# Tongji-MIC-Lab/TDVC

Measured on AMD Instinct MI355X. Metric: 1080p P-frames/sec (encode + reconstruct, lambda=2048 config), higher is better.
Workload: dtype f16; 1 GPU; 1x 1920x1080 (padded 1088x1920) 7-frame synthetic GOP (seed 1234), batch 1, P-frames coded in GOP order; gop=7, batch=1, parallelism=gop-sharded x1, weights=closed-form filler (no checkpoint ships)

## Files before the change

include/tdvc_hip.h:

```cpp
#ifndef TDVC_HIP_H
#define TDVC_HIP_H

#include <stdint.h>

#ifdef __cplusplus
extern "C" {
#endif

#define TDVC_OK 0
#define TDVC_EINVAL (-1)
#define TDVC_ENOSUP (-2)

typedef struct {
  void* p;
  int32_t N, H, W, C;
  int64_t sn;
  int32_t sp;
  int32_t dtype;
} tdvc_fmap;

enum { TDVC_F16 = 0, TDVC_F32 = 1 };
enum { TDVC_ACT_NONE = 0, TDVC_ACT_RELU = 1, TDVC_ACT_LRELU = 2, TDVC_ACT_CLAMP01 = 3, TDVC_ACT_SIGMOID = 4 };
enum { TDVC_GDN_NONE = 0, TDVC_GDN_FWD = 1, TDVC_GDN_INV = 2 };
enum { TDVC_OUT_NHWC = 0,
       TDVC_OUT_SHUFFLE2 = 1,
       TDVC_OUT_NCHW_F32 = 2 };

#define TDVC_MAX_TAPS 49

typedef struct {
  tdvc_fmap x;
  tdvc_fmap y;
  const void* w;
  const float* bias;
  int32_t cout;
  int32_t ntaps;
  int8_t tap_dy[TDVC_MAX_TAPS], tap_dx[TDVC_MAX_TAPS];
  int32_t kh, kw, stride, pad;
  int32_t ck;
  int32_t square_input;
  int32_t gdn;
  tdvc_fmap aux;
  int32_t act; float slope;
  int32_t round_before_act;
  tdvc_fmap res;
  tdvc_fmap res2;
  int32_t out_mode;
  int32_t s2d;
  int32_t bcast_T;
  float bcast_slope;
  float* chan_sum;
} tdvc_conv_desc;

int tdvc_abi_version(void);
const char* tdvc_last_error(void);
int tdvc_prepare_device(void);
const char* tdvc_last_conv_kernel(void);

int tdvc_set_predicate(const int* flag);
int tdvc_last_launch_predicated(void);
#define TDVC_MAX_PREDICATE_IMAGES 4
int tdvc_set_predicate_images(const int* flags, int n);
int tdvc_frame_changed(const tdvc_fmap* cur, tdvc_fmap* cache, int* flag, void* stream);
int tdvc_frames_changed(const tdvc_fmap* cur, tdvc_fmap* cache, int* flags, unsigned force_mask, void* stream);


int tdvc_conv_plan(int cin, int kh, int kw, int stride);
int64_t tdvc_conv_packed_bytes(int cout, int cin, int ntaps, int ck);
int tdvc_pack_conv_weights(const float* w_oihw, int cout, int cin_real, int cin, int kh, int kw,
                           int ntaps, const int8_t* tap_dy, const int8_t* tap_dx, int ck, uint16_t* dst);
int tdvc_conv2d(const tdvc_conv_desc* d, void* stream);
int tdvc_conv_chan_sum_rows(const tdvc_conv_desc* d);
const char* tdvc_conv_select(const tdvc_conv_desc* d);
int tdvc_conv2d_f32(const tdvc_conv_desc* d, void* stream);

typedef struct {
  tdvc_fmap x, y;
  const void* w;
  const float* bias;
  int32_t act1; float slope1;
  int32_t act2; float slope2;
  int32_t add_input;
  tdvc_fmap res2;
} tdvc_conv_pair_desc;
int64_t tdvc_conv_pair_packed_bytes(void);
int tdvc_pack_conv_pair_weights(const float* w1_oihw, const float* w2_oihw, uint16_t* dst);
int tdvc_conv_pair_supported(const tdvc_conv_pair_desc* d);
int tdvc_conv_pair(const tdvc_conv_pair_desc* d, void* stream);

typedef struct {
  tdvc_fmap x, om, y;
  const void* w;
  const float* bias;
  int32_t groups;
  int32_t act; float slope; int32_t round_before_act;
  void* x_planar;
} tdvc_dcn_desc;
int tdvc_dcn_fused(const tdvc_dcn_desc* d, void* stream);

int tdvc_dcn_v2_forward_f32(const float* input, const float* weight, const float* bias,
                            const float* offset, const float* mask, float* output,
                            int B, int C, int H, int W, int Cout,
                            int kh, int kw, int sh, int sw, int ph, int pw, int dh, int dw,
                            int deformable_group, void* stream);
int tdvc_dcn_v2_backward_f32(const float* input, const float* weight, const float* bias,
                             const float* offset, const float* mask, const float* grad_output,
                             float* grad_input, float* grad_offset, float* grad_mask,
                             float* grad_weight, float* grad_bias, float* columns,
                             int B, int C, int H, int W, int Cout,
                             int kh, int kw, int sh, int sw, int ph, int pw, int dh, int dw,
                             int deformable_group, void* stream);

int tdvc_nchw_to_fmap(const float* src, int C, const tdvc_fmap* y, void* stream);
int tdvc_fmap_to_nchw(const tdvc_fmap* x, int C, float* dst, void* stream);
int tdvc_scale_act_res(const tdvc_fmap* a, const float* gate, int act, float slope,
                       const tdvc_fmap* r, float r_sign, const tdvc_fmap* y, const tdvc_fmap* y2, void* stream);
int tdvc_add_flow(const tdvc_fmap* off, const tdvc_fmap* flow, void* stream);
int tdvc_bcast_add_act(const tdvc_fmap* x, const tdvc_fmap* b, int T, float slope, void* stream);

int tdvc_channel_sum(const tdvc_fmap* x, float* partial, int nblocks, void* stream);
int tdvc_se_gate(const float* partial, int nblocks, float inv_count, int N, int C, int Cmid,
                 const float* w1, const float* b1, const float* w2, const float* b2,
                 float* gate, void* stream);

int tdvc_upsample2x(const tdvc_fmap* x, const tdvc_fmap* y, void* stream);
int tdvc_avgpool2(const tdvc_fmap* x, const tdvc_fmap* y, void* stream);
int tdvc_spynet_level_input(const tdvc_fmap* ref, const tdvc_fmap* supp, const tdvc_fmap* flow_lo,
                            const tdvc_fmap* flow_up, const tdvc_fmap* cat8, void* stream);
int tdvc_resize_bilinear(const tdvc_fmap* x, const tdvc_fmap* y, const float* chscale, void* stream);

int64_t tdvc_avgpool_k_work_floats(int N, int hp, int wp, int C, int scale);
int tdvc_avgpool_k(const tdvc_fmap* x, int scale, float* pooled, int hp, int wp, float* work, int64_t work_floats, void* stream);
int tdvc_patch_match(const float* pin, const float* pref, int N, int hp, int wp, int C,
                     int32_t* idx, void* stream);
int tdvc_match_gather(const tdvc_fmap* fin, const tdvc_fmap* fref, const int32_t* idx, int scale,
                      int hp, int wp, const tdvc_fmap* cat, void* stream);

int tdvc_eb_forward(const tdvc_fmap* z, const float* params, const tdvc_fmap* noise,
                    const tdvc_fmap* z_hat, double* bits_out, float* partial, int partial_cap, void* stream);
int tdvc_gc_forward(const tdvc_fmap* y, const tdvc_fmap* gp, const tdvc_fmap* noise,
                    double* bits_out, float* partial, int partial_cap, void* stream);
int tdvc_quantize(const tdvc_fmap* y, const tdvc_fmap* noise, const tdvc_fmap* y_hat, void* stream);

int64_t tdvc_rans_encode(const int32_t* symbols, const int32_t* indexes, int64_t n,
                         const int32_t* cdfs, int32_t cdf_stride, const int32_t* cdf_sizes,
                         const int32_t* offsets, uint8_t* out, int64_t cap);
int tdvc_rans_decode(const uint8_t* data, int64_t nbytes, const int32_t* indexes, int64_t n,
                     const int32_t* cdfs, int32_t cdf_stride, const int32_t* cdf_sizes,
                     const int32_t* offsets, int32_t* symbols_out);

void* tdvc_rans_decoder_create(const uint8_t* data, int64_t nbytes);
int tdvc_rans_decoder_decode(void* handle, const int32_t* indexes, int64_t n, const int32_t* cdfs,
                             int32_t cdf_stride, const int32_t* cdf_sizes, const int32_t* offsets,
                             int32_t* symbols_out);
void tdvc_rans_decoder_destroy(void* handle);

int64_t tdvc_rans_encode_lanes(const int32_t* symbols, const int32_t* indexes, int64_t npos, int M, int L,
                               const int32_t* cdfs, int32_t cdf_stride, const int32_t* cdf_sizes,
                               const int32_t* offsets, uint8_t* out, int64_t cap);
int tdvc_rans_decode_lanes(const uint8_t* data, int64_t nbytes, const int32_t* indexes, int64_t npos, int M,
                           const int32_t* cdfs, int32_t cdf_stride, const int32_t* cdf_sizes,
                           const int32_t* offsets, int32_t* symbols_out);

int tdvc_pmf_to_quantized_cdf(const float* pmf, int n, int precision, int32_t* cdf_out);

int tdvc_ar_gather_batch(const tdvc_fmap* y_hat, const tdvc_fmap* params, const int32_t* pos, int npos,
                         const tdvc_fmap* x1, const tdvc_fmap* pc, void* stream);
int tdvc_ar_quantize_batch(const tdvc_fmap* y, const tdvc_fmap* gp, const int32_t* pos, int npos, const float* scale_table, int ntable,
                           const int32_t* symbols_in, const tdvc_fmap* y_hat, int32_t* symbols, int32_t* indexes, int64_t cbase, void* stream);
int tdvc_ar_indexes_batch(const tdvc_fmap* gp, const int32_t* pos, int npos, int B, const float* scale_table, int ntable,
                          int M, int H, int W, int32_t* indexes, int64_t cbase, void* stream);
int tdvc_ar_wavefront_batch(const uint8_t* const* data, const int64_t* nbytes, int B, const int32_t* cdfs, int32_t cdf_stride,
                            const int32_t* cdf_sizes, const int32_t* offsets, const tdvc_fmap* y, const tdvc_fmap* y_hat,
                            const tdvc_fmap* params, const tdvc_fmap* x1, const tdvc_fmap* pc, const tdvc_conv_desc* convs, int nconvs,
                            const tdvc_fmap* gp, const int32_t* pos_dev, const int32_t* step_sizes, int nsteps, int M, int W,
                            const float* scale_table, int ntable, int32_t* idx_dev, int32_t* sym_dev, void* stream);
int tdvc_ar_decode_serial_batch(const uint8_t* const* data, const int64_t* nbytes, int B, const int32_t* cdfs, int32_t cdf_stride,
                                const int32_t* cdf_sizes, const int32_t* offsets, const tdvc_fmap* y_hat, const tdvc_fmap* params,
                                const tdvc_fmap* x1, const tdvc_fmap* pc, const tdvc_conv_desc* convs, int nconvs, const tdvc_fmap* gp,
// ... 123 lines not shown
```

tdvc_amd/_lib.py:

```python
from __future__ import annotations

import ctypes as C
import os

_HERE = os.path.dirname(os.path.abspath(__file__))
LIB_PATH = os.path.join(_HERE, "libtdvc_hip.so")

MAX_TAPS = 49
F16, F32 = 0, 1
ACT_NONE, ACT_RELU, ACT_LRELU, ACT_CLAMP01, ACT_SIGMOID = 0, 1, 2, 3, 4
GDN_NONE, GDN_FWD, GDN_INV = 0, 1, 2
OUT_NHWC, OUT_SHUFFLE2, OUT_NCHW_F32 = 0, 1, 2


class FMapDesc(C.Structure):
    _fields_ = [("p", C.c_void_p), ("N", C.c_int32), ("H", C.c_int32), ("W", C.c_int32), ("C", C.c_int32),
                ("sn", C.c_int64), ("sp", C.c_int32), ("dtype", C.c_int32)]


class ConvDesc(C.Structure):
    _fields_ = [("x", FMapDesc), ("y", FMapDesc), ("w", C.c_void_p), ("bias", C.c_void_p),
                ("cout", C.c_int32), ("ntaps", C.c_int32),
                ("tap_dy", C.c_int8 * MAX_TAPS), ("tap_dx", C.c_int8 * MAX_TAPS),
                ("kh", C.c_int32), ("kw", C.c_int32), ("stride", C.c_int32), ("pad", C.c_int32),
                ("ck", C.c_int32), ("square_input", C.c_int32), ("gdn", C.c_int32),
                ("aux", FMapDesc), ("act", C.c_int32), ("slope", C.c_float),
                ("round_before_act", C.c_int32), ("res", FMapDesc), ("res2", FMapDesc), ("out_mode", C.c_int32), ("s2d", C.c_int32),
                ("bcast_T", C.c_int32), ("bcast_slope", C.c_float), ("chan_sum", C.c_void_p)]


class DcnDesc(C.Structure):
    _fields_ = [("x", FMapDesc), ("om", FMapDesc), ("y", FMapDesc), ("w", C.c_void_p), ("bias", C.c_void_p),
                ("groups", C.c_int32), ("act", C.c_int32), ("slope", C.c_float), ("round_before_act", C.c_int32), ("x_planar", C.c_void_p)]


class ConvPairDesc(C.Structure):
    _fields_ = [("x", FMapDesc), ("y", FMapDesc), ("w", C.c_void_p), ("bias", C.c_void_p), ("act1", C.c_int32), ("slope1", C.c_float),
                ("act2", C.c_int32), ("slope2", C.c_float), ("add_input", C.c_int32), ("res2", FMapDesc)]


class WgradReduceJob(C.Structure):
    _fields_ = [("work", C.c_void_p), ("bwork", C.c_void_p), ("row_off", C.c_void_p), ("chan_off", C.c_void_p), ("tap_off", C.c_void_p),
                ("bias_index", C.c_void_p), ("dw", C.c_void_p), ("db", C.c_void_p), ("scale", C.c_float),
                ("nworkers", C.c_int32), ("cow", C.c_int32), ("ciw", C.c_int32), ("ntaps", C.c_int32), ("cout", C.c_int32), ("cin", C.c_int32),
                ("wblocks", C.c_int32), ("nblocks", C.c_int32)]


_P = C.c_void_p
_FM = C.POINTER(FMapDesc)
_i, _f, _i64 = C.c_int, C.c_float, C.c_int64

SIGNATURES = {
    "tdvc_abi_version": (_i, []),
    "tdvc_conv_chan_sum_rows": (_i, [C.POINTER(ConvDesc)]),
    "tdvc_conv_select": (C.c_char_p, [C.POINTER(ConvDesc)]),
    "tdvc_last_error": (C.c_char_p, []),
    "tdvc_last_conv_kernel": (C.c_char_p, []),
    "tdvc_prepare_device": (_i, []),
    "tdvc_set_predicate": (_i, [_P]),
    "tdvc_set_predicate_images": (_i, [_P, _i]),
    "tdvc_last_launch_predicated": (_i, []),
    "tdvc_frame_changed": (_i, [_FM, _FM, _P, _P]),
    "tdvc_frames_changed": (_i, [_FM, _FM, _P, C.c_uint, _P]),
    "tdvc_conv_plan": (_i, [_i, _i, _i, _i]),
    "tdvc_conv_packed_bytes": (_i64, [_i, _i, _i, _i]),
    "tdvc_pack_conv_weights": (_i, [_P, _i, _i, _i, _i, _i, _i, _P, _P, _i, _P]),
    "tdvc_conv2d": (_i, [C.POINTER(ConvDesc), _P]),
    "tdvc_conv2d_f32": (_i, [C.POINTER(ConvDesc), _P]),
    "tdvc_pack_conv_weights_indexed": (_i, [_P] * 7 + [_i] * 4 + [_P, _P]),
    "tdvc_pack_conv_weights_indexed_f32": (_i, [_P] * 7 + [_i] * 4 + [_P, _P]),
    "tdvc_pack_job_blocks": (_i64, [_i, _i, _i, _i]),
    "tdvc_pack_conv_weights_batch": (_i, [_P, _P, _i, _i, _P]),
    "tdvc_act_backward": (_i, [_FM, _FM, _FM, _i, _f, _FM, _P]),
    "tdvc_pixel_unshuffle": (_i, [_FM, _FM, _P]),
    "tdvc_bias_grad_work_floats": (_i64, [_i, _i]),
    "tdvc_bias_grad": (_i, [_FM, _i, _P, _f, _P, _P, _i64, _P]),
    "tdvc_copy_cast": (_i, [_FM, _FM, _P]),
    "tdvc_clamp01_backward": (_i, [_FM, _FM, _P]),
    "tdvc_gate_backward_work_floats": (_i64, [_i, _i]),
    "tdvc_gate_backward": (_i, [_FM, _FM, _P, _FM, _P, _P, _i64, _P]),
    "tdvc_se_gate_backward": (_i, [_P, _i, _f, _i, _i, _i] + [_P] * 6 + [_f] + [_P] * 6),
    "tdvc_bcast_channel_add": (_i, [_FM, _P, _f, _P]),
    "tdvc_add_flow_backward": (_i, [_FM, _FM, _P]),
    "tdvc_bcast_add_act_backward": (_i, [_FM, _FM, _FM, _f, _P]),
    "tdvc_upsample2x_backward": (_i, [_FM, _FM, _P]),
    "tdvc_resize_bilinear_backward": (_i, [_FM, _FM, _P, _P]),
    "tdvc_spynet_level_input_backward": (_i, [_FM, _FM, _FM, _FM, _FM, _P]),
    "tdvc_sigmoid_f32": (_i, [_P, _P, _i64, _P]),
    "tdvc_sigmoid_backward_f32": (_i, [_P, _P, _i64, _P]),
    "tdvc_axpy_f32": (_i, [_P, _P, _f, _i64, _P]),
    "tdvc_match_gather_backward": (_i, [_FM, _FM, _P, _i, _i, _i, _FM, _FM, _FM, _P]),
    "tdvc_eb_backward": (_i, [_FM, _P, _FM, _f, _FM, _P, _P]),
    "tdvc_eb_pack": (_i, [_P, _P, _P, _i, _P]),
    "tdvc_eb_param_chain": (_i, [_P, _P, _P, _f, _i, _P]),
    "tdvc_eb_aux": (_i, [_P, _P, _f, _P, _P, _i, _P]),
    "tdvc_gc_backward": (_i, [_FM, _FM, _FM, _f, _FM, _FM, _P]),
    "tdvc_dcn_columns": (_i, [_FM, _FM, _i, _FM, _P]),
    "tdvc_ar_lanes_state_bytes": (_i64, [_i]),
    "tdvc_ar_gather_batch": (_i, [_FM, _FM, _P, _i, _FM, _FM, _P]),
    "tdvc_ar_quantize_batch": (_i, [_FM, _FM, _P, _i, _P, _i, _P, _FM, _P, _P, _i64, _P]),
    "tdvc_ar_indexes_batch": (_i, [_FM, _P, _i, _i, _P, _i, _i, _i, _i, _P, _i64, _P]),
    "tdvc_ar_wavefront_batch": (_i, [_P, _P, _i, _P, _i, _P, _P, _FM, _FM, _FM, _FM, _FM, _P, _i, _FM, _P, _P, _i, _i, _i, _P, _i, _P, _P, _P]),
    "tdvc_ar_decode_serial_batch": (_i, [_P, _P, _i, _P, _i, _P, _P, _FM, _FM, _FM, _FM, _P, _i, _FM, _P, _i, _i, _i, _P, _i, _P, _P, _P]),
    "tdvc_ar_lanes_batch_layout": (_i64, [_P, _i, _i, _P]),
    "tdvc_ar_lanes_init_batch": (_i, [_P, _i64, _P, _i, _i, _P, _P]),
    "tdvc_ar_decode_lanes_step_batch": (_i, [_FM, _P, _i, _P, _i, _P, _i64, _P, _i, _P, C.c_int32, _P, _P, _P, C.c_int32, _P, _FM, _P, _P, _i64, _P]),
    "tdvc_ar_wavefront_lanes_batch": (_i, [_P, _P, _i, _P, _i64, _P, _P, C.c_int32, _P, _P, _P, C.c_int32, _FM, _FM, _FM, _FM, _P, _i, _FM, _P, _P, _i, _i, _i,
                                           _P, _i, _P, _P, _P, _P]),
# ... 85 lines not shown
```

tdvc_amd/csrc/conv_common.h:

```cpp
#pragma once
#include "common.h"

namespace convk {

struct ConvParams {
  const half_t* x; long x_sn; int x_sp; int H, W, Cin;
  const half_t* w; const float* bias;
  FMap y; int Ho, Wo; int cout;
  FMap aux; FMap res; FMap res2;
  int ntaps, kh, kw, pad;
  int in_stride;
  int nchunks, steps;
  int square, gdn, act; float slope; int round16, out_mode;
  int tiles_x;
  int simple;
  int s2d, Corig;
  int reverse;
  int bcast_T; float bcast_slope;
  float* csum;
  int8_t tap_dy[TDVC_MAX_TAPS], tap_dx[TDVC_MAX_TAPS];
  const int* pred;
};

enum ConvSwitch { SW_NONE = -1, SW_V2, SW_V3, SW_V5, SW_V7, SW_V9, SW_V10, SW_V11, SW_ROW, SW_C8, SW_N16, SW_GDN128, SW_COUNT };
int conv_on(int id);
long conv_v9_work_limit();

constexpr long LARGE_MAP_PIXELS = 8192;

inline bool taps_dense(const tdvc_conv_desc* d, int kh, int kw, int pad) {
  if (d->ntaps != kh * kw || d->kh != kh || d->kw != kw || d->pad != pad) return false;
  for (int t = 0; t < d->ntaps; ++t)
    if (d->tap_dy[t] != t / kw || d->tap_dx[t] != t % kw) return false;
  return true;
}

inline bool all_waves_store(const tdvc_conv_desc* d, int wave_ch) {
  const int ych = d->out_mode == TDVC_OUT_SHUFFLE2 ? d->cout >> 2 : (d->cout + wave_ch - 1) / wave_ch * wave_ch;
  return d->y.C > ych - wave_ch;
}

inline int persistent_grid_x(int slots, int cout_blocks, int N, int ntiles) {
  const int gx = slots / (cout_blocks * N);
  return gx < 1 ? 1 : (gx > ntiles ? ntiles : gx);
}

template <auto Kern, typename... Args>
int launch_big_lds(const char* what, int lds_limit, dim3 grid, dim3 block, int lds, hipStream_t st, Args... args) {
  static TdvcPerDeviceFlag raised;
  bool& done = raised.flag();
  if (!done) {
    const hipError_t err = hipFuncSetAttribute(reinterpret_cast<const void*>(Kern), hipFuncAttributeMaxDynamicSharedMemorySize, lds_limit);
    if (err != hipSuccess) { tdvc_set_error("%s: hipFuncSetAttribute failed: %s", what, hipGetErrorString(err)); return (int)err; }
    done = true;
  }
  hipLaunchKernelGGL(Kern, grid, block, lds, st, args...);
  return tdvc_launch_status(what);
}


template <bool F32MAPS = false>
__device__ __forceinline__ void epilogue4(const ConvParams& p, int n, int oy, int ox, int co, float v[4]) {
  if (p.bias) {
    const f32x4 b4 = *reinterpret_cast<const f32x4*>(p.bias + co);
#pragma unroll
    for (int i = 0; i < 4; ++i) v[i] += b4[i];
  }
  int py = oy, px = ox, pc = co, PW = p.Wo;
  if (p.out_mode == TDVC_OUT_SHUFFLE2) {
    const int cq = p.cout >> 2;
    const int sub = co / cq;
    pc = co - sub * cq;
    py = 2 * oy + (sub >> 1);
    px = 2 * ox + (sub & 1);
    PW = 2 * p.Wo;
  }
  if (p.gdn) {
// ... 149 lines not shown
#pragma unroll
  for (int k0 = 0; k0 < 4; k0 += KB) {
    half8 r0[KB], r1[KB], r2[KB];
    int opix[KB], apix[KB];
    bool ok[KB];
#pragma unroll
    for (int k = 0; k < KB; ++k) {
      const int ox = ox_first + (k0 + k) * 8 + prow;
      ok[k] = full ? ch_ok : (row_ok && ox < p.Wo);
      opix[k] = ok[k] ? (mul * oy + sub_y) * PW + (mul * ox + sub_x) : 0;
      apix[k] = ok[k] ? oy * p.Wo + ox : 0;
    }
    if (gdn) {
      const half_t* ab = reinterpret_cast<const half_t*>(p.aux.p) + (long)n * p.aux.sn + (ch_ok ? co : 0);
#pragma unroll
      for (int k = 0; k < KB; ++k) r0[k] = *reinterpret_cast<const half8*>(ab + (long)apix[k] * p.aux.sp);
    }
    if (has1) {
      const half_t* rb = reinterpret_cast<const half_t*>(p.res.p) + (long)n * p.res.sn + pcc;
#pragma unroll
      for (int k = 0; k < KB; ++k) r1[k] = *reinterpret_cast<const half8*>(rb + (long)opix[k] * p.res.sp);
    }
    if (has2) {
      const half_t* rb = reinterpret_cast<const half_t*>(p.res2.p) + (long)n * p.res2.sn + pcc;
#pragma unroll
      for (int k = 0; k < KB; ++k) r2[k] = *reinterpret_cast<const half8*>(rb + (long)opix[k] * p.res2.sp);
    }
#pragma unroll
    for (int k = 0; k < KB; ++k) {
      half8 h = *reinterpret_cast<const half8*>(ew + ((k0 + k) * 8 + prow) * EPS + chunk * 16);
      if (gdn) {
        float v[8];
#pragma unroll
        for (int j = 0; j < 8; ++j) v[j] = (float)r0[k][j] * (p.gdn == TDVC_GDN_FWD ? rsqrtf((float)h[j]) : sqrtf((float)h[j]));
        if (has1) {
#pragma unroll
          for (int j = 0; j < 8; ++j) v[j] += (float)r1[k][j];
        }
        if (has2) {
#pragma unroll
          for (int j = 0; j < 8; ++j) v[j] += (float)r2[k][j];
        }
#pragma unroll
        for (int j = 0; j < 8; ++j) h[j] = (half_t)v[j];
      } else {
        if (has1) h = h + r1[k];
        if (has2) h = h + r2[k];
      }
      if (ok[k]) *reinterpret_cast<half8*>(reinterpret_cast<half_t*>(p.y.p) + (long)n * p.y.sn + (long)opix[k] * p.y.sp + pc) = h;
    }
  }
}

template <int NTX, bool BIAS_IN_ACC, bool BCAST = false, bool CSUM = false>
__device__ __forceinline__ void epilogue_lean_seq(const ConvParams& p, f32x16 (&acc)[2][NTX], const float* bias64, unsigned char* ew, int n,
                                                  int cbase, int oy_first, int ox_first, int lane, bool zero_acc, bool full, float* cs = nullptr) {
  constexpr int EPS = 144;
  const int hh = lane >> 5, r = lane & 31;
  const int chunk = lane & 7, prow = lane >> 3;
  const int co = cbase + chunk * 8;
  const bool ch_ok = co < p.y.C && co < ((p.cout + 63) & ~63);
  const int cc = ch_ok ? co : 0;
  const bool has1 = p.res.p != nullptr, has2 = p.res2.p != nullptr;
  const half_t sl = (half_t)p.slope;
  const half2v sl2 = {sl, sl}, zero2 = {(half_t)0.f, (half_t)0.f};
  const bool act = p.slope != 1.f, relu = p.slope == 0.f;
  half_t* yb = reinterpret_cast<half_t*>(p.y.p) + (long)n * p.y.sn + cc;
  const half_t* rb1 = reinterpret_cast<const half_t*>(p.res.p) + (long)n * p.res.sn + cc;
  const half_t* rb2 = reinterpret_cast<const half_t*>(p.res2.p) + (long)n * p.res2.sn + cc;
  f32x4 b4[2][4];
  if constexpr (!BIAS_IN_ACC) {
#pragma unroll
    for (int mt = 0; mt < 2; ++mt)
#pragma unroll
      for (int g = 0; g < 4; ++g) b4[mt][g] = *reinterpret_cast<const f32x4*>(bias64 + mt * 32 + 8 * g + 4 * hh);
  }
#pragma unroll
  for (int nt = 0; nt < NTX; ++nt) {
    const int oy = oy_first + nt;
    int opix[4];
    bool ok[4];
#pragma unroll
    for (int k = 0; k < 4; ++k) {
      const int ox = ox_first + k * 8 + prow;
      ok[k] = full ? ch_ok : (ch_ok && oy < p.Ho && ox < p.Wo);
      opix[k] = ok[k] ? oy * p.Wo + ox : 0;
    }
    half8 r1[4], r2[4];
    if (has1 && !BCAST) {
#pragma unroll
      for (int k = 0; k < 4; ++k) r1[k] = *reinterpret_cast<const half8*>(rb1 + (long)opix[k] * p.res.sp);
    }
    if (has2) {
#pragma unroll
      for (int k = 0; k < 4; ++k) r2[k] = *reinterpret_cast<const half8*>(rb2 + (long)opix[k] * p.res2.sp);
    }
#pragma unroll
    for (int mt = 0; mt < 2; ++mt)
#pragma unroll
      for (int g = 0; g < 4; ++g) {
        float v[4];
#pragma unroll
        for (int i = 0; i < 4; ++i) {
          v[i] = acc[mt][nt][4 * g + i];
          if constexpr (!BIAS_IN_ACC) {
            v[i] += b4[mt][g][i];
            if (zero_acc) acc[mt][nt][4 * g + i] = 0.f;
          }
        }
        half2v lo = {(half_t)v[0], (half_t)v[1]}, hi = {(half_t)v[2], (half_t)v[3]};
        if (relu) {
          lo = __builtin_elementwise_max(lo, zero2);
          hi = __builtin_elementwise_max(hi, zero2);
        } else if (act) {
          lo = __builtin_elementwise_max(lo, lo * sl2);
          hi = __builtin_elementwise_max(hi, hi * sl2);
        }
        const half4 o = {lo[0], lo[1], hi[0], hi[1]};
        *reinterpret_cast<half4*>(ew + r * EPS + (mt * 32 + 8 * g + 4 * hh) * 2) = o;
      }
    if constexpr (BCAST) {
#pragma unroll
      for (int k = 0; k < 4; ++k) {
        const half8 v = *reinterpret_cast<const half8*>(ew + (k * 8 + prow) * EPS + chunk * 16);
        half_t* yp = yb + (long)opix[k] * p.y.sp;
        const half_t* sp = has1 ? rb1 + (long)opix[k] * p.res.sp : yp;
        half8 xs[4];
#pragma unroll
        for (int t = 0; t < 4; ++t) xs[t] = *reinterpret_cast<const half8*>(sp + t * 64);
#pragma unroll
        for (int t = 0; t < 4; ++t) {
          half8 o;
#pragma unroll
          for (int j = 0; j < 8; ++j) {
            const float s = (float)xs[t][j] + (float)v[j];
            o[j] = (half_t)(s > 0.f ? s : s * p.bcast_slope);
          }
          if (ok[k]) *reinterpret_cast<half8*>(yp + t * 64) = o;
        }
      }
      continue;
    }
#pragma unroll
    for (int k = 0; k < 4; ++k) {
      half8 v = *reinterpret_cast<const half8*>(ew + (k * 8 + prow) * EPS + chunk * 16);
      if (has1) v = v + r1[k];
      if (has2) v = v + r2[k];
      if (ok[k]) *reinterpret_cast<half8*>(yb + (long)opix[k] * p.y.sp) = v;
      if constexpr (CSUM) {
#pragma unroll
        for (int j = 0; j < 8; ++j) cs[j] += ok[k] ? (float)v[j] : 0.f;
      }
    }
  }
}

template <int NTX, bool BIAS_IN_ACC = false, int MODE = 3>
__device__ __forceinline__ void epilogue_simple_rows(const ConvParams& p, f32x16 (&acc)[2][NTX], const float* bias64,
                                                     unsigned char* ew, int n, int cbase, int oy_first, int ox_first,
                                                     int lane, bool zero_acc, bool full = false) {
  if constexpr (MODE == 2) {
    epilogue_lean_seq<NTX, BIAS_IN_ACC>(p, acc, bias64, ew, n, cbase, oy_first, ox_first, lane, zero_acc, full);
    return;
  }
  if constexpr (MODE == 3) {
    if (p.simple == 2) {
      epilogue_lean_seq<NTX, BIAS_IN_ACC>(p, acc, bias64, ew, n, cbase, oy_first, ox_first, lane, zero_acc, full);
      return;
    }
  }
  PackedRow rows[NTX];
  epilogue_pack<NTX, BIAS_IN_ACC>(p, acc, bias64, lane, rows, zero_acc);
#pragma unroll
  for (int nt = 0; nt < NTX; ++nt) epilogue_store_row(p, rows[nt], ew, n, cbase, oy_first + nt, ox_first, lane, full);
}

inline bool conv_is_lean(const ConvParams& p) {
  return conv_is_simple(p) && p.out_mode == TDVC_OUT_NHWC && !p.gdn;
}

template <int NRES, int NR, bool STAMPED = false>
__device__ __forceinline__ void epilogue_lean_rows(const ConvParams& p, const f32x16 (&acc)[2][NR], unsigned char* ew, int n,
                                                   int cbase, int oy, int ox_first, int lane, bool full, long long* st = nullptr) {
#define EST(i) do { if constexpr (STAMPED) { if (st) st[i] = clock64(); } } while (0)
  static_assert(NR % 2 == 0, "two rows per round");
  constexpr int EPS = 144, EROW = 32 * EPS;
  const int hh = lane >> 5, r = lane & 31;
  const int chunk = lane & 7, prow = lane >> 3;
  const int co = cbase + chunk * 8;
  const bool ch_ok = co < p.y.C && co < ((p.cout + 63) & ~63);
  const int cc = ch_ok ? co : 0;
  int opix[NR][4];
  bool ok[NR][4];
#pragma unroll
  for (int j = 0; j < NR; ++j)
#pragma unroll
    for (int k = 0; k < 4; ++k) {
      const int ox = ox_first + k * 8 + prow;
      ok[j][k] = full ? ch_ok : (ch_ok && oy + j < p.Ho && ox < p.Wo);
      opix[j][k] = ok[j][k] ? (oy + j) * p.Wo + ox : 0;
// ... 61 lines not shown
```

tdvc_amd/csrc/conv_dispatch.hip:

```cpp
#include <stdlib.h>

#include "conv_common.h"

using convk::ConvParams;
bool conv_v2_eligible(const tdvc_conv_desc* d, int Ho, int Wo); int launch_conv_v2(const ConvParams& p, int cout_blocks, int N, hipStream_t st);
bool conv_v3_eligible(const tdvc_conv_desc* d, int Ho, int Wo); int launch_conv_v3(const ConvParams& p, int cout_blocks, int N, hipStream_t st);
bool conv_v5_eligible(const tdvc_conv_desc* d, int Ho, int Wo); int launch_conv_v5(const ConvParams& p, int cout_blocks, int N, hipStream_t st); int conv_v5_chan_sum_rows(int Ho, int Wo, int cout_blocks, int N);
bool conv_v7_eligible(const tdvc_conv_desc* d, const ConvParams& p, int Ho, int Wo); int launch_conv_v7(const ConvParams& p, int cout_blocks, int N, hipStream_t st);
bool conv_v9_eligible(const tdvc_conv_desc* d, int Ho, int Wo, bool v3_ok); int launch_conv_v9(const ConvParams& p, int ck8, int cout_tiles32, int N, hipStream_t st);
bool conv_v10_eligible(const tdvc_conv_desc* d, const ConvParams& p, int Ho, int Wo); int launch_conv_v10(const ConvParams& p, int cout_blocks, int N, hipStream_t st);
bool conv_v11_eligible(const tdvc_conv_desc* d, const ConvParams& p, int Ho, int Wo); int launch_conv_v11(const ConvParams& p, int cout_blocks, int N, hipStream_t st);
int conv_row_geometry(const tdvc_conv_desc* d, const ConvParams& p, int Ho, int Wo); int launch_conv_row(int geo, const ConvParams& p, int N, hipStream_t st);
bool conv_c8_eligible(const tdvc_conv_desc* d, const ConvParams& p, int Ho, int Wo); int launch_conv_c8(const ConvParams& p, int N, hipStream_t st);
bool conv_n16_eligible(const tdvc_conv_desc* d, int Ho, int Wo); int launch_conv_n16(const ConvParams& p, int N, hipStream_t st);
bool gdn128_eligible(const tdvc_conv_desc* d, const ConvParams& p, int Ho, int Wo); int launch_gdn128(const ConvParams& p, int N, hipStream_t st);
int conv_direct_lds_bytes(const tdvc_conv_desc* d);
int conv_cout_tiles(int cout);
int launch_conv_direct(const ConvParams& p, int ck8, int stride, int N, hipStream_t st);
int conv_f32_validate(const tdvc_conv_desc* d, int& Ho, int& Wo);

namespace {
const char* const kSwitchEnv[convk::SW_COUNT] = {nullptr, "TDVC_CONV_NO_V3", "TDVC_CONV_NO_V5", "TDVC_CONV_NO_V7", "TDVC_CONV_NO_V9", "TDVC_CONV_NO_V10",
                                                 "TDVC_CONV_NO_V11", "TDVC_CONV_NO_ROW", "TDVC_CONV_NO_C8", "TDVC_CONV_NO_N16", "TDVC_CONV_NO_GDN128"};
int g_enabled[convk::SW_COUNT] = {1, 1, 1, 1, 1, 1, 1, 15, 1, 1, 1};
long g_v9_work_limit = 1L << 20;
}

int convk::conv_on(int id) {
  static const struct EnvOff {
    bool off[convk::SW_COUNT];
    EnvOff() {
      const bool v1 = getenv("TDVC_CONV_V1") != nullptr;
      for (int i = 0; i < convk::SW_COUNT; ++i) off[i] = v1 || (kSwitchEnv[i] && getenv(kSwitchEnv[i]) != nullptr);
    }
  } env;
  return id == convk::SW_NONE ? 1 : (env.off[id] ? 0 : g_enabled[id]);
}
long convk::conv_v9_work_limit() { return g_v9_work_limit; }

extern "C" void tdvc_debug_enable_conv_v9(int enable) { g_enabled[convk::SW_V9] = enable != 0; }
extern "C" void tdvc_debug_enable_conv_v10(int enable) { g_enabled[convk::SW_V10] = enable != 0; }
extern "C" void tdvc_debug_enable_conv_v11(int enable) { g_enabled[convk::SW_V11] = enable != 0; }
extern "C" void tdvc_debug_enable_conv_row(int mask) { g_enabled[convk::SW_ROW] = mask; }
extern "C" void tdvc_debug_enable_conv_c8(int enable) { g_enabled[convk::SW_C8] = enable != 0; }
extern "C" void tdvc_debug_enable_conv_n16(int enable) { g_enabled[convk::SW_N16] = enable != 0; }
extern "C" void tdvc_debug_enable_gdn128(int enable) { g_enabled[convk::SW_GDN128] = enable != 0; }
extern "C" void tdvc_debug_set_conv_v9_work_limit(long v) { g_v9_work_limit = v; }

namespace {

struct Pick {
  const tdvc_conv_desc* d;
  int Ho, Wo;
  int geo;
  int ck8() const { return d->ck / 8; }
  int N() const { return d->x.N; }
  int cout_blocks() const { return conv_cout_tiles(d->cout) / 2; }
};

struct Entry {
  const char* name;
  int sw;
  bool (*eligible)(Pick& k, const ConvParams& p);
  int (*launch)(const Pick& k, const ConvParams& p, hipStream_t st);
  bool (*only)(const tdvc_conv_desc* d);
  const char* only_msg;
};

bool v3_on_and_eligible(const Pick& k) { return convk::conv_on(convk::SW_V3) && conv_v3_eligible(k.d, k.Ho, k.Wo); }

bool bcast_eligible(Pick& k, const ConvParams& p) {
  const tdvc_conv_desc* d = k.d;
  return d->bcast_T == 4 && d->kh == 1 && d->kw == 1 && d->stride == 1 && d->pad == 0 && d->cout == 64 && d->y.C == 64 && d->y.sp >= 4 * 64 &&
         d->y.dtype == TDVC_F16 && d->out_mode == TDVC_OUT_NHWC && d->act == TDVC_ACT_NONE && !d->gdn && !d->res2.p &&
         (!d->res.p || (d->res.dtype == TDVC_F16 && d->res.C == 64 && d->res.sp >= 4 * 64 && d->res.N == d->y.N && d->res.H == d->y.H && d->res.W == d->y.W)) &&
         !d->square_input && !d->round_before_act && d->bias && d->bcast_slope >= 0.f && d->bcast_slope <= 1.f && conv_v5_eligible(d, k.Ho, k.Wo) &&
         convk::conv_is_lean(p);
}
int bcast_launch(const Pick& k, const ConvParams& p, hipStream_t st) {
  ConvParams q = p;
  q.simple = 2;
  q.slope = 1.f;
  return launch_conv_v5(q, 1, k.N(), st);
}
bool row_eligible(Pick& k, const ConvParams& p) { return (k.geo = conv_row_geometry(k.d, p, k.Ho, k.Wo)) >= 0; }

constexpr char kNameV5[] = "conv_mfma_v5", kNameDirect[] = "conv_mfma<%d,%d,%d>";

const Entry kTable[] = {
    {"conv_mfma_v5(bcast)", convk::SW_V5, bcast_eligible, bcast_launch, [](const tdvc_conv_desc* d) { return d->bcast_T != 0; },
     "tdvc_conv2d: bcast_T needs a plain 1x1 / stride 1 conv to 64 channels of >= 8192 pixels, y (and res, the optional source of the slices) a 64-channel window of a buffer with >= 4 slices, bcast_T == 4"},
    {"conv_row(s2d)", convk::SW_ROW, [](Pick& k, const ConvParams& p) { return k.d->s2d && row_eligible(k, p); },
     [](const Pick& k, const ConvParams& p, hipStream_t st) { return launch_conv_row(k.geo, p, k.N(), st); }, nullptr, nullptr},
    {"conv_mfma_v3(s2d)", convk::SW_V3, [](Pick& k, const ConvParams&) { return k.d->s2d && conv_v3_eligible(k.d, k.Ho, k.Wo); },
     [](const Pick& k, const ConvParams& p, hipStream_t st) { return launch_conv_v3(p, k.cout_blocks(), k.N(), st); },
     [](const tdvc_conv_desc* d) { return d->s2d != 0; }, "tdvc_conv2d: s2d conv not eligible for the stage-pipelined kernel"},
    {"conv_mfma_v9", convk::SW_V9, [](Pick& k, const ConvParams&) { return conv_v9_eligible(k.d, k.Ho, k.Wo, v3_on_and_eligible(k)); },
     [](const Pick& k, const ConvParams& p, hipStream_t st) { return launch_conv_v9(p, k.ck8(), conv_cout_tiles(k.d->cout), k.N(), st); }, nullptr, nullptr},
    {"gdn128", convk::SW_GDN128, [](Pick& k, const ConvParams& p) { return gdn128_eligible(k.d, p, k.Ho, k.Wo); },
// ... 74 lines not shown
    if (d->y.dtype == TDVC_F16) TDVC_CHECK((d->y.C % 8) == 0, "tdvc_conv2d: fp16 output C %% 8");
  }
  if (d->gdn) {
    TDVC_CHECK(fmap_ok16(d->aux) && d->aux.H == Ho && d->aux.W == Wo && d->aux.N == d->x.N && d->aux.C >= d->cout &&
                   !shuf && (d->cout % 64) == 0,
               "tdvc_conv2d: GDN aux fmap mismatch");
  }
  if (d->res.p) {
    TDVC_CHECK(d->res.dtype == TDVC_F32 ? fmap_ok32(d->res) : fmap_ok16(d->res), "tdvc_conv2d: bad residual fmap");
    TDVC_CHECK(d->res.N == d->x.N && d->res.H == (shuf ? 2 * Ho : Ho) && d->res.W == (shuf ? 2 * Wo : Wo),
               "tdvc_conv2d: residual geometry mismatch");
  }
  if (d->res2.p) {
    TDVC_CHECK(fmap_ok16(d->res2) && d->res2.N == d->x.N && d->res2.H == (shuf ? 2 * Ho : Ho) && d->res2.W == (shuf ? 2 * Wo : Wo),
               "tdvc_conv2d: bad second residual fmap");
  }
  if (d->bias) TDVC_CHECK(aligned16(d->bias), "tdvc_conv2d: bias unaligned");

  memset(&p, 0, sizeof(p));
  p.x = reinterpret_cast<const half_t*>(d->x.p); p.x_sn = d->x.sn; p.x_sp = d->x.sp;
  p.H = d->x.H; p.W = d->x.W; p.Cin = d->x.C;
  p.w = reinterpret_cast<const half_t*>(d->w); p.bias = d->bias;
  p.y = to_dev(d->y); p.Ho = Ho; p.Wo = Wo; p.cout = d->cout;
  p.aux = d->gdn ? to_dev(d->aux) : null_fmap();
  p.res = d->res.p ? to_dev(d->res) : null_fmap();
  p.res2 = d->res2.p ? to_dev(d->res2) : null_fmap();
  p.ntaps = d->ntaps; p.kh = d->kh; p.kw = d->kw; p.pad = d->pad;
  p.in_stride = d->stride;
  p.s2d = d->s2d; p.Corig = d->x.C;
  p.bcast_T = d->bcast_T; p.bcast_slope = d->bcast_slope;
  p.nchunks = d->s2d ? (4 * d->x.C) / d->ck : (d->x.C + d->ck - 1) / d->ck;
  p.steps = (d->ntaps * (d->ck / 8) + 1) / 2;
  p.square = d->square_input; p.gdn = d->gdn; p.act = d->act; p.slope = d->slope;
  p.round16 = d->round_before_act; p.out_mode = d->out_mode;
  memcpy(p.tap_dy, d->tap_dy, sizeof(p.tap_dy));
  memcpy(p.tap_dx, d->tap_dx, sizeof(p.tap_dx));
  p.tiles_x = (Wo + 31) / 32;
  if (conv_cout_tiles(d->cout) > 1 && convk::conv_is_simple(p)) {
    p.simple = convk::conv_is_lean(p) ? 2 : 1;
    p.slope = convk::conv_simple_slope(p);
  }
  return TDVC_OK;
}

thread_local char g_last_kernel[48] = "";

thread_local unsigned g_walk_parity = 0;
int g_walk_mode = -1;
int next_walk_reverse() {
  if (g_walk_mode < 0) { const char* e = getenv("TDVC_CONV_WALK"); g_walk_mode = e ? atoi(e) : 1; }
  return g_walk_mode == 1 ? (int)(g_walk_parity++ & 1u) : 0;
}

int conv2d_impl(const tdvc_conv_desc* d, void* stream, bool query_rows) {
  TDVC_CHECK(d, "tdvc_conv2d: null descriptor");
  if (d->x.dtype == TDVC_F32) {
    if (query_rows) return 0;
    TDVC_CHECK(!d->chan_sum, "tdvc_conv2d: chan_sum is not available on the fp32 path (tdvc_conv_chan_sum_rows() == 0)");
    snprintf(g_last_kernel, sizeof(g_last_kernel), "conv_f32");
    return tdvc_conv2d_f32(d, stream);
  }
  ConvParams p;
  Pick k = {d, 0, 0, -1};
  if (const int rc = prepare(d, p, k.Ho, k.Wo)) return rc;
  p.reverse = query_rows ? 0 : next_walk_reverse();
  const Entry* e = select(k, p);
  const bool csum_ok = e && e->name == kNameV5 && k.cout_blocks() == 1 && p.simple == 2;
  if (query_rows) return csum_ok ? conv_v5_chan_sum_rows(k.Ho, k.Wo, 1, k.N()) : 0;
  TDVC_CHECK(!d->chan_sum || (csum_ok && (reinterpret_cast<uintptr_t>(d->chan_sum) & 15) == 0),
             "tdvc_conv2d: chan_sum on a conv whose kernel has no fused channel sum (tdvc_conv_chan_sum_rows() == 0) or unaligned");
  p.csum = d->chan_sum;
  if (!e) return TDVC_EINVAL;
  kernel_name(e, k, g_last_kernel);
  return e->launch(k, p, reinterpret_cast<hipStream_t>(stream));
}

}

extern "C" void tdvc_debug_set_conv_walk(int mode) { g_walk_mode = mode; }
extern "C" int tdvc_conv2d(const tdvc_conv_desc* d, void* stream) { return conv2d_impl(d, stream, false); }
extern "C" int tdvc_conv_chan_sum_rows(const tdvc_conv_desc* d) { return conv2d_impl(d, nullptr, true); }
extern "C" const char* tdvc_last_conv_kernel(void) { return g_last_kernel; }

extern "C" const char* tdvc_conv_select(const tdvc_conv_desc* d) {
  static thread_local char name[48];
  if (!d) { tdvc_set_error("tdvc_conv_select: null descriptor"); return nullptr; }
  if (d->x.dtype == TDVC_F32) {
    int Ho, Wo;
    return conv_f32_validate(d, Ho, Wo) == TDVC_OK ? "conv_f32" : nullptr;
  }
  ConvParams p;
  Pick k = {d, 0, 0, -1};
  if (prepare(d, p, k.Ho, k.Wo) != TDVC_OK) return nullptr;
  const Entry* e = select(k, p);
  if (!e) return nullptr;
  kernel_name(e, k, name);
  return name;
}
```

tdvc_amd/csrc/conv_mfma_v5.hip:

```cpp
#include <type_traits>

#include "conv_common.h"

using convk::ConvParams;

namespace {

typedef unsigned u32x4 __attribute__((ext_vector_type(4)));

constexpr int WR = 2, TW5 = 32, CK5 = 32, PS5 = 80, NTHR5 = 512, NWAVE = 8;
constexpr int WSL5 = 4096;

struct V5Extra {
  int nbtiles;
  int wtile_bytes;
};

template <int SIMPLE, int TL>
__global__ __launch_bounds__(NTHR5, 1) void conv_mfma_v5_kernel(const ConvParams p, const V5Extra e) {
  extern __shared__ __attribute__((aligned(16))) unsigned char smem[];
  int* tapoff = reinterpret_cast<int*>(smem);
  float* bias_s = reinterpret_cast<float*>(smem + 256);
  unsigned char* wlds = smem + 512;
  const int tid = threadIdx.x, lane = tid & 63, wave = tid >> 6;
// ... 67 lines not shown

  f32x16 acc[2][WR];
#pragma unroll
  for (int mt = 0; mt < 2; ++mt)
#pragma unroll
    for (int nt = 0; nt < WR; ++nt)
#pragma unroll
      for (int i = 0; i < 16; ++i) acc[mt][nt][i] = 0.f;

  float cs[8] = {0.f, 0.f, 0.f, 0.f, 0.f, 0.f, 0.f, 0.f};
  issue(I0{}, 0);
  if (nstages > 1) issue(I1{}, 1);

  auto stage = [&](auto setc, int S) {
    constexpr int SET = decltype(setc)::value;
    const int tile_i = S / nchunks, ch = S - tile_i * nchunks;
#pragma unroll
    for (int j = 0; j < TL; ++j) {
      const u32x4 z = {0u, 0u, 0u, 0u};
      u32x4 val = ((okmask[SET] >> j) & 1u) ? treg[SET][j] : z;
      if (p.square) {
        half8 hv = __builtin_bit_cast(half8, val);
        hv = hv * hv;
        val = __builtin_bit_cast(u32x4, hv);
      }
      if (it_dst[j] >= 0) *reinterpret_cast<u32x4*>(tbuf + it_dst[j]) = val;
    }

    const unsigned char* wch = wlds + ch * ntaps * WSL5 + lane * 16;
    for (int t = 0; t < ntaps; ++t) {
      const unsigned char* wslot = wch + t * WSL5;
      const int toff = tapoff[t];
#pragma unroll
      for (int s2 = 0; s2 < 2; ++s2) {
        half8 a[2], b[WR];
#pragma unroll
        for (int mt = 0; mt < 2; ++mt) a[mt] = *reinterpret_cast<const half8*>(wslot + (mt * 2 + s2) * 1024);
#pragma unroll
        for (int nt = 0; nt < WR; ++nt) b[nt] = *reinterpret_cast<const half8*>(tbuf + base[nt] + toff + s2 * 32);
#pragma unroll
        for (int mt = 0; mt < 2; ++mt)
#pragma unroll
          for (int nt = 0; nt < WR; ++nt)
            acc[mt][nt] = __builtin_amdgcn_mfma_f32_32x32x16_f16(a[mt], b[nt], acc[mt][nt], 0, 0, 0);
      }
    }

    if (ch == nchunks - 1) {
      const int tile = p.reverse ? e.nbtiles - 1 - (first + tile_i * stride) : first + tile_i * stride;
      const int ty = tile / p.tiles_x, tx = tile - ty * p.tiles_x;
      const int oy0 = ty * (WR * NWAVE) + wave * WR;
      if constexpr (SIMPLE == 4) {
        convk::epilogue_lean_seq<WR, false, true>(p, acc, bias_s, tbuf, n, cb * 64, oy0, tx * TW5, lane, true, false);
      } else if constexpr (SIMPLE) {
        if (SIMPLE == 2 && p.csum) convk::epilogue_lean_seq<WR, false, false, true>(p, acc, bias_s, tbuf, n, cb * 64, oy0, tx * TW5, lane, true, false, cs);
        else convk::epilogue_simple_rows<WR, false, SIMPLE>(p, acc, bias_s, tbuf, n, cb * 64, oy0, tx * TW5, lane, true);
      } else {
        const int ox = tx * TW5 + r;
#pragma unroll
        for (int nt = 0; nt < WR; ++nt) {
          const int oy = oy0 + nt;
          const bool ok = oy < p.Ho && ox < p.Wo;
#pragma unroll
          for (int mt = 0; mt < 2; ++mt) {
#pragma unroll
            for (int g = 0; g < 4; ++g) {
              float v[4];
#pragma unroll
              for (int i = 0; i < 4; ++i) { v[i] = acc[mt][nt][4 * g + i]; acc[mt][nt][4 * g + i] = 0.f; }
              if (ok) convk::epilogue4(p, n, oy, ox, (cb * 2 + mt) * 32 + 8 * g + 4 * hh, v);
            }
          }
        }
      }
    }
    if (S + 2 < nstages) issue(setc, S + 2);
  };
  for (int S = 0; S < nstages; S += 2) {
    stage(I0{}, S);
    if (S + 1 < nstages) stage(I1{}, S + 1);
  }
  if (SIMPLE == 2 && p.csum) {
#pragma unroll
    for (int j = 0; j < 8; ++j) {
      cs[j] += __shfl_xor(cs[j], 8);
      cs[j] += __shfl_xor(cs[j], 16);
      cs[j] += __shfl_xor(cs[j], 32);
    }
    if (lane < 8) {
      float* o = p.csum + (((long)n * gridDim.x + blockIdx.x) * NWAVE + wave) * 64 + lane * 8;
      *reinterpret_cast<f32x4*>(o) = f32x4{cs[0], cs[1], cs[2], cs[3]};
      *reinterpret_cast<f32x4*>(o + 4) = f32x4{cs[4], cs[5], cs[6], cs[7]};
    }
  }
}

inline int v5_wtile_bytes(int kh, int kw) {
  const int b = (WR + kh - 1) * (TW5 + kw - 1) * PS5;
  return b < 32 * 144 ? 32 * 144 : b;
}
inline int v5_lds_bytes(int kh, int kw, int ntaps, int nchunks) { return 512 + nchunks * ntaps * WSL5 + NWAVE * v5_wtile_bytes(kh, kw); }
inline int v5_tl(int kh, int kw) { return ((WR + kh - 1) * (TW5 + kw - 1) * 4 + 63) / 64; }

template <int TL>
int launch_tl(const ConvParams& q, const V5Extra& e, int mode, dim3 grid, int lds, hipStream_t st) {
  const auto go = mode == 4 ? convk::launch_big_lds<&conv_mfma_v5_kernel<4, TL>, ConvParams, V5Extra>
                  : mode == 2 ? convk::launch_big_lds<&conv_mfma_v5_kernel<2, TL>, ConvParams, V5Extra>
                  : mode == 1 ? convk::launch_big_lds<&conv_mfma_v5_kernel<1, TL>, ConvParams, V5Extra>
                              : convk::launch_big_lds<&conv_mfma_v5_kernel<0, TL>, ConvParams, V5Extra>;
  return go("tdvc_conv2d(v5)", 160 * 1024, grid, dim3(NTHR5), lds, st, q, e);
}

}

bool conv_v5_eligible(const tdvc_conv_desc* d, int Ho, int Wo) {
  const int nchunks = (d->x.C + CK5 - 1) / CK5;
  const int tl = v5_tl(d->kh, d->kw);
  const bool stride_ok = d->stride == 1 || (d->stride == 2 && d->kh == 1 && d->kw == 1 && d->pad == 0);
  return d->ck == 32 && stride_ok && d->ntaps >= 1 && d->ntaps <= 9 && d->kh <= 3 && d->kw <= 3 && d->cout >= 64 &&
         d->x.C >= 32 && !d->s2d && ((long)Ho * Wo >= convk::LARGE_MAP_PIXELS || d->stride == 2) && tl == 4 &&
         v5_lds_bytes(d->kh, d->kw, d->ntaps, nchunks) <= 160 * 1024;
}

static int v5_grid_x(int nbtiles, int cout_blocks, int N) { return convk::persistent_grid_x(256, cout_blocks, N, nbtiles); }
int conv_v5_chan_sum_rows(int Ho, int Wo, int cout_blocks, int N) {
  const int nbtiles = ((Wo + TW5 - 1) / TW5) * ((Ho + WR * NWAVE - 1) / (WR * NWAVE));
  return v5_grid_x(nbtiles, cout_blocks, N) * NWAVE;
}

int launch_conv_v5(const ConvParams& p, int cout_blocks, int N, hipStream_t st) {
  ConvParams q = p;
  q.tiles_x = (p.Wo + TW5 - 1) / TW5;
  const int tiles_y = (p.Ho + WR * NWAVE - 1) / (WR * NWAVE);
  V5Extra e;
  e.nbtiles = q.tiles_x * tiles_y;
  e.wtile_bytes = v5_wtile_bytes(p.kh, p.kw);
  const int lds = v5_lds_bytes(p.kh, p.kw, p.ntaps, p.nchunks);
  const bool simple = convk::conv_is_simple(p);
  if (simple) q.slope = convk::conv_simple_slope(p);
  dim3 grid(v5_grid_x(e.nbtiles, cout_blocks, N), cout_blocks, N);
  const int tl = v5_tl(p.kh, p.kw);
  if (tl == 4) return launch_tl<4>(q, e, p.bcast_T ? 4 : (simple ? (convk::conv_is_lean(p) ? 2 : 1) : 0), grid, lds, st);
  tdvc_set_error("conv v5: unsupported window %dx%d", p.kh, p.kw);
  return TDVC_EINVAL;
}
```

tdvc_amd/csrc/conv_n16.hip:

```cpp
#include "conv_common.h"

using convk::ConvParams;

namespace {

constexpr int N16_TH = 8, N16_TW = 64, N16_NTHR = 512;

struct N16Extra {
  int ksteps;
  int ps;
  int a_bytes;
  int ntiles, tiles_x;
  int cin_shift;
};

template <int NCB>
__global__ __launch_bounds__(N16_NTHR, 1) void conv_n16_kernel(const ConvParams p, const N16Extra e) {
  extern __shared__ __attribute__((aligned(16))) unsigned char smem[];
  unsigned char* wl = smem;
  unsigned char* tile = wl + e.a_bytes;
  const int tid = threadIdx.x, lane = tid & 63;
  const int wave = __builtin_amdgcn_readfirstlane(tid >> 6);
  const int px = lane & 15, kg = lane >> 4;
  const int TIW = N16_TW + p.kw - 1, TIH = N16_TH + p.kh - 1;
// ... 63 lines not shown
      const int off = frag_off(S);
#pragma unroll
      for (int cb = 0; cb < NCB; ++cb) a[cb] = *reinterpret_cast<const half8*>(wl + ((S * NCB + cb) * 64 + lane) * 16);
#pragma unroll
      for (int c = 0; c < 4; ++c) b[c] = *reinterpret_cast<const half8*>(tile + off + c * cstep);
    };
    auto mm = [&](half8 (&a)[NCB], half8 (&b)[4]) {
#pragma unroll
      for (int c = 0; c < 4; ++c)
#pragma unroll
        for (int cb = 0; cb < NCB; ++cb) acc[cb][c] = __builtin_amdgcn_mfma_f32_16x16x32_f16(a[cb], b[c], acc[cb][c], 0, 0, 0);
    };
    const int KS = e.ksteps;
    load(0, a0, b0);
    for (int S = 0; S < KS; S += 2) {
      load(min(S + 1, KS - 1), a1, b1);
      mm(a0, b0);
      load(min(S + 2, KS - 1), a0, b0);
      if (S + 1 < KS) mm(a1, b1);
    }

    const int oy = ty * N16_TH + wave;
#pragma unroll
    for (int c = 0; c < 4; ++c) {
      const int ox = tx * N16_TW + 16 * c + px;
      if (oy < p.Ho && ox < p.Wo) {
#pragma unroll
        for (int cb = 0; cb < NCB; ++cb) {
          float v[4] = {acc[cb][c][0], acc[cb][c][1], acc[cb][c][2], acc[cb][c][3]};
          convk::epilogue4(p, n, oy, ox, 16 * cb + 4 * kg, v);
        }
      }
    }
  }
}

inline int n16_ps(int cin) { return 2 * cin + 16; }
inline int n16_ksteps(int ntaps, int cin) { return (ntaps * cin + 31) / 32; }
inline int n16_lds(int cin, int kh, int kw, int ntaps, int ncb) {
  return n16_ksteps(ntaps, cin) * ncb * 1024 + (N16_TH + kh - 1) * (N16_TW + kw - 1) * n16_ps(cin);
}

}

bool conv_n16_eligible(const tdvc_conv_desc* d, int Ho, int Wo) {
  const int cin = d->x.C;
  const bool cin_ok = cin == 8 || cin == 16 || cin == 32 || cin == 64;
  const bool dense = convk::taps_dense(d, d->kh, d->kw, d->pad);
  return cin_ok && dense && d->ck == cin && d->stride == 1 && d->cout <= 32 && !d->s2d && !d->square_input && !d->gdn &&
         (long)Ho * Wo >= convk::LARGE_MAP_PIXELS &&
         n16_lds(cin, d->kh, d->kw, d->ntaps, d->cout <= 16 ? 1 : 2) <= 150 * 1024;
}

int launch_conv_n16(const ConvParams& p, int N, hipStream_t st) {
  const int ncb = p.cout <= 16 ? 1 : 2;
  N16Extra e;
  e.ksteps = n16_ksteps(p.ntaps, p.Cin);
  e.ps = n16_ps(p.Cin);
  e.a_bytes = e.ksteps * ncb * 1024;
  e.tiles_x = (p.Wo + N16_TW - 1) / N16_TW;
  e.ntiles = N * e.tiles_x * ((p.Ho + N16_TH - 1) / N16_TH);
  e.cin_shift = p.Cin == 8 ? 3 : p.Cin == 16 ? 4 : p.Cin == 32 ? 5 : 6;
  const int lds = n16_lds(p.Cin, p.kh, p.kw, p.ntaps, ncb);
  const int per_cu = lds <= 78 * 1024 ? 2 : 1;
  int grid = e.ntiles < 256 * per_cu ? e.ntiles : 256 * per_cu;
  const auto go = ncb == 1 ? convk::launch_big_lds<&conv_n16_kernel<1>, ConvParams, N16Extra> : convk::launch_big_lds<&conv_n16_kernel<2>, ConvParams, N16Extra>;
  return go("tdvc_conv2d(n16)", 160 * 1024, dim3(grid), dim3(N16_NTHR), lds, st, p, e);
}
```

tdvc_amd/csrc/lib.cpp:

```cpp
#include <hip/hip_runtime.h>
#include <stdarg.h>
#include <stdio.h>

#include <mutex>

#include "../../include/tdvc_hip.h"

static thread_local char g_err[512] = "";

void tdvc_set_error(const char* fmt, ...) {
  va_list ap;
  va_start(ap, fmt);
  vsnprintf(g_err, sizeof(g_err), fmt, ap);
  va_end(ap);
}

extern "C" int tdvc_abi_version(void) { return 10; }
extern "C" const char* tdvc_last_error(void) { return g_err; }

static thread_local const int* g_pred = nullptr;
static thread_local int g_pred_taken = 0, g_pred_last = 0;
static thread_local const int* g_pred_img = nullptr;
static thread_local int g_pred_img_n = 0;

extern "C" int tdvc_set_predicate(const int* flag) {
  if (reinterpret_cast<uintptr_t>(flag) & 3) { tdvc_set_error("tdvc_set_predicate: flag must be 4-byte aligned"); return TDVC_EINVAL; }
  if (flag && g_pred_img) { tdvc_set_error("tdvc_set_predicate: a per-image predicate is set (clear it first)"); return TDVC_EINVAL; }
  g_pred = flag;
  return TDVC_OK;
}
extern "C" int tdvc_set_predicate_images(const int* flags, int n) {
  if (!flags || n == 0) { g_pred_img = nullptr; g_pred_img_n = 0; return TDVC_OK; }
  if (reinterpret_cast<uintptr_t>(flags) & 3) { tdvc_set_error("tdvc_set_predicate_images: flags must be 4-byte aligned"); return TDVC_EINVAL; }
  if (n < 1 || n > TDVC_MAX_PREDICATE_IMAGES) { tdvc_set_error("tdvc_set_predicate_images: 1 <= n <= %d images, got %d", TDVC_MAX_PREDICATE_IMAGES, n); return TDVC_EINVAL; }
  if (g_pred) { tdvc_set_error("tdvc_set_predicate_images: a launch predicate is set (clear it first)"); return TDVC_EINVAL; }
  g_pred_img = flags; g_pred_img_n = n;
  return TDVC_OK;
}
const int* tdvc_launch_predicate_images(int N) {
  if (!g_pred_img || N != g_pred_img_n) return nullptr;
  g_pred_taken = 1;
  return g_pred_img;
}
extern "C" int tdvc_last_launch_predicated(void) { return g_pred_last; }
const int* tdvc_launch_predicate() {
  g_pred_taken = g_pred != nullptr;
  return g_pred;
}
static thread_local long g_launches = 0, g_loop_launches = 0;
void tdvc_note_launch() {
  g_pred_last = g_pred_taken;
  g_pred_taken = 0;
  ++g_launches;
}
long tdvc_launch_count() { return g_launches; }
void tdvc_set_loop_launches(long n) { g_loop_launches = n; }
extern "C" int64_t tdvc_ar_last_loop_launches(void) { return g_loop_launches; }

namespace {
constexpr int kMaxDev = 64;
constexpr size_t kZeroBytes = 4096, kDumpBytes = 16384;
std::mutex g_scratch_mu;
unsigned char* g_scratch[kMaxDev] = {};
}

int tdvc_scratch_pages(const void** zeros, void** dump) {
  int dev = 0;
  hipError_t err = hipGetDevice(&dev);
  if (err != hipSuccess || dev < 0 || dev >= kMaxDev) {
    tdvc_set_error("scratch pages: hipGetDevice failed or device index %d out of range: %s", dev, hipGetErrorString(err));
// ... 22 lines not shown
```

tdvc_amd/csrc/pointwise.hip:

```cpp
#include "pointwise_common.h"

namespace {

__global__ void nchw_to_fmap_kernel(const float* src, int C, FMap y) {
  const long npix = (long)y.H * y.W;
  const long i = (long)blockIdx.x * blockDim.x + threadIdx.x;
  if (i >= npix * y.N) return;
  const int n = (int)(i / npix);
  const long pix = i % npix;
  for (int c0 = 0; c0 < y.C; c0 += 8) {
    float v[8];
#pragma unroll
    for (int j = 0; j < 8; ++j) v[j] = (c0 + j < C) ? src[((long)n * C + c0 + j) * npix + pix] : 0.f;
    store8(y, n, pix, c0, v);
  }
}

__global__ void fmap_to_nchw_kernel(FMap x, int C, float* dst) {
  const long npix = (long)x.H * x.W;
  const long i = (long)blockIdx.x * blockDim.x + threadIdx.x;
  if (i >= npix * x.N) return;
  const int n = (int)(i / npix);
  const long pix = i % npix;
  for (int c0 = 0; c0 < C; c0 += 8) {
    float v[8];
    load8(x, n, pix, c0, v);
#pragma unroll
    for (int j = 0; j < 8; ++j)
      if (c0 + j < C) dst[((long)n * C + c0 + j) * npix + pix] = v[j];
  }
}

__global__ void scale_act_res_kernel(FMap a, const float* gate, int act, float slope, FMap r, float rs, FMap y, FMap y2) {
  const int chunks = (a.C + 7) / 8;
  const long npix = (long)a.H * a.W;
  const long i = (long)blockIdx.x * blockDim.x + threadIdx.x;
  if (i >= npix * chunks * a.N) return;
  const int c = (int)(i % chunks) * 8;
  const long t = i / chunks;
  const long pix = t % npix;
  const int n = (int)(t / npix);
  float v[8];
  load8(a, n, pix, c, v);
  if (gate) {
#pragma unroll
    for (int j = 0; j < 8; ++j)
      if (c + j < a.C) v[j] *= gate[(long)n * a.C + c + j];
  }
  if (act) {
#pragma unroll
    for (int j = 0; j < 8; ++j) v[j] = act_apply(v[j], act, slope);
  }
  if (r.p) {
    float q[8];
    load8(r, n, pix, c, q);
#pragma unroll
    for (int j = 0; j < 8; ++j) v[j] += rs * q[j];
  }
  store8(y, n, pix, c, v);
  if (y2.p) store8(y2, n, pix, c, v);
}

template <int U>
__global__ __launch_bounds__(256) void scale_act_res16_kernel(FMap a, const float* gate, int act, float slope, FMap r, float rs, FMap y, FMap y2,
                                                              unsigned total, unsigned chunks, unsigned npix) {
  const unsigned T = gridDim.x * 256u;
  for (unsigned base = blockIdx.x * 256u + threadIdx.x; base < total; base += U * T) {
    half8 av[U], rv[U];
    unsigned ck[U], nn[U];
    long pa[U];
    bool ok[U];
#pragma unroll
    for (int u = 0; u < U; ++u) {
      const unsigned i = base + u * T;
      ok[u] = i < total;
      const unsigned ii = ok[u] ? i : 0u;
      const unsigned pp = ii / chunks;
      ck[u] = ii - pp * chunks;
      nn[u] = pp / npix;
      pa[u] = (long)(pp - nn[u] * npix);
      av[u] = *reinterpret_cast<const half8*>(reinterpret_cast<const half_t*>(a.p) + (long)nn[u] * a.sn + pa[u] * a.sp + ck[u] * 8);
      if (r.p) rv[u] = *reinterpret_cast<const half8*>(reinterpret_cast<const half_t*>(r.p) + (long)nn[u] * r.sn + pa[u] * r.sp + ck[u] * 8);
    }
#pragma unroll
    for (int u = 0; u < U; ++u) {
      float v[8];
#pragma unroll
      for (int j = 0; j < 8; ++j) v[j] = (float)av[u][j];
      if (gate) {
        const f32x4* g4 = reinterpret_cast<const f32x4*>(gate + (long)nn[u] * a.C + ck[u] * 8);
        const f32x4 g0 = g4[0], g1 = g4[1];
#pragma unroll
        for (int j = 0; j < 4; ++j) { v[j] *= g0[j]; v[4 + j] *= g1[j]; }
      }
      if (act) {
#pragma unroll
        for (int j = 0; j < 8; ++j) v[j] = act_apply(v[j], act, slope);
      }
      if (r.p) {
#pragma unroll
        for (int j = 0; j < 8; ++j) v[j] += rs * (float)rv[u][j];
      }
      half8 h;
#pragma unroll
      for (int j = 0; j < 8; ++j) h[j] = (half_t)v[j];
      if (ok[u]) {
        *reinterpret_cast<half8*>(reinterpret_cast<half_t*>(y.p) + (long)nn[u] * y.sn + pa[u] * y.sp + ck[u] * 8) = h;
        if (y2.p) *reinterpret_cast<half8*>(reinterpret_cast<half_t*>(y2.p) + (long)nn[u] * y2.sn + pa[u] * y2.sp + ck[u] * 8) = h;
      }
    }
  }
}

__global__ void add_flow_kernel(FMap off, FMap flow) {
  const int chunks = off.C / 8;
  const long npix = (long)off.H * off.W;
  const long i = (long)blockIdx.x * blockDim.x + threadIdx.x;
  if (i >= npix * chunks * off.N) return;
  const int c = (int)(i % chunks) * 8;
  const long t = i / chunks;
  const long pix = t % npix;
  const int n = (int)(t / npix);
  const float* fp = reinterpret_cast<const float*>(flow.p) + (long)n * flow.sn + pix * flow.sp;
  const float fx = fp[0], fy = fp[1];
  float v[8];
  load8(off, n, pix, c, v);
#pragma unroll
  for (int j = 0; j < 8; ++j) v[j] += (j & 1) ? fy : fx;
  store8(off, n, pix, c, v);
}

__global__ void bcast_add_act_kernel(FMap x, FMap b, float slope) {
  const int chunks = x.C / 8;
  const long npix = (long)x.H * x.W;
  const long i = (long)blockIdx.x * blockDim.x + threadIdx.x;
  if (i >= npix * chunks * x.N) return;
  const int c = (int)(i % chunks) * 8;
  const long t = i / chunks;
  const long pix = t % npix;
  const int n = (int)(t / npix);
  float v[8], q[8];
  load8(x, n, pix, c, v);
  load8(b, n, pix, c % b.C, q);
#pragma unroll
  for (int j = 0; j < 8; ++j) v[j] = act_apply(v[j] + q[j], TDVC_ACT_LRELU, slope);
  store8(x, n, pix, c, v);
}

template <int T>
__global__ __launch_bounds__(256) void bcast_add_act_t_kernel(FMap x, FMap b, float slope, unsigned total, unsigned chunks, unsigned npix) {
  const unsigned i = blockIdx.x * 256u + threadIdx.x;
  if (i >= total) return;
  const unsigned pp = i / chunks, ck = i - pp * chunks;
  const unsigned n = pp / npix;
  const long pix = (long)(pp - n * npix);
  const half8 bv = *reinterpret_cast<const half8*>(reinterpret_cast<const half_t*>(b.p) + (long)n * b.sn + pix * b.sp + ck * 8);
  half_t* xp = reinterpret_cast<half_t*>(x.p) + (long)n * x.sn + pix * x.sp + ck * 8;
  half8 xv[T];
#pragma unroll
  for (int t = 0; t < T; ++t) xv[t] = *reinterpret_cast<const half8*>(xp + t * b.C);
#pragma unroll
  for (int t = 0; t < T; ++t) {
    half8 h;
#pragma unroll
// ... 73 lines not shown
    for (int wy = 0; wy < ways; ++wy) s += part[wy * C + tid];
    mean[tid] = s * inv_count;
  }
  __syncthreads();
  if (tid < Cmid) {
    float s = b1[tid];
    for (int c = 0; c < C; ++c) s += w1[tid * C + c] * mean[c];
    mid[tid] = s > 0.f ? s : 0.f;
  }
  __syncthreads();
  if (tid < C) {
    float s = b2[tid];
    for (int j = 0; j < Cmid; ++j) s += w2[tid * Cmid + j] * mid[j];
    gate[(long)n * C + tid] = 1.f / (1.f + expf(-s));
  }
}

__global__ void upsample2x_kernel(FMap x, FMap y) {
  const int chunks = x.C / 8;
  const long npix = (long)y.H * y.W;
  const long i = (long)blockIdx.x * blockDim.x + threadIdx.x;
  if (i >= npix * chunks * y.N) return;
  const int c = (int)(i % chunks) * 8;
  const long t = i / chunks;
  const long pix = t % npix;
  const int n = (int)(t / npix);
  const int oy = (int)(pix / y.W), ox = (int)(pix % y.W);
  const float sy = fmaxf((oy + 0.5f) * 0.5f - 0.5f, 0.f), sx = fmaxf((ox + 0.5f) * 0.5f - 0.5f, 0.f);
  const int y0 = (int)sy, x0 = (int)sx;
  const int y1 = y0 + (y0 < x.H - 1), x1 = x0 + (x0 < x.W - 1);
  const float ly1 = sy - y0, lx1 = sx - x0, ly0 = 1.f - ly1, lx0 = 1.f - lx1;
  float a[8], b[8], cc[8], d[8], v[8];
  load8(x, n, (long)y0 * x.W + x0, c, a);
  load8(x, n, (long)y0 * x.W + x1, c, b);
  load8(x, n, (long)y1 * x.W + x0, c, cc);
  load8(x, n, (long)y1 * x.W + x1, c, d);
#pragma unroll
  for (int j = 0; j < 8; ++j) v[j] = ly0 * (lx0 * a[j] + lx1 * b[j]) + ly1 * (lx0 * cc[j] + lx1 * d[j]);
  store8(y, n, pix, c, v);
}

__global__ void avgpool2_kernel(FMap x, FMap y) {
  const long npix = (long)y.H * y.W;
  const long i = (long)blockIdx.x * blockDim.x + threadIdx.x;
  if (i >= npix * y.N) return;
  const int n = (int)(i / npix);
  const long pix = i % npix;
  const int oy = (int)(pix / y.W), ox = (int)(pix % y.W);
  const float* xp = reinterpret_cast<const float*>(x.p) + (long)n * x.sn;
  float* yp = reinterpret_cast<float*>(y.p) + (long)n * y.sn + pix * y.sp;
  const long p00 = ((long)(2 * oy) * x.W + 2 * ox) * x.sp, p10 = p00 + (long)x.W * x.sp;
  for (int c = 0; c < y.C; ++c)
    yp[c] = (xp[p00 + c] + xp[p00 + x.sp + c] + xp[p10 + c] + xp[p10 + x.sp + c]) * 0.25f;
}

template <bool VEC>
__global__ void spynet_level_input_kernel(FMap ref, FMap supp, FMap flow_lo, FMap flow_up, FMap cat8) {
  typedef float f32x2 __attribute__((ext_vector_type(2)));
  const int H = ref.H, W = ref.W;
  const long npix = (long)H * W;
  const long i = (long)blockIdx.x * blockDim.x + threadIdx.x;
  if (i >= npix * ref.N) return;
  const int n = (int)(i / npix);
  const long pix = i % npix;
  const int y = (int)(pix / W), x = (int)(pix % W);
  float fx = 0.f, fy = 0.f;
  if (flow_lo.p) {
    const int h2 = flow_lo.H, w2 = flow_lo.W;
    const float ry = (H > 1) ? (float)(h2 - 1) / (float)(H - 1) : 0.f;
    const float rx = (W > 1) ? (float)(w2 - 1) / (float)(W - 1) : 0.f;
    const float sy = ry * y, sx = rx * x;
    const int y0 = (int)sy, x0 = (int)sx;
    const int y1 = y0 + (y0 < h2 - 1), x1 = x0 + (x0 < w2 - 1);
    const float ly1 = sy - y0, lx1 = sx - x0, ly0 = 1.f - ly1, lx0 = 1.f - lx1;
    const float* fl = reinterpret_cast<const float*>(flow_lo.p) + (long)n * flow_lo.sn;
    const float* pa = fl + ((long)y0 * w2 + x0) * flow_lo.sp;
    const float* pb = fl + ((long)y0 * w2 + x1) * flow_lo.sp;
    const float* pc = fl + ((long)y1 * w2 + x0) * flow_lo.sp;
    const float* pd = fl + ((long)y1 * w2 + x1) * flow_lo.sp;
    f32x2 a, b, c, d;
    if constexpr (VEC) {
      a = *reinterpret_cast<const f32x2*>(pa); b = *reinterpret_cast<const f32x2*>(pb);
      c = *reinterpret_cast<const f32x2*>(pc); d = *reinterpret_cast<const f32x2*>(pd);
    } else {
      a = f32x2{pa[0], pa[1]}; b = f32x2{pb[0], pb[1]}; c = f32x2{pc[0], pc[1]}; d = f32x2{pd[0], pd[1]};
    }
    fx = (ly0 * (lx0 * a[0] + lx1 * b[0]) + ly1 * (lx0 * c[0] + lx1 * d[0])) * 2.0f;
    fy = (ly0 * (lx0 * a[1] + lx1 * b[1]) + ly1 * (lx0 * c[1] + lx1 * d[1])) * 2.0f;
  }
  const float gx = (float)x + fx, gy = (float)y + fy;
  const float wm = (float)(W - 1 > 1 ? W - 1 : 1), hm = (float)(H - 1 > 1 ? H - 1 : 1);
  const float nx = 2.0f * gx / wm - 1.0f, ny = 2.0f * gy / hm - 1.0f;
  float ix = ((nx + 1.f) / 2.f) * (float)(W - 1), iy = ((ny + 1.f) / 2.f) * (float)(H - 1);
  ix = fminf((float)(W - 1), fmaxf(ix, 0.f));
  iy = fminf((float)(H - 1), fmaxf(iy, 0.f));
  const float xw = floorf(ix), yn = floorf(iy);
  const int ix0 = (int)xw, iy0 = (int)yn, ix1 = ix0 + 1, iy1 = iy0 + 1;
  const float w_nw = ((float)ix1 - ix) * ((float)iy1 - iy), w_ne = (ix - (float)ix0) * ((float)iy1 - iy);
  const float w_sw = ((float)ix1 - ix) * (iy - (float)iy0), w_se = (ix - (float)ix0) * (iy - (float)iy0);
  const float* sp = reinterpret_cast<const float*>(supp.p) + (long)n * supp.sn;
  float wv[3] = {0.f, 0.f, 0.f};
  const bool x0ok = ix0 >= 0 && ix0 < W, x1ok = ix1 >= 0 && ix1 < W, y0ok = iy0 >= 0 && iy0 < H, y1ok = iy1 >= 0 && iy1 < H;
  const float* rp = reinterpret_cast<const float*>(ref.p) + (long)n * ref.sn + pix * ref.sp;
  float r3[3];
  if constexpr (VEC) {
    const int cx0 = min(max(ix0, 0), W - 1), cx1 = min(max(ix1, 0), W - 1), cy0 = min(max(iy0, 0), H - 1), cy1 = min(max(iy1, 0), H - 1);
// ... 333 lines not shown
  const int n = (int)(t / npix);
  float v[8];
  load8(y, n, pix, c, v);
  if (noise.p) {
    float q[8];
    load8(noise, n, pix, c, q);
#pragma unroll
    for (int j = 0; j < 8; ++j) v[j] += q[j];
  } else {
#pragma unroll
    for (int j = 0; j < 8; ++j) v[j] = rintf(v[j]);
  }
  store8(y_hat, n, pix, c, v);
}

}

extern "C" int tdvc_nchw_to_fmap(const float* src, int C, const tdvc_fmap* y, void* stream) {
  TDVC_CHECK(src && y && fmap_any(*y) && C >= 1 && C <= y->C, "tdvc_nchw_to_fmap: bad arguments");
  const long total = (long)y->N * y->H * y->W;
  hipLaunchKernelGGL(nchw_to_fmap_kernel, grid1d(total), dim3(EW_BLOCK), 0, ST(stream), src, C, to_dev(*y));
  return tdvc_launch_status("tdvc_nchw_to_fmap");
}

extern "C" int tdvc_fmap_to_nchw(const tdvc_fmap* x, int C, float* dst, void* stream) {
  TDVC_CHECK(dst && x && fmap_any(*x) && C >= 1 && C <= x->C, "tdvc_fmap_to_nchw: bad arguments");
  const long total = (long)x->N * x->H * x->W;
  hipLaunchKernelGGL(fmap_to_nchw_kernel, grid1d(total), dim3(EW_BLOCK), 0, ST(stream), to_dev(*x), C, dst);
  return tdvc_launch_status("tdvc_fmap_to_nchw");
}

extern "C" int tdvc_scale_act_res(const tdvc_fmap* a, const float* gate, int act, float slope,
                                  const tdvc_fmap* r, float r_sign, const tdvc_fmap* y, const tdvc_fmap* y2, void* stream) {
  TDVC_CHECK(a && y && fmap_any(*a) && fmap_any(*y) && same_geom(*a, *y) && y->C == a->C, "tdvc_scale_act_res: bad a/y");
  if (r) TDVC_CHECK(fmap_any(*r) && same_geom(*a, *r) && r->C == a->C, "tdvc_scale_act_res: bad residual");
  if (y2) TDVC_CHECK(fmap_any(*y2) && same_geom(*a, *y2) && y2->C == a->C, "tdvc_scale_act_res: bad y2");
  const long total = (long)a->N * a->H * a->W * ((a->C + 7) / 8);
  const bool all16 = a->dtype == TDVC_F16 && y->dtype == TDVC_F16 && (!r || r->dtype == TDVC_F16) && (!y2 || y2->dtype == TDVC_F16) &&
                     (!gate || aligned16(gate)) && total < (1L << 31) - (1L << 23);
  if (all16) {
    constexpr int U = 4;
    long blocks = (total + 256 * U - 1) / (256 * U);
    if (blocks > 4096) blocks = 4096;
    hipLaunchKernelGGL(scale_act_res16_kernel<U>, dim3((unsigned)blocks), dim3(256), 0, ST(stream), to_dev(*a), gate, act, slope,
                       r ? to_dev(*r) : null_fmap(), r_sign, to_dev(*y), y2 ? to_dev(*y2) : null_fmap(), (unsigned)total, (unsigned)(a->C / 8),
                       (unsigned)((long)a->H * a->W));
    return tdvc_launch_status("tdvc_scale_act_res");
  }
  hipLaunchKernelGGL(scale_act_res_kernel, grid1d(total), dim3(EW_BLOCK), 0, ST(stream), to_dev(*a), gate, act, slope,
                     r ? to_dev(*r) : null_fmap(), r_sign, to_dev(*y), y2 ? to_dev(*y2) : null_fmap());
  return tdvc_launch_status("tdvc_scale_act_res");
}

extern "C" int tdvc_add_flow(const tdvc_fmap* off, const tdvc_fmap* flow, void* stream) {
  TDVC_CHECK(off && flow && fmap_ok16(*off) && fmap_ok32(*flow) && flow->C >= 2 && same_geom(*off, *flow), "tdvc_add_flow: bad arguments");
  const long total = (long)off->N * off->H * off->W * (off->C / 8);
  hipLaunchKernelGGL(add_flow_kernel, grid1d(total), dim3(EW_BLOCK), 0, ST(stream), to_dev(*off), to_dev(*flow));
  return tdvc_launch_status("tdvc_add_flow");
}

extern "C" int tdvc_bcast_add_act(const tdvc_fmap* x, const tdvc_fmap* b, int T, float slope, void* stream) {
  TDVC_CHECK(x && b && fmap_ok16(*x) && fmap_ok16(*b) && same_geom(*x, *b) && x->C == T * b->C, "tdvc_bcast_add_act: bad arguments");
  const long total = (long)x->N * x->H * x->W * (x->C / 8);
  if (T == 4 && total / 4 < (1L << 31)) {
    const long items = total / 4;
    hipLaunchKernelGGL(bcast_add_act_t_kernel<4>, grid1d(items), dim3(256), 0, ST(stream), to_dev(*x), to_dev(*b), slope, (unsigned)items,
                       (unsigned)(b->C / 8), (unsigned)((long)x->H * x->W));
    return tdvc_launch_status("tdvc_bcast_add_act");
  }
  hipLaunchKernelGGL(bcast_add_act_kernel, grid1d(total), dim3(EW_BLOCK), 0, ST(stream), to_dev(*x), to_dev(*b), slope);
  return tdvc_launch_status("tdvc_bcast_add_act");
}

extern "C" int tdvc_channel_sum(const tdvc_fmap* x, float* partial, int nblocks, void* stream) {
  TDVC_CHECK(x && partial && fmap_any(*x) && (x->C % 8) == 0 && x->C <= 256 && nblocks >= 1 && nblocks <= 4096, "tdvc_channel_sum: bad arguments");
  hipLaunchKernelGGL(channel_sum_kernel, dim3(nblocks, x->N), dim3(256), 0, ST(stream), to_dev(*x), partial, nblocks);
  return tdvc_launch_status("tdvc_channel_sum");
}

extern "C" int tdvc_se_gate(const float* partial, int nblocks, float inv_count, int N, int C, int Cmid,
                            const float* w1, const float* b1, const float* w2, const float* b2, float* gate, void* stream) {
  TDVC_CHECK(partial && w1 && b1 && w2 && b2 && gate && C <= 256 && Cmid <= 32 && N >= 1, "tdvc_se_gate: bad arguments");
  hipLaunchKernelGGL(se_gate_kernel, dim3(N), dim3(1024), 0, ST(stream), partial, nblocks, inv_count, C, Cmid, w1, b1, w2, b2, gate);
  return tdvc_launch_status("tdvc_se_gate");
}

extern "C" int tdvc_upsample2x(const tdvc_fmap* x, const tdvc_fmap* y, void* stream) {
  TDVC_CHECK(x && y && fmap_ok16(*x) && fmap_ok16(*y) && y->H == 2 * x->H && y->W == 2 * x->W && y->C == x->C && y->N == x->N,
             "tdvc_upsample2x: bad arguments");
  const long total = (long)y->N * y->H * y->W * (y->C / 8);
  hipLaunchKernelGGL(upsample2x_kernel, grid1d(total), dim3(EW_BLOCK), 0, ST(stream), to_dev(*x), to_dev(*y));
  return tdvc_launch_status("tdvc_upsample2x");
}

extern "C" int tdvc_avgpool2(const tdvc_fmap* x, const tdvc_fmap* y, void* stream) {
  TDVC_CHECK(x && y && fmap_ok32(*x) && fmap_ok32(*y) && y->H == x->H / 2 && y->W == x->W / 2 && y->C <= x->C && y->N == x->N,
             "tdvc_avgpool2: bad arguments");
  const long total = (long)y->N * y->H * y->W;
  hipLaunchKernelGGL(avgpool2_kernel, grid1d(total), dim3(EW_BLOCK), 0, ST(stream), to_dev(*x), to_dev(*y));
  return tdvc_launch_status("tdvc_avgpool2");
}

extern "C" int tdvc_spynet_level_input(const tdvc_fmap* ref, const tdvc_fmap* supp, const tdvc_fmap* flow_lo,
                                       const tdvc_fmap* flow_up, const tdvc_fmap* cat8, void* stream) {
  TDVC_CHECK(ref && supp && flow_up && cat8, "tdvc_spynet_level_input: null");
  TDVC_CHECK(fmap_ok32(*ref) && fmap_ok32(*supp) && ref->C >= 3 && supp->C >= 3 && same_geom(*ref, *supp), "tdvc_spynet_level_input: bad ref/supp");
  TDVC_CHECK(fmap_ok32(*flow_up) && flow_up->C >= 2 && same_geom(*ref, *flow_up), "tdvc_spynet_level_input: bad flow_up");
  TDVC_CHECK(fmap_ok16(*cat8) && cat8->C == 8 && same_geom(*ref, *cat8), "tdvc_spynet_level_input: bad cat8");
  if (flow_lo) TDVC_CHECK(fmap_ok32(*flow_lo) && flow_lo->C >= 2 && flow_lo->N == ref->N && flow_lo->H * 2 == ref->H && flow_lo->W * 2 == ref->W,
                          "tdvc_spynet_level_input: bad flow_lo");
  const long total = (long)ref->N * ref->H * ref->W;
  auto pix16 = [](const tdvc_fmap& f) { return f.C >= 4 && (f.sp % 4) == 0 && (f.sn % 4) == 0 && aligned16(f.p); };
  auto pix8 = [](const tdvc_fmap& f) { return (f.sp % 2) == 0 && (f.sn % 2) == 0 && (((uintptr_t)f.p) & 7) == 0; };
  const bool vec = pix16(*ref) && pix16(*supp) && pix8(*flow_up) && (!flow_lo || pix8(*flow_lo));
  if (vec)
    hipLaunchKernelGGL(spynet_level_input_kernel<true>, grid1d(total), dim3(EW_BLOCK), 0, ST(stream), to_dev(*ref), to_dev(*supp),
                       flow_lo ? to_dev(*flow_lo) : null_fmap(), to_dev(*flow_up), to_dev(*cat8));
  else
    hipLaunchKernelGGL(spynet_level_input_kernel<false>, grid1d(total), dim3(EW_BLOCK), 0, ST(stream), to_dev(*ref), to_dev(*supp),
                       flow_lo ? to_dev(*flow_lo) : null_fmap(), to_dev(*flow_up), to_dev(*cat8));
  return tdvc_launch_status("tdvc_spynet_level_input");
}

extern "C" int tdvc_resize_bilinear(const tdvc_fmap* x, const tdvc_fmap* y, const float* chscale, void* stream) {
  TDVC_CHECK(x && y && fmap_ok32(*x) && fmap_ok32(*y) && y->C <= x->C && y->N == x->N, "tdvc_resize_bilinear: bad arguments");
  const long total = (long)y->N * y->H * y->W;
  hipLaunchKernelGGL(resize_bilinear_kernel, grid1d(total), dim3(EW_BLOCK), 0, ST(stream), to_dev(*x), to_dev(*y), chscale);
  return tdvc_launch_status("tdvc_resize_bilinear");
}

extern "C" int64_t tdvc_avgpool_k_work_floats(int N, int hp, int wp, int C_, int scale) {
  return (int64_t)N * hp * wp * ((scale + POOL_ROWS - 1) / POOL_ROWS) * C_;
}

extern "C" int tdvc_avgpool_k(const tdvc_fmap* x, int scale, float* pooled, int hp, int wp, float* work, int64_t work_floats, void* stream) {
  TDVC_CHECK(x && pooled && work && fmap_ok16(*x) && x->C <= 256 && scale >= 1 && hp == x->H / scale && wp == x->W / scale && hp >= 1 && wp >= 1,
             "tdvc_avgpool_k: bad arguments");
  const int nsplit = (scale + POOL_ROWS - 1) / POOL_ROWS;
  TDVC_CHECK(work_floats >= tdvc_avgpool_k_work_floats(x->N, hp, wp, x->C, scale), "tdvc_avgpool_k: workspace too small (tdvc_avgpool_k_work_floats)");
  const int* pred = tdvc_launch_predicate();
  hipLaunchKernelGGL(avgpool_k_strip_kernel, dim3(hp * wp * nsplit, x->N), dim3(256), 0, ST(stream), to_dev(*x), scale, work, wp, nsplit, pred);
  const long total = (long)x->N * hp * wp * x->C;
  hipLaunchKernelGGL(avgpool_k_final_kernel, grid1d(total), dim3(256), 0, ST(stream), work, pooled, total, x->C, nsplit, (float)scale * (float)scale, pred);
  return tdvc_launch_status("tdvc_avgpool_k");
}

extern "C" int tdvc_frame_changed(const tdvc_fmap* cur, tdvc_fmap* cache, int* flag, void* stream) {
  TDVC_CHECK(cur && cache && flag && fmap_ok16(*cur) && fmap_ok16(*cache) && same_geom(*cur, *cache) && cur->C == cache->C &&
             (reinterpret_cast<uintptr_t>(flag) & 3) == 0, "tdvc_frame_changed: fp16 maps of one geometry and a 4-byte aligned flag");
  const hipError_t err = hipMemsetAsync(flag, 0, sizeof(int), ST(stream));
  if (err != hipSuccess) { tdvc_set_error("tdvc_frame_changed: hipMemsetAsync failed: %s", hipGetErrorString(err)); return (int)err; }
  const long words = (long)cur->N * cur->H * cur->W * (cur->C / 8);
  hipLaunchKernelGGL(frame_compare_kernel, grid1d(words), dim3(EW_BLOCK), 0, ST(stream), to_dev(*cur), to_dev(*cache), words, flag);
// ... 69 lines not shown
```

tdvc_amd/model/modules.py:

```python
from __future__ import annotations

import torch
import torch.nn as nn

from .. import ops
from ..ops import ACT_LRELU, ACT_NONE, ACT_RELU, FM
from .ring import SlotRing


class PackCache:

    def _pk(self, key, fn):
        c = self.__dict__.setdefault("_packed", {})
        if key not in c:
            c[key] = fn()
        return c[key]


def _dev(m: nn.Module):
    return next(m.parameters()).device


def pk_conv(owner: PackCache, name: str, conv: nn.Module, **kw) -> ops.PackedConv:
    def build():
        w = conv.weight
        if w.dim() == 5:
            co, ci, kt, kh, kw_ = w.shape
            if kt == 1:
                return ops.pack_conv(w.view(co, ci, kh, kw_), conv.bias, stride=1, pad=conv.padding[-1], device=w.device,
                                     param_w=conv.weight, param_b=conv.bias, **kw)
            return ops.pack_conv(w, conv.bias, stride=1, pad=0, device=w.device,
                                 layout=ops.convpack.WeightLayout.conv3d_temporal(co, ci, kt), param_w=conv.weight, param_b=conv.bias, **kw)
        return ops.pack_conv(w, conv.bias, stride=conv.stride[0], pad=conv.padding[0], device=w.device, **kw)
    return owner._pk(name, build)


class ConvAct(nn.Module):

    def __init__(self, cin, cout, k, stride=1, padding=0):
        super().__init__()
        self.conv = nn.Conv2d(cin, cout, k, stride, padding, bias=True)


class SELayer(nn.Module, PackCache):

    def __init__(self, channels, ratio=16):
        super().__init__()
        self.channels = channels
        self.conv1 = ConvAct(channels, int(channels / ratio), 1)
        self.conv2 = ConvAct(int(channels / ratio), channels, 1)

    def params(self) -> ops.SEParams:
        def build():
            c, m = self.channels, self.conv1.conv.out_channels
            f = lambda t: t.detach().float().contiguous()
            return ops.SEParams(f(self.conv1.conv.weight.view(m, c)), f(self.conv1.conv.bias),
                                f(self.conv2.conv.weight.view(c, m)), f(self.conv2.conv.bias), c, m,
                                params=(self.conv1.conv.weight, self.conv1.conv.bias, self.conv2.conv.weight, self.conv2.conv.bias))
        return self._pk("se", build)

    def gate(self, x: FM, partial=None) -> torch.Tensor:
        return ops.se_gate(x, self.params(), partial=partial)

    def run(self, x: FM, out: FM | None = None, act=ACT_NONE, slope=0.0, res: FM | None = None, out2: FM | None = None, sums: list | None = None):
        out = FM.empty(x.N, x.H, x.W, x.C, dtype=x.t.dtype, device=x.t.device) if out is None else out
        return ops.scale_act_res(x, out, gate=self.gate(x, sums[0] if sums else None), act=act, slope=slope, res=res, out2=out2)


class Res_Block(nn.Module, PackCache):

    def __init__(self, channels=64):
        super().__init__()
        self.conv1 = nn.Conv2d(channels, channels, 3, 1, 1)
        self.conv2 = nn.Conv2d(channels, channels, 3, 1, 1)

    def run(self, x: FM, out: FM | None = None, res2: FM | None = None) -> FM:
        if self.conv1.in_channels == 64 and ops.conv_pair_supported(x, out, res2) and (out is None or out.desc().p != x.desc().p):
            pp = self._pk("pair", lambda: ops.pack_conv_pair(self.conv1.weight, self.conv1.bias, self.conv2.weight, self.conv2.bias))
            return ops.conv_pair(x, pp, out=out, act1=ACT_RELU, act2=ACT_NONE, add_input=True, res2=res2)
        t = ops.conv(x, pk_conv(self, "c1", self.conv1), act=ACT_RELU)
        return ops.conv(t, pk_conv(self, "c2", self.conv2), out=out, res=x, res2=res2)


def res_stack(n, ch=64):
    return nn.Sequential(*[Res_Block(ch) for _ in range(n)])


def run_stack(stack, x: FM, out: FM | None = None, res2: FM | None = None) -> FM:
    n = len(stack)
    for i, blk in enumerate(stack):
        last = i == n - 1
        x = blk.run(x, out=out if last else None, res2=res2 if last else None)
    return x


class SPyNetBasicModule(nn.Module):
    def __init__(self):
        super().__init__()
        ch = [8, 32, 64, 32, 16, 2]
        self.basic_module = nn.Sequential(*[ConvAct(ch[i], ch[i + 1], 7, 1, 3) for i in range(5)])


class SPyNet(nn.Module, PackCache):

    def __init__(self):
        super().__init__()
        self.basic_module = nn.ModuleList([SPyNetBasicModule() for _ in range(6)])
        self.register_buffer("mean", torch.tensor([0.485, 0.456, 0.406]).view(1, 3, 1, 1))
        self.register_buffer("std", torch.tensor([0.229, 0.224, 0.225]).view(1, 3, 1, 1))

    def compute_flow(self, ref: FM, supp: FM) -> FM:
        refs, supps = [ref], [supp]
        for _ in range(5):
            refs.append(ops.avgpool2(refs[-1]))
            supps.append(ops.avgpool2(supps[-1]))
        refs, supps = refs[::-1], supps[::-1]
        dev = ref.t.device
        flow = None
        for lvl in range(6):
            r, s = refs[lvl], supps[lvl]
            up = FM.empty(r.N, r.H, r.W, 2, dtype=torch.float32, device=dev)
            x = FM.empty(r.N, r.H, r.W, 8, device=dev)
            ops.spynet_level_input(r, s, flow, up, x)
            bm = self.basic_module[lvl].basic_module
            for i in range(4):
                x = ops.conv(x, pk_conv(self, f"l{lvl}c{i}", bm[i].conv), act=ACT_RELU)
            flow = ops.conv(x, pk_conv(self, f"l{lvl}c4", bm[4].conv), res=up, out_dtype=torch.float32)
        return flow

    def run(self, ref: FM, supp: FM) -> FM:
        H, W = ref.H, ref.W
        Hu = H if H % 32 == 0 else 32 * (H // 32 + 1)
        Wu = W if W % 32 == 0 else 32 * (W // 32 + 1)
        if (Hu, Wu) != (H, W):
            ref, supp = ops.resize_bilinear(ref, Hu, Wu), ops.resize_bilinear(supp, Hu, Wu)
        flow = self.compute_flow(ref, supp)
        if (Hu, Wu) != (H, W):
            sc = torch.tensor([float(W) / float(Wu), float(H) / float(Hu)], dtype=torch.float32, device=flow.t.device)
            flow = ops.resize_bilinear(flow, H, W, sc)
        return flow


class FeaExtra(nn.Module, PackCache):

    def __init__(self, num_block):
        super().__init__()
        self.conv_first = nn.Conv2d(3, 64, 3, 1, 1)
        self.residual_layer = res_stack(num_block)

    def run(self, img8: FM, out: FM) -> FM:
        x = ops.conv(img8, pk_conv(self, "first", self.conv_first), act=ACT_LRELU, slope=0.1)
        return run_stack(self.residual_layer, x, out=out)


class OffsetGen(nn.Module, PackCache):

    def __init__(self, nf=64):
        super().__init__()
        self.offset_conv11 = nn.ModuleDict()
        self.offset_conv11_1 = nn.ModuleDict()
        self.offset_conv12 = nn.ModuleDict()
        self.feat_fusion = nn.ModuleDict()
        for i in (3, 2, 1):
            lv = f"l{i}"
            self.offset_conv11[lv] = nn.Conv2d(nf * 2, nf, 3, 1, 1)
            self.offset_conv11_1[lv] = nn.Conv2d(nf, nf, 3, 1, 1)
            self.offset_conv12[lv] = nn.Conv2d(nf, nf, 3, 1, 1)
            if i < 3:
                self.feat_fusion[lv] = nn.Conv2d(nf * 2, nf, 1, 1, 0)
        self.upsample_conv = nn.Conv2d(nf, nf, 3, 1, 1)
        self.conv_l2_1 = nn.Conv2d(nf, nf, 3, 2, 1)
        self.conv_l2_2 = nn.Conv2d(nf, nf, 3, 1, 1)
        self.conv_l3_1 = nn.Conv2d(nf, nf, 3, 2, 1)
        self.conv_l3_2 = nn.Conv2d(nf, nf, 3, 1, 1)
        self.spynet = SPyNet()
        self.attn = SELayer(64)
        self.feat_fusion_ = nn.Conv2d(nf, nf, 3, 1, 1)

    def run(self, feats: FM, cur32: FM, ref32: FM) -> FM:
        B, H, W = feats.N, feats.H, feats.W
        dev = feats.t.device
        lr = dict(act=ACT_LRELU, slope=0.1)
        cat1 = feats.ch(0, 128)
        cat2 = FM.empty(B, H // 2, W // 2, 128, device=dev)
        cat3 = FM.empty(B, H // 4, W // 4, 128, device=dev)
        for k in (0, 1):
            t = ops.conv(cat1.ch(64 * k, 64), pk_conv(self, "l2_1", self.conv_l2_1), **lr)
            ops.conv(t, pk_conv(self, "l2_2", self.conv_l2_2), out=cat2.ch(64 * k, 64), **lr)
            t = ops.conv(cat2.ch(64 * k, 64), pk_conv(self, "l3_1", self.conv_l3_1), **lr)
            ops.conv(t, pk_conv(self, "l3_2", self.conv_l3_2), out=cat3.ch(64 * k, 64), **lr)
        cats = {1: cat1, 2: cat2, 3: cat3}
        up_o1 = None
        off = None
        for i in (3, 2, 1):
            lv = f"l{i}"
            c = cats[i]
            o1 = ops.conv(c, pk_conv(self, "c11" + lv, self.offset_conv11[lv]), **lr)
            if i == 3:
                if ops.conv_pair_supported(o1):
                    c1_, c2_ = self.offset_conv11_1[lv], self.offset_conv12[lv]
                    pp = self._pk("pair_l3", lambda: ops.pack_conv_pair(c1_.weight, c1_.bias, c2_.weight, c2_.bias))
                    off = ops.conv_pair(o1, pp, act1=ACT_LRELU, slope1=0.1, act2=ACT_LRELU, slope2=0.1, add_input=False)
                else:
                    o1 = ops.conv(o1, pk_conv(self, "c11_1" + lv, self.offset_conv11_1[lv]), **lr)
                    off = ops.conv(o1, pk_conv(self, "c12" + lv, self.offset_conv12[lv]), **lr)
            else:
                ops.conv(o1, pk_conv(self, "c11_1" + lv, self.offset_conv11_1[lv]), out=up_o1.ch(64, 64), **lr)
                off = ops.conv(up_o1, pk_conv(self, "ff" + lv, self.feat_fusion[lv]), **lr)
            if i > 1:
                up = ops.upsample2x(off)
                up_o1 = FM.empty(B, up.H, up.W, 128, device=dev)
                ops.conv(up, pk_conv(self, "upc", self.upsample_conv), out=up_o1.ch(0, 64))
        flow = self.spynet.run(cur32, ref32)
        if ops.TAPE is not None:
            off = ops.clone(off)
        ops.add_flow(off, flow)
        sums = []
        e = ops.conv(off, pk_conv(self, "ff_", self.feat_fusion_), chan_sum=sums)
        return self.attn.run(e, sums=sums)


class DCN(nn.Module, PackCache):

    def __init__(self, cin, cout, k, stride, padding, dilation=1, deformable_groups=1):
        super().__init__()
        assert k == 3 and stride == 1 and padding == 1 and dilation == 1
        self.deformable_groups = deformable_groups
        self.weight = nn.Parameter(torch.zeros(cout, cin, k, k))
        self.bias = nn.Parameter(torch.zeros(cout))
        self.conv_offset_mask = nn.Conv2d(cin, deformable_groups * 3 * k * k, k, stride, padding)

    def run(self, x: FM, y: FM, out: FM, act=ACT_NONE, slope=0.0) -> FM:
        om = ops.conv(y, pk_conv(self, "om", self.conv_offset_mask))
        pc = self._pk("w", lambda: ops.pack_conv(self.weight, self.bias, stride=1, pad=1, ck=8 * self.deformable_groups,
                                                 device=self.weight.device))
        return ops.dcn_fused(x, om, pc, out, groups=self.deformable_groups, act=act, slope=slope, round16=True)


class MCNet(nn.Module, PackCache):

    def __init__(self, num_block):
        super().__init__()
        self.dconv = DCN(64, 64, 3, stride=1, padding=1, deformable_groups=8)
        self.recon_layer = res_stack(num_block)
        self.feat_down = nn.Conv2d(64, 3, 3, 1, 1)
        self.conv = nn.Conv2d(128, 64, 3, 1, 1)

    def run(self, offset: FM, feats: FM, out: FM) -> FM:
        ref = feats.ch(64, 64)
        dcn_out = feats.ch(128, 64)
        self.dconv.run(ref, offset, dcn_out, act=ACT_LRELU, slope=0.1)
        perm = list(range(64, 128)) + list(range(0, 64))
        pc = self._pk("conv", lambda: ops.pack_conv(self.conv.weight, self.conv.bias, stride=1, pad=1, cin_perm=perm,
                                                    device=self.conv.weight.device))
        o2 = ops.conv(feats.ch(64, 128), pc, act=ACT_LRELU, slope=0.1)
        return run_stack(self.recon_layer, o2, out=out, res2=dcn_out)


class Bottleneck3D(nn.Module):
    def __init__(self):
        super().__init__()
        self.conv1 = nn.Conv3d(64, 64, (1, 3, 3), padding=(0, 1, 1))
        self.spatial_conv3d = nn.Conv3d(64, 64, (1, 3, 3), padding=(0, 1, 1))
        self.temporal_conv3d = nn.Conv3d(64, 64, (3, 1, 1), stride=(3, 1, 1), bias=False)
        self.conv3 = nn.Conv3d(64, 64, (1, 3, 3), padding=(0, 1, 1))


LOOPFILTER_PAIR = True
LOOPFILTER_BCAST = True
LOOPFILTER_REUSE = True
LOOPFILTER_RING = 9


class LoopFilterReuse:

    __slots__ = ("key", "ring", "A", "S", "F", "flags", "usable", "log")

    def __init__(self, key, slots):
        self.key, self.ring, self.usable, self.log = key, SlotRing(slots), None, []
        self.A = self.S = self.F = self.flags = None


class LoopFilter(nn.Module, PackCache):

    def __init__(self):
        super().__init__()
        self.conv01 = nn.Conv2d(3, 64, 3, 1, 1)
        self.conv02 = nn.Conv2d(64, 64, 3, 1, 1)
        self.conv1 = nn.Conv3d(64, 64, (1, 3, 3), padding=(0, 1, 1))
        self.layer1 = Bottleneck3D()
        self.attn = SELayer(64)
        self.feat_fusion = nn.Conv2d(256, 64, 1, 1)

    def _slices(self, name, conv, src: FM, dst: FM, res_buf: FM | None = None, **kw):
        pc = pk_conv(self, name, conv)
        for b in range(src.N):
            ops.conv(src.as_slices(b, 4, 64), pc, out=dst.as_slices(b, 4, 64),
                     res=res_buf.as_slices(b, 4, 64) if res_buf is not None else None, **kw)

    def run(self, xt: FM, refs8: FM, out: FM) -> FM:
        if (LOOPFILTER_REUSE and LOOPFILTER_PAIR and LOOPFILTER_BCAST and not self.training and ops.TAPE is None and ops.PROFILE is None
                and not xt.f32 and not refs8.f32 and xt.H * xt.W >= 8192 and ops.conv_pair_supported(xt.as_slices(0, 4, 64))):
            r = self._run_reuse(xt, refs8, out)
            if r is not None:
                return r
        return self._run_plain(xt, refs8, out)

    def reuse_state(self) -> LoopFilterReuse | None:
        return self.__dict__.get("_packed", {}).get("lf_reuse")

    def _run_reuse(self, xt: FM, refs8: FM, out: FM) -> FM | None:
        B, H, W = xt.N, xt.H, xt.W
        dev = xt.t.device
        key = (dev.index, ops._stream().value, B, H, W)
        cache = self.__dict__.setdefault("_packed", {})
        st = cache.get("lf_reuse")
        if st is None or st.key != key or st.ring.slots != LOOPFILTER_RING:
            st = cache["lf_reuse"] = LoopFilterReuse(key, LOOPFILTER_RING)
        if st.usable is False:
            return None
        try:
            return self._reuse_call(st, xt, refs8, out)
        except BaseException:
            cache.pop("lf_reuse", None)
            raise

    def _reuse_call(self, st: LoopFilterReuse, xt: FM, refs8: FM, out: FM) -> FM | None:
        B, H, W = xt.N, xt.H, xt.W
        dev = xt.t.device
        lr = dict(act=ACT_LRELU, slope=0.1)
        R = st.ring.slots
        if st.A is None:
            st.A, st.S = FM.empty(B, H, W, 64 * R, device=dev), FM.empty(B, H, W, 64 * R, device=dev)
            st.F = FM.empty(B * R, H, W, refs8.C, device=dev)
            st.flags = torch.ones((B, 4), dtype=torch.int32, device=dev)
            a3, a4, s4 = FM(st.A.t, st.A.off, 3, 64, 64), FM(st.A.t, st.A.off, 4, 64, 64), FM(st.S.t, st.S.off, 4, 64, 64)
            if not (ops.conv_pair_supported(a3) and ops.conv_pair_supported(a4, s4)):
                st.usable = False
                st.A = st.S = st.F = st.flags = None
                return None
        p, force = st.ring.begin()
        win = lambda buf, b, j0, n: FM(buf.t, buf.off + b * buf.sn + 64 * (p + j0), n, 64, 64)
        l1 = self.layer1
        p01, pc1 = pk_conv(self, "c01", self.conv01), pk_conv(self, "c1", self.conv1)
        pp_a = self._pk("pair_c02_c1", lambda: ops.pack_conv_pair(self.conv02.weight, self.conv02.bias,
                                                                   self.conv1.weight.view(64, 64, 3, 3), self.conv1.bias))
        pp_b = self._pk("pair_b1_bs", lambda: ops.pack_conv_pair(l1.conv1.weight.view(64, 64, 3, 3), l1.conv1.bias,
                                                                  l1.spatial_conv3d.weight.view(64, 64, 3, 3), l1.spatial_conv3d.bias))
        log = []
        for b in range(B):
            frames = refs8.batch(4 * b + 1, 3)
            ops.frames_changed(frames, st.F.batch(b * R + p, 3), st.flags[b, :3], force)
            with ops.predicate_images(st.flags[b, :3]) as lg:
                t = ops.conv(frames, p01, **lr)
                ops.conv_pair(t, pp_a, out=win(st.A, b, 0, 3), act1=ACT_NONE, act2=ACT_LRELU, slope2=0.1, add_input=False)
            log += lg
            ops.conv(xt.as_slices(b, 4, 64).batch(3, 1), pc1, out=win(st.A, b, 3, 1), **lr)
            with ops.predicate_images(st.flags[b, :4]) as lg:
                ops.conv_pair(win(st.A, b, 0, 4), pp_b, out=win(st.S, b, 0, 4), act1=ACT_LRELU, slope1=0.1, act2=ACT_NONE, add_input=False)
            log += lg
        st.log = list(log)
        if not all(log):
            st.usable = False
            st.A = st.S = st.F = st.flags = None
            return None
        st.usable = True
        st.ring.commit()
        s = FM.empty(B, H, W, 256, device=dev)
        ops.conv(st.S.ch(64 * p, 192), pk_conv(self, "bt", l1.temporal_conv3d), out=s.ch(0, 64), bcast_T=4, bcast_slope=0.1,
                 res=st.S.ch(64 * p, 64))
        o = FM.empty(B, H, W, 256, device=dev)
        pc3 = pk_conv(self, "b3", l1.conv3)
        for b in range(B):
            ops.conv(s.as_slices(b, 4, 64), pc3, out=o.as_slices(b, 4, 64), res=win(st.A, b, 0, 4))
        sums = []
        f = ops.conv(o, pk_conv(self, "ff", self.feat_fusion), chan_sum=sums, **lr)
        return self.attn.run(f, out=out, res=xt.ch(192, 64), sums=sums)

    def _run_plain(self, xt: FM, refs8: FM, out: FM) -> FM:
        B, H, W = xt.N, xt.H, xt.W
        dev = xt.t.device
        lr = dict(act=ACT_LRELU, slope=0.1)
        p01, p02 = pk_conv(self, "c01", self.conv01), pk_conv(self, "c02", self.conv02)
        a = FM.empty(B, H, W, 256, device=dev)
        fuse = LOOPFILTER_PAIR and ops.conv_pair_supported(a.as_slices(0, 4, 64).batch(0, 3))
        if fuse:
            pp = self._pk("pair_c02_c1", lambda: ops.pack_conv_pair(self.conv02.weight, self.conv02.bias,
                                                                     self.conv1.weight.view(64, 64, 3, 3), self.conv1.bias))
            pc1 = pk_conv(self, "c1", self.conv1)
        for b in range(B):
            t = ops.conv(refs8.batch(4 * b + 1, 3), p01, **lr)
            if fuse:
                ops.conv_pair(t, pp, out=a.as_slices(b, 4, 64).batch(0, 3), act1=ACT_NONE, act2=ACT_LRELU, slope2=0.1, add_input=False)
                ops.conv(xt.as_slices(b, 4, 64).batch(3, 1), pc1, out=a.as_slices(b, 4, 64).batch(3, 1), **lr)
            else:
                ops.conv(t, p02, out=xt.as_slices(b, 4, 64).batch(0, 3))
        if not fuse:
            self._slices("c1", self.conv1, xt, a, **lr)
        l1 = self.layer1
        bf = FM.empty(B, H, W, 256, device=dev)
        s = FM.empty(B, H, W, 256, device=dev)
        if LOOPFILTER_PAIR and ops.conv_pair_supported(a.as_slices(0, 4, 64), s.as_slices(0, 4, 64)):
            pp = self._pk("pair_b1_bs", lambda: ops.pack_conv_pair(l1.conv1.weight.view(64, 64, 3, 3), l1.conv1.bias,
                                                                    l1.spatial_conv3d.weight.view(64, 64, 3, 3), l1.spatial_conv3d.bias))
            for b in range(B):
                ops.conv_pair(a.as_slices(b, 4, 64), pp, out=s.as_slices(b, 4, 64), act1=ACT_LRELU, slope1=0.1, act2=ACT_NONE,
                              add_input=False)
        else:
            self._slices("b1", l1.conv1, a, bf, **lr)
            self._slices("bs", l1.spatial_conv3d, bf, s)
        if ops.TAPE is None and LOOPFILTER_BCAST and H * W >= 8192:
            ops.conv(s.ch(0, 192), pk_conv(self, "bt", l1.temporal_conv3d), out=s.ch(0, 64), bcast_T=4, bcast_slope=0.1)
        else:
            tm = ops.conv(s.ch(0, 192), pk_conv(self, "bt", l1.temporal_conv3d))
            if ops.TAPE is not None:
                s = ops.clone(s)
            ops.bcast_add_act(s, tm, 4, 0.1)
        o = bf if ops.TAPE is None else FM.empty(B, H, W, 256, device=dev)
        self._slices("b3", l1.conv3, s, o, res_buf=a)
        sums = []
        f = ops.conv(o, pk_conv(self, "ff", self.feat_fusion), chan_sum=sums, **lr)
        return self.attn.run(f, out=out, res=xt.ch(192, 64), sums=sums)


class FeatureExtract(nn.Module, PackCache):

    def __init__(self, cin, mid, nblocks):
        super().__init__()
        self.conv_first = nn.Conv2d(cin, mid, 3, 1, 1)
        self.body = res_stack(nblocks, mid)
        self.conv_last = nn.Conv2d(mid, mid, 3, 1, 1)

    def run(self, x: FM, out: FM | None = None) -> FM:
        x1 = ops.conv(x, pk_conv(self, "first", self.conv_first), act=ACT_LRELU, slope=0.01)
        t = run_stack(self.body, x1)
        return ops.conv(t, pk_conv(self, "last", self.conv_last), out=out, res=x1)


FEATUREFIX_REUSE = True


class IFrameReuse:

    __slots__ = ("key", "y", "iframe", "pref", "flag", "usable", "log")

    def __init__(self, key):
        self.key, self.usable, self.log = key, None, []
        self.y = self.iframe = self.pref = self.flag = None


class FeatureFix(nn.Module, PackCache):

    def __init__(self):
        super().__init__()
        self.FeatureExtract_input = FeatureExtract(64, 64, 2)
        self.FeatureExtract_ref = FeatureExtract(3, 64, 2)
        self.recon_layer = res_stack(2)
        self.conv_10 = nn.Conv2d(64, 64, 3, 2, 1)
        self.conv_11 = nn.Conv2d(64, 64, 3, 1, 1)
        self.conv_12 = nn.Conv2d(64, 64, 3, 2, 1)
        self.conv_13 = nn.Conv2d(64, 64, 3, 1, 1)
        self.featfusion = nn.Conv2d(128, 64, 3, 1, 1)
        self.featfusion2 = nn.Conv2d(128, 64, 3, 1, 1)
        self.featdown = nn.Conv2d(64, 3, 3, 1, 1)
        self.attn = SELayer(64)

    def run(self, x: FM, iframe8: FM, training: bool, trace=None) -> torch.Tensor:
        B, H, W = x.N, x.H, x.W
        dev = x.t.device
        lr = dict(act=ACT_LRELU, slope=0.1)
        fin = self.FeatureExtract_input.run(x)
        scale = 8 if training else int(H / 8)
        if FEATUREFIX_REUSE and not training and ops.TAPE is None and ops.PROFILE is None and trace is None and not iframe8.f32:
            y, pref = self._iframe_features(iframe8, scale)
            fref = y.ch(64, 64)
        else:
            y = FM.empty(B, H, W, 128, device=dev)
            fref = self.FeatureExtract_ref.run(iframe8, out=y.ch(64, 64))
            pref = ops.avgpool_k(fref, scale)
        pin = ops.avgpool_k(fin, scale)
        idx = ops.patch_match(pin, pref)
        cat = FM.empty(B, H, W, 128, device=dev)
        ops.match_gather(fin, fref, idx, scale, cat)
        ops.conv(cat, pk_conv(self, "ff", self.featfusion), out=y.ch(0, 64), **lr)
        sums = []
        o2 = ops.conv(y, pk_conv(self, "ff2", self.featfusion2), chan_sum=sums)
        o2 = self.attn.run(o2, sums=sums, **lr)
        o = run_stack(self.recon_layer, o2, res2=x)
        rgb = torch.empty((B, 3, H, W), dtype=torch.float32, device=dev)
        ops.conv(o, pk_conv(self, "down", self.featdown), act=ops.ACT_CLAMP01, nchw_out=rgb)
        if trace is not None:
            trace.update(ff_idx=idx, ff_fin=fin, ff_fref=fref)
        return rgb

    def reuse_state(self) -> IFrameReuse | None:
        return self.__dict__.get("_packed", {}).get("iframe_reuse")

    def _iframe_features(self, iframe8: FM, scale: int):
        B, H, W = iframe8.N, iframe8.H, iframe8.W
        dev = iframe8.t.device
        key = (dev.index, ops._stream().value, B, H, W, scale)
        cache = self.__dict__.setdefault("_packed", {})
        st = cache.get("iframe_reuse")
        if st is None or st.key != key:
            st = cache["iframe_reuse"] = IFrameReuse(key)

        def chain(y, pref):
            fref = self.FeatureExtract_ref.run(iframe8, out=y.ch(64, 64))
            ops.avgpool_k(fref, scale, out=pref)

        def fresh():
            return (FM.empty(B, H, W, 128, device=dev),
                    torch.empty((B, H // scale, W // scale, 64), dtype=torch.float32, device=dev))

        if st.usable is False:
            y, pref = fresh()
            chain(y, pref)
            return y, pref
        if st.usable is None:
            st.y, st.pref = fresh()
            st.iframe = FM.empty(B, H, W, iframe8.C, device=dev)
            st.flag = torch.ones(1, dtype=torch.int32, device=dev)
            ops.copy_cast(iframe8, st.iframe)
        else:
            ops.frame_changed(iframe8, st.iframe, st.flag)
        with ops.predicate(st.flag) as log:
            chain(st.y, st.pref)
        st.log = list(log)
        y, pref = st.y, st.pref
        if not all(log):
            if st.usable is not None:
                chain(y, pref)
            st.usable = False
            st.y = st.iframe = st.pref = st.flag = None
        else:
            st.usable = True
        return y, pref
```

tdvc_amd/model/pnet.py:

```python
from __future__ import annotations

import torch
import torch.nn as nn

from .. import ops
from ..ops import FM
from .coder import MVCoder, ResCoder
from .modules import FeaExtra, FeatureFix, LoopFilter, MCNet, OffsetGen


def _ref_views(refs8: FM, B: int):
    return (FM(refs8.t, refs8.off + 3 * refs8.sn, B, refs8.C, 4 * refs8.sn), FM(refs8.t, refs8.off, B, refs8.C, 4 * refs8.sn))


class VideoCompressor(nn.Module):
    fp32_islands_supported = True

    def __init__(self):
        super().__init__()
        self.coder_fp32 = False
        self.train_coder_fp32 = False
        self.stream_order = "raster"
        self.stream_lanes = 64
        self.mvCoder = MVCoder(N=128)
        self.resCoder = ResCoder(N=128)
        self.extra_fea = FeaExtra(2)
        self.motion_est = OffsetGen()
        self.mcnet = MCNet(3)
        self.loopfilter = FeatureFix()
        self.mcfilter = LoopFilter()

    def clear_packed(self):
        for m in self.modules():
            m.__dict__.pop("_packed", None)
            m.__dict__.pop("_tables", None)
            m.__dict__.pop("_ar_cache", None)

    def load_state_dict(self, *a, **kw):
        r = super().load_state_dict(*a, **kw)
        self.clear_packed()
        return r

    def _apply(self, fn, *a, **kw):
        self.clear_packed()
        return super()._apply(fn, *a, **kw)

    def forward(self, input_image, refer_frames, enabled_amp=True, is_compress=False, trace=None, noise=None):
        noise = noise or {}
        if not (input_image.is_cuda and refer_frames.is_cuda):
            raise RuntimeError("tdvc_amd.VideoCompressor runs on a HIP device only (no CPU fallback)")
        f32 = (not enabled_amp) or self.coder_fp32
        if self.training and self.train_coder_fp32:
            f32 = True
        elif f32 and self.training:
            if not self.__dict__.get("_warned_fp32_train"):
                import warnings
                warnings.warn("tdvc_amd: the fp32-island coders are an inference / coding mode; training runs the default "
                              "fp16-in / fp32-accumulate coders (enabled_amp=False ignored in .train())")
                self.__dict__["_warned_fp32_train"] = True
            f32 = False
        training = self.training
        B, _, H, W = input_image.shape
        if H % 64 or W % 64:
            raise RuntimeError(f"input must be padded to a multiple of 64 (got {H}x{W}); see tools/predict.py:51-53")
        dev = input_image.device
        with torch.cuda.device(dev), torch.no_grad():
            x = input_image.float()
            refs = refer_frames.float().reshape(B * 4, 3, H, W)
            cur32 = ops.from_nchw(x, Cpad=4, dtype=torch.float32)
            cur8 = ops.from_nchw(x, Cpad=8)
            refs8 = ops.from_nchw(refs, Cpad=8)
            last = refer_frames[:, 3].float()
            ref32 = ops.from_nchw(last, Cpad=4, dtype=torch.float32)
            ref8, iframe8 = _ref_views(refs8, B)
            if ops.TAPE is not None:
                for t in (cur32, cur8, refs8, ref32, ref8, iframe8):
                    ops.TAPE.mark_input(t)

            feats = FM.empty(B, H, W, 192, device=dev)
            npx_ = float(B * H * W)
            f_cur = self.extra_fea.run(cur8, feats.ch(0, 64))
            self.extra_fea.run(ref8, feats.ch(64, 64))
            estmv = self.motion_est.run(feats, cur32, ref32)

            tr_mv = {} if trace is not None else None
            mv_hat, mv_bits = self.mvCoder.run(estmv, training=training, trace=tr_mv, noise=noise.get("mv"), f32=f32)
            coded = {}
            if is_compress:
                self.mvCoder.update(force=True)
                coded["mv"] = self.mvCoder.compress(estmv, f32=f32)

            xt = FM.empty(B, H, W, 256, device=dev)
            pred1 = self.mcnet.run(mv_hat, feats, xt.ch(192, 64))
            pred = FM.empty(B, H, W, 64, device=dev)
            self.mcfilter.run(xt, refs8, pred)
            resid = ops.scale_act_res(f_cur, FM.empty(B, H, W, 64, device=dev), res=pred, res_sign=-1.0)

            tr_res = {} if trace is not None else None
            recon_f, res_bits = self.resCoder.run(resid, training=training, res=pred, trace=tr_res, noise=noise.get("res"), f32=f32)
            if is_compress:
                self.resCoder.update(force=True)
                coded["res"] = self.resCoder.compress(resid, f32=f32)
                self.last_strings = {k: v["strings"] for k, v in coded.items()}
                self.last_ac_bpp = {k: sum(len(s[0]) for s in v["strings"]) * 8.0 / npx_ for k, v in coded.items()}

            recon = self.loopfilter.run(recon_f, iframe8, training=training, trace=trace)

            npx = float(B * H * W)
            bpp_mv = (mv_bits.sum() / npx).float().view(-1)
            bpp_res = (res_bits.sum() / npx).float().view(-1)
            if trace is not None:
                trace.update(f_cur=f_cur, f_ref=feats.ch(64, 64), estmv=estmv, mv_x_hat=mv_hat, pred1=pred1, pred=pred,
                             resid=resid, recon_f=recon_f, mv=tr_mv, res=tr_res)
        if training:
            return recon, bpp_res, bpp_mv, self.mvCoder.aux_loss(), self.resCoder.aux_loss()
        return recon, bpp_res, bpp_mv

    def _prepare(self, refer_frames, input_image=None):
        B, _, _, H, W = refer_frames.shape
        if H % 64 or W % 64:
            raise RuntimeError(f"frames must be padded to a multiple of 64 (got {H}x{W})")
        dev = refer_frames.device
        refs8 = ops.from_nchw(refer_frames.float().reshape(B * 4, 3, H, W), Cpad=8)
        last = refer_frames[:, 3].float()
        ref8, iframe8 = _ref_views(refs8, B)
        feats = FM.empty(B, H, W, 192, device=dev)
        self.extra_fea.run(ref8, feats.ch(64, 64))
        return B, H, W, dev, refs8, last, iframe8, feats

    def _reconstruct(self, mv_y_hat: FM, res_y_hat_fn, feats: FM, refs8: FM, iframe8: FM):
        B, H, W, dev = feats.N, feats.H, feats.W, feats.t.device
        mv_hat = self.mvCoder.run_g_s(mv_y_hat)
        xt = FM.empty(B, H, W, 256, device=dev)
        self.mcnet.run(mv_hat, feats, xt.ch(192, 64))
        pred = FM.empty(B, H, W, 64, device=dev)
        self.mcfilter.run(xt, refs8, pred)
        recon_f = self.resCoder.run_g_s(res_y_hat_fn(pred), res=pred)
        return self.loopfilter.run(recon_f, iframe8, training=False)

    @torch.no_grad()
    def encode(self, input_image, refer_frames):
        assert not self.training
        if refer_frames.shape[0] > 1:
            return self._encode_batch(input_image, refer_frames)
        B, H, W, dev, refs8, last, iframe8, feats = self._prepare(refer_frames)
        x = input_image.float()
        f_cur = self.extra_fea.run(ops.from_nchw(x, Cpad=8), feats.ch(0, 64))
        estmv = self.motion_est.run(feats, ops.from_nchw(x, Cpad=4, dtype=torch.float32), ops.from_nchw(last, Cpad=4, dtype=torch.float32))
        self.mvCoder.update()
# ... 79 lines not shown
```

tdvc_amd/ops.py:

```python
from __future__ import annotations

import ctypes as C
from dataclasses import dataclass

import numpy as np
import torch

from . import _lib as L
from . import convpack
from ._lib import (ACT_CLAMP01, ACT_LRELU, ACT_NONE, ACT_RELU, GDN_FWD, GDN_INV, GDN_NONE, OUT_NCHW_F32,
                   OUT_NHWC, OUT_SHUFFLE2)


_raw_stream = torch._C._cuda_getCurrentRawStream
_cur_dev = torch._C._cuda_getDevice
FORCE_STREAM = None
FORCE_KEEP = None


def _stream():
    if FORCE_STREAM is not None:
        return C.c_void_p(FORCE_STREAM)
    return C.c_void_p(_raw_stream(_cur_dev()))

# ... 398 lines not shown
        out_dtype = torch.float32 if x.f32 else torch.float16
    if pc.s2d and (x.f32 or x.N * (x.H // 2) * (x.W // 2) <= SMALL_MAP_PIXELS):
        pc = _plain_form(pc)
    if pc.s2d:
        if x.H % 2 or x.W % 2:
            raise L.TdvcHipError("conv: the space-to-depth stride-2 path needs even H, W")
        Ho, Wo = x.H // 2, x.W // 2
    else:
        Ho = (x.H + 2 * pc.pad - pc.kh) // pc.stride + 1
        Wo = (x.W + 2 * pc.pad - pc.kw) // pc.stride + 1
    wt = pc.packed_f32() if x.f32 else pc.w
    key = "_tmpl32" if x.f32 else "_tmpl16"
    tm = pc.__dict__.get(key)
    if tm is None or tm[1] != wt.data_ptr():
        t_ = L.ConvDesc()
        t_.w = wt.data_ptr()
        t_.bias = pc.bias.data_ptr()
        t_.cout, t_.ntaps = pc.cout, len(pc.taps)
        for i, (dy, dx) in enumerate(pc.taps):
            t_.tap_dy[i], t_.tap_dx[i] = dy, dx
        t_.kh, t_.kw, t_.stride, t_.pad, t_.ck = pc.kh, pc.kw, pc.stride, pc.pad, pc.ck
        t_.s2d = int(pc.s2d)
        tm = pc.__dict__[key] = (t_, wt.data_ptr())
    d = L.ConvDesc.from_buffer_copy(tm[0])
    d.x = x.desc()
    d.square_input, d.gdn = int(square), gdn
    d.aux = aux.desc() if aux is not None else _NULL_FM
    d.act, d.slope, d.round_before_act = act, slope, int(round16)
    d.res = res.desc() if res is not None else _NULL_FM
    d.res2 = res2.desc() if res2 is not None else _NULL_FM
    d.bcast_T, d.bcast_slope = int(bcast_T), float(bcast_slope)
    if nchw_out is not None:
        assert nchw_out.shape == (x.N, pc.cout, Ho, Wo) and nchw_out.dtype == torch.float32 and nchw_out.is_contiguous()
        d.out_mode = OUT_NCHW_F32
        d.y = L.FMapDesc(nchw_out.data_ptr(), x.N, Ho, Wo, pc.cout, pc.cout * Ho * Wo, 1, L.F32)
        ret = nchw_out
    else:
        if pc.shuffle:
            d.out_mode = OUT_SHUFFLE2
            if out is None:
                out = FM.empty(x.N, 2 * Ho, 2 * Wo, pad8(pc.cout // 4), dtype=out_dtype, device=x.t.device)
        else:
            d.out_mode = OUT_NHWC
            if out is None:
                out = FM.empty(x.N, Ho, Wo, pc.cout if (out_dtype == torch.float32 and not x.f32) else pad8(pc.cout),
                               dtype=out_dtype, device=x.t.device)
        d.y = out.desc()
        ret = out
    return d, ret, Ho, Wo, pc, rec_pc


def conv(x: FM, pc: PackedConv, out: FM | None = None, act=ACT_NONE, slope=0.0, res: FM | None = None,
         res2: FM | None = None, gdn=GDN_NONE, aux: FM | None = None, square=False, out_dtype=None,
         round16=False, nchw_out: torch.Tensor | None = None, bcast_T=0, bcast_slope=0.0, chan_sum: list | None = None) -> FM | torch.Tensor:
    d, ret, Ho, Wo, pc, rec_pc = conv_desc(x, pc, out, act, slope, res, res2, gdn, aux, square, out_dtype, round16, nchw_out, bcast_T, bcast_slope)
    if chan_sum is not None and TAPE is None and FUSE_CHAN_SUM:
        rows = L.lib().tdvc_conv_chan_sum_rows(C.byref(d))
        if rows > 0:
            part = torch.empty((x.N, rows, pc.cout), dtype=torch.float32, device=x.t.device)
            d.chan_sum = part.data_ptr()
            chan_sum.append((part, rows))
    if bcast_T and TAPE is not None and not _IN_BACKWARD:
        raise L.TdvcHipError("conv: bcast_T is an inference-only fusion (under the tape use conv + bcast_add_act)")
    if PROFILE is not None:
        e0, e1 = torch.cuda.Event(enable_timing=True), torch.cuda.Event(enable_timing=True)
        e0.record()
        L.check(L.lib().tdvc_conv2d(C.byref(d), _stream()), "conv2d")
        e1.record()
        PROFILE.append(dict(kernel=L.lib().tdvc_last_conv_kernel().decode(),
                            shape=f"{pc.kh}x{pc.kw} s{pc.stride} {x.C}->{pc.cout} @{x.H}x{x.W}" + (" f32out" if out_dtype == torch.float32 else "") + (" nchw" if nchw_out is not None else ""),
                            e0=e0, e1=e1,
                            flops=2.0 * x.N * Ho * Wo * pc.cout * x.C * len(pc.taps),
                            flops_real=(x.N * Ho * Wo * pc.flops_per_px) if pc.s2d else 2.0 * x.N * Ho * Wo * pc.cout * pc.cin_real * len(pc.taps),
                            bytes=2.0 * x.N * (x.H * x.W * x.C + Ho * Wo * pc.cout * (4 if pc.shuffle else 1) / (4 if pc.shuffle else 1))))
        _rec("conv", x, rec_pc, None if nchw_out is not None else ret, act, slope, res, res2, gdn, aux, square, nchw_out)
        return ret
    L.check(L.lib().tdvc_conv2d(C.byref(d), _stream()), "conv2d")
    _log_predicated()
    _rec("conv", x, rec_pc, None if nchw_out is not None else ret, act, slope, res, res2, gdn, aux, square, nchw_out)
    return ret


class PackedConvPair:

    def __init__(self, w: torch.Tensor, bias: torch.Tensor):
        self.w, self.bias = w, bias


def pack_conv_pair(w1: torch.Tensor, b1: torch.Tensor | None, w2: torch.Tensor, b2: torch.Tensor | None) -> PackedConvPair:
    for w in (w1, w2):
        if tuple(w.shape) != (64, 64, 3, 3):
            raise L.TdvcHipError(f"pack_conv_pair: weights must be (64, 64, 3, 3), got {tuple(w.shape)}")
    frag = lambda w: w.detach().float().reshape(4, 16, 2, 4, 8, 9).permute(0, 5, 2, 3, 1, 4)
    w = torch.stack([frag(w1), frag(w2)]).contiguous().to(torch.float16)
    zb = lambda b_: torch.zeros(64, device=w1.device) if b_ is None else b_.detach().float()
    return PackedConvPair(w, torch.cat([zb(b1), zb(b2)]).contiguous())


def _pair_desc(x: FM, pp: PackedConvPair, out: FM, act1, slope1, act2, slope2, add_input, res2):
    d = L.ConvPairDesc()
    d.x, d.y = x.desc(), out.desc()
    d.w, d.bias = pp.w.data_ptr(), pp.bias.data_ptr()
    d.act1, d.slope1, d.act2, d.slope2 = act1, slope1, act2, slope2
    d.add_input = 1 if add_input else 0
    d.res2 = res2.desc() if res2 is not None else L.FMapDesc()
    return d


def conv_pair_supported(x: FM, out: FM | None = None, res2: FM | None = None) -> bool:
    if TAPE is not None or x.f32 or x.C != 64:
        return False
    d = L.ConvPairDesc()
    d.x = x.desc()
    d.y = out.desc() if out is not None else x.desc()
    d.res2 = res2.desc() if res2 is not None else L.FMapDesc()
    d.w = d.bias = 1
    return bool(L.lib().tdvc_conv_pair_supported(C.byref(d)))


def conv_pair(x: FM, pp: PackedConvPair, out: FM | None = None, act1=ACT_RELU, slope1=0.0, act2=ACT_NONE, slope2=0.0,
              add_input=True, res2: FM | None = None) -> FM:
    if TAPE is not None:
        raise L.TdvcHipError("conv_pair: inference only (the intermediate map is not kept for the backward pass)")
    if out is None:
        out = FM.empty(x.N, x.H, x.W, 64, device=x.t.device)
    d = _pair_desc(x, pp, out, act1, slope1, act2, slope2, add_input, res2)
    if PROFILE is not None:
        e0, e1 = torch.cuda.Event(enable_timing=True), torch.cuda.Event(enable_timing=True)
        e0.record()
        L.check(L.lib().tdvc_conv_pair(C.byref(d), _stream()), "conv_pair")
        e1.record()
        fl = 2 * 2.0 * x.N * x.H * x.W * 64 * 64 * 9
        PROFILE.append(dict(kernel="conv_pair", shape=f"2x(3x3 s1 64->64) @{x.H}x{x.W}", e0=e0, e1=e1, flops=fl, flops_real=fl,
# ... 255 lines not shown
def dcn_col2im(x: FM, om: FM, dcol: FM, groups: int, dom: FM) -> FM:
    dx32 = FM.zeros(x.N, x.H, x.W, x.C, dtype=torch.float32, device=x.t.device)
    lib = L.lib()
    nwork = lib.tdvc_dcn_col2im_work_floats(x.N, x.H, x.W, groups)
    work = torch.empty((nwork,), dtype=torch.float32, device=x.t.device)
    d1, d2, d3, d4 = x.desc(), om.desc(), dcol.desc(), dom.desc()
    if DETERMINISTIC:
        dev = x.t.device
        cap = max(1 << 16, x.N * x.H * x.W * groups * 36 // 8)
        keys = torch.empty((cap,), dtype=torch.int64, device=dev)
        vals = torch.empty((cap, 8), dtype=torch.float32, device=dev)
        cnt = torch.zeros((1,), dtype=torch.int32, device=dev)
        L.check(lib.tdvc_dcn_col2im_det(C.byref(d1), C.byref(d2), C.byref(d3), groups, dx32.t.data_ptr(), C.byref(d4), work.data_ptr(), nwork,
                                        keys.data_ptr(), vals.data_ptr(), cnt.data_ptr(), cap, _stream()), "dcn_col2im_det")
        n = int(cnt.item())
        if n > cap:
            raise L.TdvcHipError(f"dcn_col2im (deterministic): {n} far samples exceed the record capacity {cap}")
        if n:
            ks, order = torch.sort(keys[:n], stable=True)
            L.check(lib.tdvc_dcn_far_apply(ks.data_ptr(), order.data_ptr(), vals.data_ptr(), n, dx32.t.data_ptr(), _stream()), "dcn_far_apply")
        return dx32
    L.check(lib.tdvc_dcn_col2im(C.byref(d1), C.byref(d2), C.byref(d3), groups, dx32.t.data_ptr(), C.byref(d4), work.data_ptr(), nwork, _stream()),
            "dcn_col2im")
    return dx32


def dcn_column_conv(pc: PackedConv, groups: int) -> PackedConv:
    cp = pc.__dict__.get("_colpc")
    if cp is None:
        cin = 8 * groups
        chan = np.array([(g * 8 + j) * 9 + t for g in range(groups) for t in range(9) for j in range(8)], dtype=np.int64)
        lay = convpack.WeightLayout(pc.cout, 9 * cin, 1, 1, np.arange(pc.cout, dtype=np.int64) * cin * 9, chan, np.zeros(1, dtype=np.int64))
        cp = pack_conv(pc.wsrc, None, stride=1, pad=0, layout=lay, param_w=pc.param_w)
        pc.__dict__["_colpc"] = cp
    return cp


def sigmoid_f32(x: torch.Tensor) -> torch.Tensor:
    out = torch.empty_like(x)
    L.check(L.lib().tdvc_sigmoid_f32(x.data_ptr(), out.data_ptr(), x.numel(), _stream()), "sigmoid_f32")
    return out


def sigmoid_backward_f32(g: torch.Tensor, s: torch.Tensor) -> torch.Tensor:
    L.check(L.lib().tdvc_sigmoid_backward_f32(g.data_ptr(), s.data_ptr(), g.numel(), _stream()), "sigmoid_backward_f32")
    return g


def axpy_f32(dst: torch.Tensor, src: torch.Tensor, scale: float) -> None:
    assert dst.numel() == src.numel() and dst.dtype == src.dtype == torch.float32 and dst.is_contiguous() and src.is_contiguous()
    L.check(L.lib().tdvc_axpy_f32(dst.data_ptr(), src.data_ptr(), scale, dst.numel(), _stream()), "axpy_f32")


def scale_act_res(a: FM, out: FM, gate: torch.Tensor | None = None, act=ACT_NONE, slope=0.0, res: FM | None = None,
                  res_sign=1.0, out2: FM | None = None) -> FM:
    da, dy = a.desc(), out.desc()
    dr = res.desc() if res is not None else None
    d2 = out2.desc() if out2 is not None else None
    L.check(L.lib().tdvc_scale_act_res(C.byref(da), gate.data_ptr() if gate is not None else None, act, slope,
                                       C.byref(dr) if dr is not None else None, res_sign, C.byref(dy),
                                       C.byref(d2) if d2 is not None else None, _stream()), "scale_act_res")
    _rec("scale_act_res", a, out, gate, act, slope, res, res_sign, out2)
    return out


def clone(x: FM) -> FM:
    out = copy_cast(x, FM.empty(x.N, x.H, x.W, x.C, dtype=x.t.dtype, device=x.t.device))
    _rec("clone", x, out)
    return out


def add_flow(off: FM, flow: FM):
    do, df = off.desc(), flow.desc()
    L.check(L.lib().tdvc_add_flow(C.byref(do), C.byref(df), _stream()), "add_flow")
    _rec("add_flow", off, flow)


def bcast_add_act(x: FM, b: FM, T: int, slope: float):
    dx, db = x.desc(), b.desc()
    L.check(L.lib().tdvc_bcast_add_act(C.byref(dx), C.byref(db), T, slope, _stream()), "bcast_add_act")
    _rec("bcast_add_act", x, b, slope)


@dataclass
class SEParams:
    w1: torch.Tensor
    b1: torch.Tensor
    w2: torch.Tensor
    b2: torch.Tensor
    C: int
    Cmid: int
    params: tuple = ()


FUSE_CHAN_SUM = True


def se_gate(x: FM, p: SEParams, partial=None) -> torch.Tensor:
    npix = x.H * x.W
    gate = torch.empty((x.N, x.C), dtype=torch.float32, device=x.t.device)
    lib = L.lib()
    if partial is not None:
        partial, nblocks = partial
        assert tuple(partial.shape) == (x.N, nblocks, x.C) and partial.dtype == torch.float32
    else:
        nblocks = max(1, min(1024, npix // 256))
        partial = torch.empty((x.N, nblocks, x.C), dtype=torch.float32, device=x.t.device)
        dx = x.desc()
        L.check(lib.tdvc_channel_sum(C.byref(dx), partial.data_ptr(), nblocks, _stream()), "channel_sum")
    L.check(lib.tdvc_se_gate(partial.data_ptr(), nblocks, 1.0 / npix, x.N, p.C, p.Cmid, p.w1.data_ptr(),
                             p.b1.data_ptr(), p.w2.data_ptr(), p.b2.data_ptr(), gate.data_ptr(), _stream()), "se_gate")
    _rec("se_gate", x, p, partial, nblocks, gate)
    return gate


def upsample2x(x: FM, out: FM | None = None) -> FM:
    if out is None:
        out = FM.empty(x.N, 2 * x.H, 2 * x.W, x.C, device=x.t.device)
    dx, dy = x.desc(), out.desc()
    L.check(L.lib().tdvc_upsample2x(C.byref(dx), C.byref(dy), _stream()), "upsample2x")
    _rec("upsample2x", x, out)
    return out


def avgpool2(x: FM) -> FM:
    out = FM.empty(x.N, x.H // 2, x.W // 2, x.C, dtype=torch.float32, device=x.t.device)
    dx, dy = x.desc(), out.desc()
    L.check(L.lib().tdvc_avgpool2(C.byref(dx), C.byref(dy), _stream()), "avgpool2")
    return out


def spynet_level_input(ref: FM, supp: FM, flow_lo: FM | None, flow_up: FM, cat8: FM):
    dr, ds, du, dc = ref.desc(), supp.desc(), flow_up.desc(), cat8.desc()
    dl = flow_lo.desc() if flow_lo is not None else None
    L.check(L.lib().tdvc_spynet_level_input(C.byref(dr), C.byref(ds), C.byref(dl) if dl is not None else None,
                                            C.byref(du), C.byref(dc), _stream()), "spynet_level_input")
    _rec("spynet_level_input", supp, flow_lo, flow_up, cat8)


def spynet_level_input_backward(supp: FM, flow_up: FM, dcat8: FM, dflow_up: FM, dflow_lo: FM | None) -> None:
    d1, d2, d3, d4 = supp.desc(), flow_up.desc(), dcat8.desc(), dflow_up.desc()
    d5 = dflow_lo.desc() if dflow_lo is not None else None
    L.check(L.lib().tdvc_spynet_level_input_backward(C.byref(d1), C.byref(d2), C.byref(d3), C.byref(d4),
                                                     C.byref(d5) if d5 is not None else None, _stream()), "spynet_level_input_backward")


def resize_bilinear(x: FM, H: int, W: int, chscale: torch.Tensor | None = None) -> FM:
    out = FM.empty(x.N, H, W, x.C, dtype=torch.float32, device=x.t.device)
    dx, dy = x.desc(), out.desc()
    L.check(L.lib().tdvc_resize_bilinear(C.byref(dx), C.byref(dy), chscale.data_ptr() if chscale is not None else None,
                                         _stream()), "resize_bilinear")
    _rec("resize_bilinear", x, out, chscale)
    return out


def resize_bilinear_backward(dy: FM, dx: FM, chscale: torch.Tensor | None = None) -> None:
    d1, d2 = dy.desc(), dx.desc()
    L.check(L.lib().tdvc_resize_bilinear_backward(C.byref(d1), C.byref(d2), chscale.data_ptr() if chscale is not None else None, _stream()),
            "resize_bilinear_backward")


def avgpool_k(x: FM, scale: int, out: torch.Tensor | None = None) -> torch.Tensor:
    hp, wp = x.H // scale, x.W // scale
    pooled = torch.empty((x.N, hp, wp, x.C), dtype=torch.float32, device=x.t.device) if out is None else out
    assert pooled.shape == (x.N, hp, wp, x.C) and pooled.dtype == torch.float32 and pooled.is_contiguous()
    nwork = L.lib().tdvc_avgpool_k_work_floats(x.N, hp, wp, x.C, scale)
    work = torch.empty((nwork,), dtype=torch.float32, device=x.t.device)
    dx = x.desc()
    L.check(L.lib().tdvc_avgpool_k(C.byref(dx), scale, pooled.data_ptr(), hp, wp, work.data_ptr(), nwork, _stream()), "avgpool_k")
    _log_predicated(2)
    return pooled


def patch_match(pin: torch.Tensor, pref: torch.Tensor) -> torch.Tensor:
    N, hp, wp, Cc = pin.shape
    Lp = ((hp + 3) // 3 + 1) * ((wp + 3) // 3 + 1)
    idx = torch.empty((N, Lp), dtype=torch.int32, device=pin.device)
    L.check(L.lib().tdvc_patch_match(pin.data_ptr(), pref.data_ptr(), N, hp, wp, Cc, idx.data_ptr(), _stream()),
            "patch_match")
    return idx


# ... 356 lines not shown
```

Measured before the change: 51.38 frames/s.

## Fuse flow-add into conv epilogue, add RGB head kernel, pyramid pool, resid fusion

Adds several inference-only fusions. Flow addition moves into the v5 conv epilogue. A dedicated 3x3 64->≤4 channel NCHW fp32 head kernel uses MFMA with double-buffered tile prefetch. A single-launch five-level avgpool pyramid is added for SpyNet inputs. A three-way scale_act_res lets the loop filter output and the residual subtraction be written in one pass. Together these aim to cut kernel launches and intermediate memory round-trips, at the cost of more code paths and fallbacks that depend on supported shapes.

```diff
diff --git a/include/tdvc_hip.h b/include/tdvc_hip.h
--- a/include/tdvc_hip.h
+++ b/include/tdvc_hip.h
@@ -50,6 +50,7 @@
   int32_t bcast_T;
   float bcast_slope;
   float* chan_sum;
+  tdvc_fmap flow;
 } tdvc_conv_desc;
 
 int tdvc_abi_version(void);
@@ -71,6 +72,7 @@
                            int ntaps, const int8_t* tap_dy, const int8_t* tap_dx, int ck, uint16_t* dst);
 int tdvc_conv2d(const tdvc_conv_desc* d, void* stream);
 int tdvc_conv_chan_sum_rows(const tdvc_conv_desc* d);
+int tdvc_conv_flow_supported(const tdvc_conv_desc* d);
 const char* tdvc_conv_select(const tdvc_conv_desc* d);
 int tdvc_conv2d_f32(const tdvc_conv_desc* d, void* stream);
 
@@ -115,6 +117,8 @@
 int tdvc_fmap_to_nchw(const tdvc_fmap* x, int C, float* dst, void* stream);
 int tdvc_scale_act_res(const tdvc_fmap* a, const float* gate, int act, float slope,
                        const tdvc_fmap* r, float r_sign, const tdvc_fmap* y, const tdvc_fmap* y2, void* stream);
+int tdvc_scale_act_res3(const tdvc_fmap* a, const float* gate, int act, float slope, const tdvc_fmap* r, float r_sign,
+                        const tdvc_fmap* y, const tdvc_fmap* b, float b_sign, const tdvc_fmap* y3, void* stream);
 int tdvc_add_flow(const tdvc_fmap* off, const tdvc_fmap* flow, void* stream);
 int tdvc_bcast_add_act(const tdvc_fmap* x, const tdvc_fmap* b, int T, float slope, void* stream);
 
@@ -125,6 +129,7 @@
 
 int tdvc_upsample2x(const tdvc_fmap* x, const tdvc_fmap* y, void* stream);
 int tdvc_avgpool2(const tdvc_fmap* x, const tdvc_fmap* y, void* stream);
+int tdvc_avgpool2_pyramid(const tdvc_fmap* xa, const tdvc_fmap* xb, const tdvc_fmap* ya, const tdvc_fmap* yb, void* stream);
 int tdvc_spynet_level_input(const tdvc_fmap* ref, const tdvc_fmap* supp, const tdvc_fmap* flow_lo,
                             const tdvc_fmap* flow_up, const tdvc_fmap* cat8, void* stream);
 int tdvc_resize_bilinear(const tdvc_fmap* x, const tdvc_fmap* y, const float* chscale, void* stream);
diff --git a/tdvc_amd/_lib.py b/tdvc_amd/_lib.py
--- a/tdvc_amd/_lib.py
+++ b/tdvc_amd/_lib.py
@@ -26,7 +26,7 @@
                 ("ck", C.c_int32), ("square_input", C.c_int32), ("gdn", C.c_int32),
                 ("aux", FMapDesc), ("act", C.c_int32), ("slope", C.c_float),
                 ("round_before_act", C.c_int32), ("res", FMapDesc), ("res2", FMapDesc), ("out_mode", C.c_int32), ("s2d", C.c_int32),
-                ("bcast_T", C.c_int32), ("bcast_slope", C.c_float), ("chan_sum", C.c_void_p)]
+                ("bcast_T", C.c_int32), ("bcast_slope", C.c_float), ("chan_sum", C.c_void_p), ("flow", FMapDesc)]
 
 
 class DcnDesc(C.Structure):
@@ -54,6 +54,9 @@
     "tdvc_abi_version": (_i, []),
     "tdvc_conv_chan_sum_rows": (_i, [C.POINTER(ConvDesc)]),
     "tdvc_conv_select": (C.c_char_p, [C.POINTER(ConvDesc)]),
+    "tdvc_conv_flow_supported": (_i, [C.POINTER(ConvDesc)]),
+    "tdvc_scale_act_res3": (_i, [_FM, _P, _i, _f, _FM, _f, _FM, _FM, _f, _FM, _P]),
+    "tdvc_avgpool2_pyramid": (_i, [_FM, _FM, _FM, _FM, _P]),
     "tdvc_last_error": (C.c_char_p, []),
     "tdvc_last_conv_kernel": (C.c_char_p, []),
     "tdvc_prepare_device": (_i, []),
diff --git a/tdvc_amd/csrc/conv_common.h b/tdvc_amd/csrc/conv_common.h
--- a/tdvc_amd/csrc/conv_common.h
+++ b/tdvc_amd/csrc/conv_common.h
@@ -20,9 +20,10 @@
   float* csum;
   int8_t tap_dy[TDVC_MAX_TAPS], tap_dx[TDVC_MAX_TAPS];
   const int* pred;
+  FMap flow;
 };
 
-enum ConvSwitch { SW_NONE = -1, SW_V2, SW_V3, SW_V5, SW_V7, SW_V9, SW_V10, SW_V11, SW_ROW, SW_C8, SW_N16, SW_GDN128, SW_COUNT };
+enum ConvSwitch { SW_NONE = -1, SW_V2, SW_V3, SW_V5, SW_V7, SW_V9, SW_V10, SW_V11, SW_ROW, SW_C8, SW_N16, SW_GDN128, SW_HEAD3, SW_COUNT };
 int conv_on(int id);
 long conv_v9_work_limit();
 
@@ -278,7 +279,7 @@
   }
 }
 
-template <int NTX, bool BIAS_IN_ACC, bool BCAST = false, bool CSUM = false>
+template <int NTX, bool BIAS_IN_ACC, bool BCAST = false, bool CSUM = false, bool FLOW = false>
 __device__ __forceinline__ void epilogue_lean_seq(const ConvParams& p, f32x16 (&acc)[2][NTX], const float* bias64, unsigned char* ew, int n,
                                                   int cbase, int oy_first, int ox_first, int lane, bool zero_acc, bool full, float* cs = nullptr) {
   constexpr int EPS = 144;
@@ -321,6 +322,16 @@
 #pragma unroll
       for (int k = 0; k < 4; ++k) r2[k] = *reinterpret_cast<const half8*>(rb2 + (long)opix[k] * p.res2.sp);
     }
+    float fx[4], fy[4];
+    if constexpr (FLOW) {
+      const float* fb = reinterpret_cast<const float*>(p.flow.p) + (long)n * p.flow.sn;
+#pragma unroll
+      for (int k = 0; k < 4; ++k) {
+        const float* fp = fb + (long)opix[k] * p.flow.sp;
+        fx[k] = fp[0];
+        fy[k] = fp[1];
+      }
+    }
 #pragma unroll
     for (int mt = 0; mt < 2; ++mt)
 #pragma unroll
@@ -372,6 +383,14 @@
       half8 v = *reinterpret_cast<const half8*>(ew + (k * 8 + prow) * EPS + chunk * 16);
       if (has1) v = v + r1[k];
       if (has2) v = v + r2[k];
+      if constexpr (FLOW) {
+#pragma unroll
+        for (int j = 0; j < 8; ++j) {
+          float s = (float)v[j];
+          s += (j & 1) ? fy[k] : fx[k];
+          v[j] = (half_t)s;
+        }
+      }
       if (ok[k]) *reinterpret_cast<half8*>(yb + (long)opix[k] * p.y.sp) = v;
       if constexpr (CSUM) {
 #pragma unroll
diff --git a/tdvc_amd/csrc/conv_dispatch.hip b/tdvc_amd/csrc/conv_dispatch.hip
--- a/tdvc_amd/csrc/conv_dispatch.hip
+++ b/tdvc_amd/csrc/conv_dispatch.hip
@@ -21,8 +21,8 @@
 
 namespace {
 const char* const kSwitchEnv[convk::SW_COUNT] = {nullptr, "TDVC_CONV_NO_V3", "TDVC_CONV_NO_V5", "TDVC_CONV_NO_V7", "TDVC_CONV_NO_V9", "TDVC_CONV_NO_V10",
-                                                 "TDVC_CONV_NO_V11", "TDVC_CONV_NO_ROW", "TDVC_CONV_NO_C8", "TDVC_CONV_NO_N16", "TDVC_CONV_NO_GDN128"};
-int g_enabled[convk::SW_COUNT] = {1, 1, 1, 1, 1, 1, 1, 15, 1, 1, 1};
+                                                 "TDVC_CONV_NO_V11", "TDVC_CONV_NO_ROW", "TDVC_CONV_NO_C8", "TDVC_CONV_NO_N16", "TDVC_CONV_NO_GDN128", "TDVC_CONV_NO_HEAD3"};
+int g_enabled[convk::SW_COUNT] = {1, 1, 1, 1, 1, 1, 1, 15, 1, 1, 1, 1};
 long g_v9_work_limit = 1L << 20;
 }
 
@@ -45,6 +45,7 @@
 extern "C" void tdvc_debug_enable_conv_c8(int enable) { g_enabled[convk::SW_C8] = enable != 0; }
 extern "C" void tdvc_debug_enable_conv_n16(int enable) { g_enabled[convk::SW_N16] = enable != 0; }
 extern "C" void tdvc_debug_enable_gdn128(int enable) { g_enabled[convk::SW_GDN128] = enable != 0; }
+extern "C" void tdvc_debug_enable_conv_head3(int enable) { g_enabled[convk::SW_HEAD3] = enable != 0; }
 extern "C" void tdvc_debug_set_conv_v9_work_limit(long v) { g_v9_work_limit = v; }
 
 namespace {
@@ -225,25 +226,41 @@
   return g_walk_mode == 1 ? (int)(g_walk_parity++ & 1u) : 0;
 }
 
-int conv2d_impl(const tdvc_conv_desc* d, void* stream, bool query_rows) {
+bool conv_flow_ok(const tdvc_conv_desc* d, const Entry* e, const ConvParams& p) {
+  return e && e->name == kNameV5 && p.simple == 2 && !d->chan_sum;
+}
+bool flow_map_ok(const tdvc_conv_desc* d, int Ho, int Wo) {
+  return fmap_ok32(d->flow) && d->flow.C >= 2 && d->flow.N == d->x.N && d->flow.H == Ho && d->flow.W == Wo;
+}
+constexpr char kFlowMsg[] = "tdvc_conv2d: flow on a conv whose kernel does not add it (tdvc_conv_flow_supported() == 0), with chan_sum, or not an fp32 map of >= 2 channels and the output's geometry";
+
+enum Query { LAUNCH = 0, QUERY_ROWS = 1, QUERY_FLOW = 2 };
+int conv2d_impl(const tdvc_conv_desc* d, void* stream, int query) {
+  const bool query_rows = query == QUERY_ROWS;
   TDVC_CHECK(d, "tdvc_conv2d: null descriptor");
   if (d->x.dtype == TDVC_F32) {
-    if (query_rows) return 0;
+    if (query != LAUNCH) return 0;
     TDVC_CHECK(!d->chan_sum, "tdvc_conv2d: chan_sum is not available on the fp32 path (tdvc_conv_chan_sum_rows() == 0)");
+    TDVC_CHECK(!d->flow.p, "tdvc_conv2d: flow is not available on the fp32 path (tdvc_conv_flow_supported() == 0)");
     snprintf(g_last_kernel, sizeof(g_last_kernel), "conv_f32");
     return tdvc_conv2d_f32(d, stream);
   }
   ConvParams p;
   Pick k = {d, 0, 0, -1};
   if (const int rc = prepare(d, p, k.Ho, k.Wo)) return rc;
-  p.reverse = query_rows ? 0 : next_walk_reverse();
+  p.reverse = query != LAUNCH ? 0 : next_walk_reverse();
   const Entry* e = select(k, p);
   const bool csum_ok = e && e->name == kNameV5 && k.cout_blocks() == 1 && p.simple == 2;
   if (query_rows) return csum_ok ? conv_v5_chan_sum_rows(k.Ho, k.Wo, 1, k.N()) : 0;
+  if (query == QUERY_FLOW) return conv_flow_ok(d, e, p) && (!d->flow.p || flow_map_ok(d, k.Ho, k.Wo)) ? 1 : 0;
   TDVC_CHECK(!d->chan_sum || (csum_ok && (reinterpret_cast<uintptr_t>(d->chan_sum) & 15) == 0),
              "tdvc_conv2d: chan_sum on a conv whose kernel has no fused channel sum (tdvc_conv_chan_sum_rows() == 0) or unaligned");
   p.csum = d->chan_sum;
   if (!e) return TDVC_EINVAL;
+  if (d->flow.p) {
+    TDVC_CHECK(conv_flow_ok(d, e, p) && flow_map_ok(d, k.Ho, k.Wo), "%s", kFlowMsg);
+    p.flow = to_dev(d->flow);
+  }
   kernel_name(e, k, g_last_kernel);
   return e->launch(k, p, reinterpret_cast<hipStream_t>(stream));
 }
@@ -251,8 +268,9 @@
 }
 
 extern "C" void tdvc_debug_set_conv_walk(int mode) { g_walk_mode = mode; }
-extern "C" int tdvc_conv2d(const tdvc_conv_desc* d, void* stream) { return conv2d_impl(d, stream, false); }
-extern "C" int tdvc_conv_chan_sum_rows(const tdvc_conv_desc* d) { return conv2d_impl(d, nullptr, true); }
+extern "C" int tdvc_conv2d(const tdvc_conv_desc* d, void* stream) { return conv2d_impl(d, stream, LAUNCH); }
+extern "C" int tdvc_conv_chan_sum_rows(const tdvc_conv_desc* d) { return conv2d_impl(d, nullptr, QUERY_ROWS); }
+extern "C" int tdvc_conv_flow_supported(const tdvc_conv_desc* d) { return conv2d_impl(d, nullptr, QUERY_FLOW); }
 extern "C" const char* tdvc_last_conv_kernel(void) { return g_last_kernel; }
 
 extern "C" const char* tdvc_conv_select(const tdvc_conv_desc* d) {
@@ -260,6 +278,7 @@
   if (!d) { tdvc_set_error("tdvc_conv_select: null descriptor"); return nullptr; }
   if (d->x.dtype == TDVC_F32) {
     int Ho, Wo;
+    if (d->flow.p) { tdvc_set_error("%s", kFlowMsg); return nullptr; }
     return conv_f32_validate(d, Ho, Wo) == TDVC_OK ? "conv_f32" : nullptr;
   }
   ConvParams p;
@@ -267,6 +286,7 @@
   if (prepare(d, p, k.Ho, k.Wo) != TDVC_OK) return nullptr;
   const Entry* e = select(k, p);
   if (!e) return nullptr;
+  if (d->flow.p && !(conv_flow_ok(d, e, p) && flow_map_ok(d, k.Ho, k.Wo))) { tdvc_set_error("%s", kFlowMsg); return nullptr; }
   kernel_name(e, k, name);
   return name;
 }
diff --git a/tdvc_amd/csrc/conv_head3.hip b/tdvc_amd/csrc/conv_head3.hip
--- /dev/null
+++ b/tdvc_amd/csrc/conv_head3.hip
@@ -0,0 +1,150 @@
+#include "conv_common.h"
+
+using convk::ConvParams;
+
+namespace {
+
+typedef unsigned u32x4 __attribute__((ext_vector_type(4)));
+
+constexpr int H3_TH = 8, H3_TW = 64, H3_NTHR = 512;
+constexpr int H3_CIN = 64, H3_KS = 18;
+constexpr int H3_TIW = H3_TW + 2, H3_TIH = H3_TH + 2;
+constexpr int H3_PS = 2 * H3_CIN + 16;
+constexpr int H3_ITEMS = H3_TIH * H3_TIW * (H3_CIN / 8);
+constexpr int H3_PER_THR = (H3_ITEMS + H3_NTHR - 1) / H3_NTHR;
+constexpr int H3_A_BYTES = H3_KS * 1024;
+constexpr int H3_LDS = H3_A_BYTES + H3_TIH * H3_TIW * H3_PS;
+
+struct Head3Extra {
+  int ntiles, tiles_x, tiles_per_img;
+};
+
+__global__ __launch_bounds__(H3_NTHR, 1) void conv_head3_kernel(const ConvParams p, const Head3Extra e) {
+  extern __shared__ __attribute__((aligned(16))) unsigned char smem[];
+  unsigned char* wl = smem;
+  unsigned char* tile = wl + H3_A_BYTES;
+  const int tid = threadIdx.x, lane = tid & 63;
+  const int wave = __builtin_amdgcn_readfirstlane(tid >> 6);
+  const int px = lane & 15, kg = lane >> 4;
+
+  for (int i = tid; i < H3_KS * 64; i += H3_NTHR) {
+    const int ln = i & 63, S = i >> 6;
+    const int q = 4 * S + (ln >> 4), s = q >> 1, h = q & 1;
+    half8 v = {0, 0, 0, 0, 0, 0, 0, 0};
+    if (s < p.steps) v = *reinterpret_cast<const half8*>(p.w + ((long)s * 64 + (ln & 15) + 32 * h) * 8);
+    *reinterpret_cast<half8*>(wl + (long)i * 16) = v;
+  }
+
+  u32x4 treg[H3_PER_THR];
+  unsigned okmask = 0u;
+  auto issue = [&](int tile_i) {
+    const int n = tile_i / e.tiles_per_img, rem = tile_i - n * e.tiles_per_img;
+    const int ty = rem / e.tiles_x, tx = rem - ty * e.tiles_x;
+    const half_t* xn = p.x + (long)n * p.x_sn;
+    const int iy0 = ty * H3_TH - 1, ix0 = tx * H3_TW - 1;
+    unsigned m = 0u;
+#pragma unroll
+    for (int u = 0; u < H3_PER_THR; ++u) {
+      const int idx = tid + u * H3_NTHR;
+      const int pix = idx >> 3, c8 = idx & 7;
+      const int rr = pix / H3_TIW, cc = pix - rr * H3_TIW;
+      const int iy = iy0 + rr, ix = ix0 + cc;
+      const bool ok = (int)(idx < H3_ITEMS) & (int)(iy >= 0) & (int)(iy < p.H) & (int)(ix >= 0) & (int)(ix < p.W);
+      const half_t* src = xn + ((long)(ok ? iy : 0) * p.W + (ok ? ix : 0)) * p.x_sp + c8 * 8;
+      treg[u] = *reinterpret_cast<const u32x4*>(src);
+      m |= (ok ? 1u : 0u) << u;
+    }
+    okmask = m;
+  };
+  auto publish = [&]() {
+#pragma unroll
+    for (int u = 0; u < H3_PER_THR; ++u) {
+      const int idx = tid + u * H3_NTHR;
+      const int pix = idx >> 3, c8 = idx & 7;
+      const u32x4 z = {0u, 0u, 0u, 0u};
+      const u32x4 val = ((okmask >> u) & 1u) ? treg[u] : z;
+      if (idx < H3_ITEMS) *reinterpret_cast<u32x4*>(tile + pix * H3_PS + c8 * 16) = val;
+    }
+  };
+
+  const int base = (wave * H3_TIW + px) * H3_PS;
+  constexpr int cstep = 16 * H3_PS;
+  auto frag_off = [&](int S) {
+    const int tap = S >> 1;
+    const int dy = tap / 3, dx = tap - dy * 3;
+    return base + (dy * H3_TIW + dx) * H3_PS + (32 * (S & 1) + 8 * kg) * 2;
+  };
+
+  f32x4 b4 = {0.f, 0.f, 0.f, 0.f};
+  if (p.bias) b4 = *reinterpret_cast<const f32x4*>(p.bias);
+
+  int tile_i = blockIdx.x;
+  if (tile_i < e.ntiles) issue(tile_i);
+  for (; tile_i < e.ntiles; tile_i += gridDim.x) {
+    const int n = tile_i / e.tiles_per_img, rem = tile_i - n * e.tiles_per_img;
+    const int ty = rem / e.tiles_x, tx = rem - ty * e.tiles_x;
+    publish();
+    __syncthreads();
+    if (tile_i + (int)gridDim.x < e.ntiles) issue(tile_i + gridDim.x);
+
+    f32x4 acc[4];
+#pragma unroll
+    for (int c = 0; c < 4; ++c) acc[c] = f32x4{0.f, 0.f, 0.f, 0.f};
+    half8 a0, b0[4], a1, b1[4];
+    auto load = [&](int S, half8& a, half8 (&b)[4]) {
+      const int off = frag_off(S);
+      a = *reinterpret_cast<const half8*>(wl + (S * 64 + lane) * 16);
+#pragma unroll
+      for (int c = 0; c < 4; ++c) b[c] = *reinterpret_cast<const half8*>(tile + off + c * cstep);
+    };
+    auto mm = [&](const half8& a, half8 (&b)[4]) {
+#pragma unroll
+      for (int c = 0; c < 4; ++c) acc[c] = __builtin_amdgcn_mfma_f32_16x16x32_f16(a, b[c], acc[c], 0, 0, 0);
+    };
+    load(0, a0, b0);
+#pragma unroll 1
+    for (int S = 0; S < H3_KS; S += 2) {
+      load(S + 1, a1, b1);
+      mm(a0, b0);
+      load(min(S + 2, H3_KS - 1), a0, b0);
+      mm(a1, b1);
+    }
+
+    const int oy = ty * H3_TH + wave;
+    const int ox = tx * H3_TW + lane;
+    const bool st_ok = oy < p.Ho && ox < p.Wo;
+    float* yrow = reinterpret_cast<float*>(p.y.p) + ((long)n * p.cout * p.Ho + oy) * p.Wo + ox;
+#pragma unroll
+    for (int ch = 0; ch < 4; ++ch) {
+      if (ch < p.cout) {
+        float mine = 0.f;
+#pragma unroll
+        for (int c = 0; c < 4; ++c) {
+          float v = acc[c][ch];
+          if (p.bias) v += b4[ch];
+          if (p.act) v = act_apply(v, p.act, p.slope);
+          const float got = __shfl(v, px);
+          if (kg == c) mine = got;
+        }
+        if (st_ok) yrow[(long)ch * p.Ho * p.Wo] = mine;
+      }
+    }
+    __syncthreads();
+  }
+}
+
+}
+
+bool conv_head3_takes(const ConvParams& p) {
+  return p.kh == 3 && p.kw == 3 && p.pad == 1 && p.ntaps == 9 && p.in_stride == 1 && p.Cin == H3_CIN && p.steps == 2 * H3_KS && p.cout >= 1 &&
+         p.cout <= 4 && p.out_mode == TDVC_OUT_NCHW_F32 && !p.res.p && !p.res2.p && !p.round16 && !p.gdn && !p.square && !p.s2d;
+}
+
+int launch_conv_head3(const ConvParams& p, int N, hipStream_t st) {
+  Head3Extra e;
+  e.tiles_x = (p.Wo + H3_TW - 1) / H3_TW;
+  e.tiles_per_img = e.tiles_x * ((p.Ho + H3_TH - 1) / H3_TH);
+  e.ntiles = N * e.tiles_per_img;
+  const int grid = e.ntiles < 256 ? e.ntiles : 256;
+  return convk::launch_big_lds<&conv_head3_kernel, ConvParams, Head3Extra>("tdvc_conv2d(head3)", 160 * 1024, dim3(grid), dim3(H3_NTHR), H3_LDS, st, p, e);
+}
diff --git a/tdvc_amd/csrc/conv_mfma_v5.hip b/tdvc_amd/csrc/conv_mfma_v5.hip
--- a/tdvc_amd/csrc/conv_mfma_v5.hip
+++ b/tdvc_amd/csrc/conv_mfma_v5.hip
@@ -143,6 +143,8 @@
       const int oy0 = ty * (WR * NWAVE) + wave * WR;
       if constexpr (SIMPLE == 4) {
         convk::epilogue_lean_seq<WR, false, true>(p, acc, bias_s, tbuf, n, cb * 64, oy0, tx * TW5, lane, true, false);
+      } else if constexpr (SIMPLE == 5) {
+        convk::epilogue_lean_seq<WR, false, false, false, true>(p, acc, bias_s, tbuf, n, cb * 64, oy0, tx * TW5, lane, true, false);
       } else if constexpr (SIMPLE) {
         if (SIMPLE == 2 && p.csum) convk::epilogue_lean_seq<WR, false, false, true>(p, acc, bias_s, tbuf, n, cb * 64, oy0, tx * TW5, lane, true, false, cs);
         else convk::epilogue_simple_rows<WR, false, SIMPLE>(p, acc, bias_s, tbuf, n, cb * 64, oy0, tx * TW5, lane, true);
@@ -195,7 +197,8 @@
 
 template <int TL>
 int launch_tl(const ConvParams& q, const V5Extra& e, int mode, dim3 grid, int lds, hipStream_t st) {
-  const auto go = mode == 4 ? convk::launch_big_lds<&conv_mfma_v5_kernel<4, TL>, ConvParams, V5Extra>
+  const auto go = mode == 5 ? convk::launch_big_lds<&conv_mfma_v5_kernel<5, TL>, ConvParams, V5Extra>
+                  : mode == 4 ? convk::launch_big_lds<&conv_mfma_v5_kernel<4, TL>, ConvParams, V5Extra>
                   : mode == 2 ? convk::launch_big_lds<&conv_mfma_v5_kernel<2, TL>, ConvParams, V5Extra>
                   : mode == 1 ? convk::launch_big_lds<&conv_mfma_v5_kernel<1, TL>, ConvParams, V5Extra>
                               : convk::launch_big_lds<&conv_mfma_v5_kernel<0, TL>, ConvParams, V5Extra>;
@@ -231,7 +234,12 @@
   if (simple) q.slope = convk::conv_simple_slope(p);
   dim3 grid(v5_grid_x(e.nbtiles, cout_blocks, N), cout_blocks, N);
   const int tl = v5_tl(p.kh, p.kw);
-  if (tl == 4) return launch_tl<4>(q, e, p.bcast_T ? 4 : (simple ? (convk::conv_is_lean(p) ? 2 : 1) : 0), grid, lds, st);
+  const bool lean = simple && convk::conv_is_lean(p);
+  if (p.flow.p && !(lean && !p.bcast_T && !p.csum)) {
+    tdvc_set_error("conv v5: flow needs the lean epilogue without channel sums");
+    return TDVC_EINVAL;
+  }
+  if (tl == 4) return launch_tl<4>(q, e, p.bcast_T ? 4 : (p.flow.p ? 5 : (simple ? (lean ? 2 : 1) : 0)), grid, lds, st);
   tdvc_set_error("conv v5: unsupported window %dx%d", p.kh, p.kw);
   return TDVC_EINVAL;
 }
diff --git a/tdvc_amd/csrc/conv_n16.hip b/tdvc_amd/csrc/conv_n16.hip
--- a/tdvc_amd/csrc/conv_n16.hip
+++ b/tdvc_amd/csrc/conv_n16.hip
@@ -139,7 +139,14 @@
          n16_lds(cin, d->kh, d->kw, d->ntaps, d->cout <= 16 ? 1 : 2) <= 150 * 1024;
 }
 
+bool conv_head3_takes(const ConvParams& p);
+int launch_conv_head3(const ConvParams& p, int N, hipStream_t st);
+static thread_local int g_n16_last_form = 0;
+extern "C" int tdvc_debug_conv_n16_last_form(void) { return g_n16_last_form; }
+
 int launch_conv_n16(const ConvParams& p, int N, hipStream_t st) {
+  g_n16_last_form = convk::conv_on(convk::SW_HEAD3) && conv_head3_takes(p);
+  if (g_n16_last_form) return launch_conv_head3(p, N, st);
   const int ncb = p.cout <= 16 ? 1 : 2;
   N16Extra e;
   e.ksteps = n16_ksteps(p.ntaps, p.Cin);
diff --git a/tdvc_amd/csrc/lib.cpp b/tdvc_amd/csrc/lib.cpp
--- a/tdvc_amd/csrc/lib.cpp
+++ b/tdvc_amd/csrc/lib.cpp
@@ -15,7 +15,7 @@
   va_end(ap);
 }
 
-extern "C" int tdvc_abi_version(void) { return 10; }
+extern "C" int tdvc_abi_version(void) { return 11; }
 extern "C" const char* tdvc_last_error(void) { return g_err; }
 
 static thread_local const int* g_pred = nullptr;
diff --git a/tdvc_amd/csrc/pointwise.hip b/tdvc_amd/csrc/pointwise.hip
--- a/tdvc_amd/csrc/pointwise.hip
+++ b/tdvc_amd/csrc/pointwise.hip
@@ -61,12 +61,13 @@
   if (y2.p) store8(y2, n, pix, c, v);
 }
 
-template <int U>
-__global__ __launch_bounds__(256) void scale_act_res16_kernel(FMap a, const float* gate, int act, float slope, FMap r, float rs, FMap y, FMap y2,
-                                                              unsigned total, unsigned chunks, unsigned npix) {
+template <int U, bool Y3>
+__device__ __forceinline__ void scale_act_res16_body(const FMap& a, const float* gate, int act, float slope, const FMap& r, float rs, const FMap& y,
+                                                     const FMap& y2, const FMap& b, float rs3, const FMap& y3, unsigned total, unsigned chunks,
+                                                     unsigned npix) {
   const unsigned T = gridDim.x * 256u;
   for (unsigned base = blockIdx.x * 256u + threadIdx.x; base < total; base += U * T) {
-    half8 av[U], rv[U];
+    half8 av[U], rv[U], bv[U];
     unsigned ck[U], nn[U];
     long pa[U];
     bool ok[U];
@@ -81,6 +82,7 @@
       pa[u] = (long)(pp - nn[u] * npix);
       av[u] = *reinterpret_cast<const half8*>(reinterpret_cast<const half_t*>(a.p) + (long)nn[u] * a.sn + pa[u] * a.sp + ck[u] * 8);
       if (r.p) rv[u] = *reinterpret_cast<const half8*>(reinterpret_cast<const half_t*>(r.p) + (long)nn[u] * r.sn + pa[u] * r.sp + ck[u] * 8);
+      if constexpr (Y3) bv[u] = *reinterpret_cast<const half8*>(reinterpret_cast<const half_t*>(b.p) + (long)nn[u] * b.sn + pa[u] * b.sp + ck[u] * 8);
     }
 #pragma unroll
     for (int u = 0; u < U; ++u) {
@@ -108,8 +110,31 @@
         *reinterpret_cast<half8*>(reinterpret_cast<half_t*>(y.p) + (long)nn[u] * y.sn + pa[u] * y.sp + ck[u] * 8) = h;
         if (y2.p) *reinterpret_cast<half8*>(reinterpret_cast<half_t*>(y2.p) + (long)nn[u] * y2.sn + pa[u] * y2.sp + ck[u] * 8) = h;
       }
-    }
-  }
+      if constexpr (Y3) {
+        half8 h3;
+#pragma unroll
+        for (int j = 0; j < 8; ++j) {
+          float w = (float)bv[u][j];
+          w += rs3 * (float)h[j];
+          h3[j] = (half_t)w;
+        }
+        if (ok[u]) *reinterpret_cast<half8*>(reinterpret_cast<half_t*>(y3.p) + (long)nn[u] * y3.sn + pa[u] * y3.sp + ck[u] * 8) = h3;
+      }
+    }
+  }
+}
+
+template <int U>
+__global__ __launch_bounds__(256) void scale_act_res16_kernel(FMap a, const float* gate, int act, float slope, FMap r, float rs, FMap y, FMap y2,
+                                                              unsigned total, unsigned chunks, unsigned npix) {
+  scale_act_res16_body<U, false>(a, gate, act, slope, r, rs, y, y2, a, 0.f, a, total, chunks, npix);
+}
+
+template <int U>
+__global__ __launch_bounds__(256) void scale_act_res16_y3_kernel(FMap a, const float* gate, int act, float slope, FMap r, float rs, FMap y, FMap b,
+                                                                 float rs3, FMap y3, unsigned total, unsigned chunks, unsigned npix) {
+  const FMap none = {};
+  scale_act_res16_body<U, true>(a, gate, act, slope, r, rs, y, none, b, rs3, y3, total, chunks, npix);
 }
 
 __global__ void add_flow_kernel(FMap off, FMap flow) {
@@ -289,6 +314,53 @@
   const long p00 = ((long)(2 * oy) * x.W + 2 * ox) * x.sp, p10 = p00 + (long)x.W * x.sp;
   for (int c = 0; c < y.C; ++c)
     yp[c] = (xp[p00 + c] + xp[p00 + x.sp + c] + xp[p10 + c] + xp[p10 + x.sp + c]) * 0.25f;
+}
+
+struct PyramidMaps { FMap x[2]; FMap y[2][5]; };
+template <bool VEC>
+__global__ __launch_bounds__(256) void avgpool2_pyramid_kernel(const PyramidMaps a) {
+  __shared__ __attribute__((aligned(16))) float lv[2][16 * 16 * 4];
+  const int m = blockIdx.z & 1, n = blockIdx.z >> 1, tid = threadIdx.x;
+  const int C = a.y[0][0].C;
+  float v[4] = {0.f, 0.f, 0.f, 0.f};
+  {
+    const FMap x = m ? a.x[1] : a.x[0];
+    const int ly = tid >> 4, lx = tid & 15;
+    const int oy = blockIdx.y * 16 + ly, ox = blockIdx.x * 16 + lx;
+    const float* xp = reinterpret_cast<const float*>(x.p) + (long)n * x.sn;
+    const long p00 = ((long)(2 * oy) * x.W + 2 * ox) * x.sp, p10 = p00 + (long)x.W * x.sp;
+    if constexpr (VEC) {
+      const f32x4 q00 = *reinterpret_cast<const f32x4*>(xp + p00), q01 = *reinterpret_cast<const f32x4*>(xp + p00 + x.sp);
+      const f32x4 q10 = *reinterpret_cast<const f32x4*>(xp + p10), q11 = *reinterpret_cast<const f32x4*>(xp + p10 + x.sp);
+#pragma unroll
+      for (int c = 0; c < 4; ++c) v[c] = (q00[c] + q01[c] + q10[c] + q11[c]) * 0.25f;
+    } else {
+      for (int c = 0; c < C; ++c) v[c] = (xp[p00 + c] + xp[p00 + x.sp + c] + xp[p10 + c] + xp[p10 + x.sp + c]) * 0.25f;
+    }
+  }
+  int S = 16;
+#pragma unroll
+  for (int k = 0; k < 5; ++k, S >>= 1) {
+    const int ly = tid / S, lx = tid - ly * S;
+    const bool mine = tid < S * S;
+    float* cur = lv[k & 1];
+    if (k > 0 && mine) {
+      const float* up = lv[(k - 1) & 1] + ((2 * ly) * (2 * S) + 2 * lx) * 4;
+#pragma unroll
+      for (int c = 0; c < 4; ++c) v[c] = (up[c] + up[4 + c] + up[2 * S * 4 + c] + up[2 * S * 4 + 4 + c]) * 0.25f;
+    }
+    if (mine) {
+      const FMap y = m ? a.y[1][k] : a.y[0][k];
+      float* yp = reinterpret_cast<float*>(y.p) + (long)n * y.sn + ((long)(blockIdx.y * S + ly) * y.W + blockIdx.x * S + lx) * y.sp;
+      if constexpr (VEC) {
+        *reinterpret_cast<f32x4*>(yp) = f32x4{v[0], v[1], v[2], v[3]};
+      } else {
+        for (int c = 0; c < C; ++c) yp[c] = v[c];
+      }
+      *reinterpret_cast<f32x4*>(cur + (ly * S + lx) * 4) = f32x4{v[0], v[1], v[2], v[3]};
+    }
+    if (k < 4) __syncthreads();
+  }
 }
 
 template <bool VEC>
@@ -728,6 +800,24 @@
   return tdvc_launch_status("tdvc_scale_act_res");
 }
 
+extern "C" int tdvc_scale_act_res3(const tdvc_fmap* a, const float* gate, int act, float slope, const tdvc_fmap* r, float r_sign,
+                                   const tdvc_fmap* y, const tdvc_fmap* b, float b_sign, const tdvc_fmap* y3, void* stream) {
+  TDVC_CHECK(a && y && b && y3 && fmap_ok16(*a) && fmap_ok16(*y) && same_geom(*a, *y) && y->C == a->C, "tdvc_scale_act_res3: a / y must be fp16 maps of one geometry");
+  if (r) TDVC_CHECK(fmap_ok16(*r) && same_geom(*a, *r) && r->C == a->C, "tdvc_scale_act_res3: bad residual");
+  TDVC_CHECK(fmap_ok16(*b) && same_geom(*a, *b) && b->C == a->C && fmap_ok16(*y3) && same_geom(*a, *y3) && y3->C == a->C,
+             "tdvc_scale_act_res3: b / y3 must be fp16 maps of a's geometry");
+  TDVC_CHECK(y3->p != y->p && y3->p != a->p && (!r || y3->p != r->p), "tdvc_scale_act_res3: y3 must not alias a, r or y");
+  const long total = (long)a->N * a->H * a->W * (a->C / 8);
+  TDVC_CHECK((!gate || aligned16(gate)) && total < (1L << 31) - (1L << 23), "tdvc_scale_act_res3: gate unaligned or map too large");
+  constexpr int U = 4;
+  long blocks = (total + 256 * U - 1) / (256 * U);
+  if (blocks > 4096) blocks = 4096;
+  hipLaunchKernelGGL(scale_act_res16_y3_kernel<U>, dim3((unsigned)blocks), dim3(256), 0, ST(stream), to_dev(*a), gate, act, slope,
+                     r ? to_dev(*r) : null_fmap(), r_sign, to_dev(*y), to_dev(*b), b_sign, to_dev(*y3), (unsigned)total, (unsigned)(a->C / 8),
+                     (unsigned)((long)a->H * a->W));
+  return tdvc_launch_status("tdvc_scale_act_res3");
+}
+
 extern "C" int tdvc_add_flow(const tdvc_fmap* off, const tdvc_fmap* flow, void* stream) {
   TDVC_CHECK(off && flow && fmap_ok16(*off) && fmap_ok32(*flow) && flow->C >= 2 && same_geom(*off, *flow), "tdvc_add_flow: bad arguments");
   const long total = (long)off->N * off->H * off->W * (off->C / 8);
@@ -775,6 +865,31 @@
   const long total = (long)y->N * y->H * y->W;
   hipLaunchKernelGGL(avgpool2_kernel, grid1d(total), dim3(EW_BLOCK), 0, ST(stream), to_dev(*x), to_dev(*y));
   return tdvc_launch_status("tdvc_avgpool2");
+}
+
+extern "C" int tdvc_avgpool2_pyramid(const tdvc_fmap* xa, const tdvc_fmap* xb, const tdvc_fmap* ya, const tdvc_fmap* yb, void* stream) {
+  TDVC_CHECK(xa && xb && ya && yb && fmap_ok32(*xa) && fmap_ok32(*xb) && same_geom(*xa, *xb), "tdvc_avgpool2_pyramid: two fp32 maps of one geometry");
+  TDVC_CHECK((xa->H % 32) == 0 && (xa->W % 32) == 0, "tdvc_avgpool2_pyramid: H and W must be multiples of 32 (got %dx%d)", xa->H, xa->W);
+  const int C_ = ya[0].C;
+  TDVC_CHECK(C_ >= 1 && C_ <= 4 && C_ <= xa->C && C_ <= xb->C, "tdvc_avgpool2_pyramid: 1 <= C <= 4 channels, not more than the inputs have");
+  auto pix16 = [](const tdvc_fmap& f) { return f.C == 4 && (f.sp % 4) == 0 && (f.sn % 4) == 0 && aligned16(f.p); };
+  bool vec = xa->C >= 4 && xb->C >= 4 && (xa->sp % 4) == 0 && (xb->sp % 4) == 0 && (xa->sn % 4) == 0 && (xb->sn % 4) == 0 && aligned16(xa->p) && aligned16(xb->p);
+  PyramidMaps a;
+  a.x[0] = to_dev(*xa);
+  a.x[1] = to_dev(*xb);
+  for (int m = 0; m < 2; ++m)
+    for (int k = 0; k < 5; ++k) {
+      const tdvc_fmap& y = (m ? yb : ya)[k];
+      TDVC_CHECK(fmap_ok32(y) && y.N == xa->N && y.H == xa->H >> (k + 1) && y.W == xa->W >> (k + 1) && y.C == C_,
+                 "tdvc_avgpool2_pyramid: level %d of map %d must be an fp32 map of %d x %d x %d", k + 1, m, xa->H >> (k + 1), xa->W >> (k + 1), C_);
+      vec = vec && pix16(y);
+      a.y[m][k] = to_dev(y);
+    }
+  TDVC_CHECK(2L * xa->N <= 65535, "tdvc_avgpool2_pyramid: batch too large");
+  const dim3 grid(xa->W / 32, xa->H / 32, 2 * xa->N);
+  if (vec) hipLaunchKernelGGL(avgpool2_pyramid_kernel<true>, grid, dim3(256), 0, ST(stream), a);
+  else hipLaunchKernelGGL(avgpool2_pyramid_kernel<false>, grid, dim3(256), 0, ST(stream), a);
+  return tdvc_launch_status("tdvc_avgpool2_pyramid");
 }
 
 extern "C" int tdvc_spynet_level_input(const tdvc_fmap* ref, const tdvc_fmap* supp, const tdvc_fmap* flow_lo,
diff --git a/tdvc_amd/model/modules.py b/tdvc_amd/model/modules.py
--- a/tdvc_amd/model/modules.py
+++ b/tdvc_amd/model/modules.py
@@ -62,9 +62,15 @@
     def gate(self, x: FM, partial=None) -> torch.Tensor:
         return ops.se_gate(x, self.params(), partial=partial)
 
-    def run(self, x: FM, out: FM | None = None, act=ACT_NONE, slope=0.0, res: FM | None = None, out2: FM | None = None, sums: list | None = None):
+    def run(self, x: FM, out: FM | None = None, act=ACT_NONE, slope=0.0, res: FM | None = None, out2: FM | None = None, sums: list | None = None,
+            then: tuple | None = None):
         out = FM.empty(x.N, x.H, x.W, x.C, dtype=x.t.dtype, device=x.t.device) if out is None else out
-        return ops.scale_act_res(x, out, gate=self.gate(x, sums[0] if sums else None), act=act, slope=slope, res=res, out2=out2)
+        gate = self.gate(x, sums[0] if sums else None)
+        if then is not None:
+            assert out2 is None
+            b, b_sign, out3 = then
+            return ops.scale_act_res3(x, out, b, out3, b_sign, gate=gate, act=act, slope=slope, res=res)
+        return ops.scale_act_res(x, out, gate=gate, act=act, slope=slope, res=res, out2=out2)
 
 
 class Res_Block(nn.Module, PackCache):
@@ -94,6 +100,16 @@
     return x
 
 
+PYRAMID_FUSED = True
+FLOW_EPILOGUE = True
+RESID_FUSED = True
+RGB_HEAD = True
+
+
+def glue_fusions_allowed(module: nn.Module, traced: bool = False) -> bool:
+    return not module.training and ops.TAPE is None and ops.PROFILE is None and not traced
+
+
 class SPyNetBasicModule(nn.Module):
     def __init__(self):
         super().__init__()
@@ -109,11 +125,15 @@
         self.register_buffer("mean", torch.tensor([0.485, 0.456, 0.406]).view(1, 3, 1, 1))
         self.register_buffer("std", torch.tensor([0.229, 0.224, 0.225]).view(1, 3, 1, 1))
 
-    def compute_flow(self, ref: FM, supp: FM) -> FM:
-        refs, supps = [ref], [supp]
-        for _ in range(5):
-            refs.append(ops.avgpool2(refs[-1]))
-            supps.append(ops.avgpool2(supps[-1]))
+    def compute_flow(self, ref: FM, supp: FM, fused: bool = False) -> FM:
+        if fused and PYRAMID_FUSED and ops.avgpool2_pyramid_supported(ref, supp):
+            lr_, ls_ = ops.avgpool2_pyramid(ref, supp)
+            refs, supps = [ref] + lr_, [supp] + ls_
+        else:
+            refs, supps = [ref], [supp]
+            for _ in range(5):
+                refs.append(ops.avgpool2(refs[-1]))
+                supps.append(ops.avgpool2(supps[-1]))
         refs, supps = refs[::-1], supps[::-1]
         dev = ref.t.device
         flow = None
@@ -128,13 +148,13 @@
             flow = ops.conv(x, pk_conv(self, f"l{lvl}c4", bm[4].conv), res=up, out_dtype=torch.float32)
         return flow
 
-    def run(self, ref: FM, supp: FM) -> FM:
+    def run(self, ref: FM, supp: FM, fused: bool = False) -> FM:
         H, W = ref.H, ref.W
         Hu = H if H % 32 == 0 else 32 * (H // 32 + 1)
         Wu = W if W % 32 == 0 else 32 * (W // 32 + 1)
         if (Hu, Wu) != (H, W):
             ref, supp = ops.resize_bilinear(ref, Hu, Wu), ops.resize_bilinear(supp, Hu, Wu)
-        flow = self.compute_flow(ref, supp)
+        flow = self.compute_flow(ref, supp, fused)
         if (Hu, Wu) != (H, W):
             sc = torch.tensor([float(W) / float(Wu), float(H) / float(Hu)], dtype=torch.float32, device=flow.t.device)
             flow = ops.resize_bilinear(flow, H, W, sc)
@@ -177,8 +197,10 @@
         self.attn = SELayer(64)
         self.feat_fusion_ = nn.Conv2d(nf, nf, 3, 1, 1)
 
-    def run(self, feats: FM, cur32: FM, ref32: FM) -> FM:
+    def run(self, feats: FM, cur32: FM, ref32: FM, traced: bool = False) -> FM:
         B, H, W = feats.N, feats.H, feats.W
+        fuse = glue_fusions_allowed(self, traced)
+        flow = None
         dev = feats.t.device
         lr = dict(act=ACT_LRELU, slope=0.1)
         cat1 = feats.ch(0, 128)
@@ -195,6 +217,8 @@
         for i in (3, 2, 1):
             lv = f"l{i}"
             c = cats[i]
+            if i == 1 and fuse and FLOW_EPILOGUE:
+                flow = self.spynet.run(cur32, ref32, fused=fuse)
             o1 = ops.conv(c, pk_conv(self, "c11" + lv, self.offset_conv11[lv]), **lr)
             if i == 3:
                 if ops.conv_pair_supported(o1):
@@ -206,15 +230,16 @@
                     off = ops.conv(o1, pk_conv(self, "c12" + lv, self.offset_conv12[lv]), **lr)
             else:
                 ops.conv(o1, pk_conv(self, "c11_1" + lv, self.offset_conv11_1[lv]), out=up_o1.ch(64, 64), **lr)
-                off = ops.conv(up_o1, pk_conv(self, "ff" + lv, self.feat_fusion[lv]), **lr)
+                off = ops.conv(up_o1, pk_conv(self, "ff" + lv, self.feat_fusion[lv]), flow=flow if i == 1 else None, **lr)
             if i > 1:
                 up = ops.upsample2x(off)
                 up_o1 = FM.empty(B, up.H, up.W, 128, device=dev)
                 ops.conv(up, pk_conv(self, "upc", self.upsample_conv), out=up_o1.ch(0, 64))
-        flow = self.spynet.run(cur32, ref32)
-        if ops.TAPE is not None:
-            off = ops.clone(off)
-        ops.add_flow(off, flow)
+        if flow is None:
+            flow = self.spynet.run(cur32, ref32, fused=fuse)
+            if ops.TAPE is not None:
+                off = ops.clone(off)
+            ops.add_flow(off, flow)
         sums = []
         e = ops.conv(off, pk_conv(self, "ff_", self.feat_fusion_), chan_sum=sums)
         return self.attn.run(e, sums=sums)
@@ -298,18 +323,18 @@
             ops.conv(src.as_slices(b, 4, 64), pc, out=dst.as_slices(b, 4, 64),
                      res=res_buf.as_slices(b, 4, 64) if res_buf is not None else None, **kw)
 
-    def run(self, xt: FM, refs8: FM, out: FM) -> FM:
+    def run(self, xt: FM, refs8: FM, out: FM, then: tuple | None = None) -> FM:
         if (LOOPFILTER_REUSE and LOOPFILTER_PAIR and LOOPFILTER_BCAST and not self.training and ops.TAPE is None and ops.PROFILE is None
                 and not xt.f32 and not refs8.f32 and xt.H * xt.W >= 8192 and ops.conv_pair_supported(xt.as_slices(0, 4, 64))):
-            r = self._run_reuse(xt, refs8, out)
+            r = self._run_reuse(xt, refs8, out, then)
             if r is not None:
                 return r
-        return self._run_plain(xt, refs8, out)
+        return self._run_plain(xt, refs8, out, then)
 
     def reuse_state(self) -> LoopFilterReuse | None:
         return self.__dict__.get("_packed", {}).get("lf_reuse")
 
-    def _run_reuse(self, xt: FM, refs8: FM, out: FM) -> FM | None:
+    def _run_reuse(self, xt: FM, refs8: FM, out: FM, then: tuple | None = None) -> FM | None:
         B, H, W = xt.N, xt.H, xt.W
         dev = xt.t.device
         key = (dev.index, ops._stream().value, B, H, W)
@@ -320,12 +345,12 @@
         if st.usable is False:
             return None
         try:
-            return self._reuse_call(st, xt, refs8, out)
+            return self._reuse_call(st, xt, refs8, out, then)
         except BaseException:
             cache.pop("lf_reuse", None)
             raise
 
-    def _reuse_call(self, st: LoopFilterReuse, xt: FM, refs8: FM, out: FM) -> FM | None:
+    def _reuse_call(self, st: LoopFilterReuse, xt: FM, refs8: FM, out: FM, then: tuple | None = None) -> FM | None:
         B, H, W = xt.N, xt.H, xt.W
         dev = xt.t.device
         lr = dict(act=ACT_LRELU, slope=0.1)
@@ -375,9 +400,9 @@
             ops.conv(s.as_slices(b, 4, 64), pc3, out=o.as_slices(b, 4, 64), res=win(st.A, b, 0, 4))
         sums = []
         f = ops.conv(o, pk_conv(self, "ff", self.feat_fusion), chan_sum=sums, **lr)
-        return self.attn.run(f, out=out, res=xt.ch(192, 64), sums=sums)
-
-    def _run_plain(self, xt: FM, refs8: FM, out: FM) -> FM:
+        return self.attn.run(f, out=out, res=xt.ch(192, 64), sums=sums, then=then)
+
+    def _run_plain(self, xt: FM, refs8: FM, out: FM, then: tuple | None = None) -> FM:
         B, H, W = xt.N, xt.H, xt.W
         dev = xt.t.device
         lr = dict(act=ACT_LRELU, slope=0.1)
@@ -420,7 +445,7 @@
         self._slices("b3", l1.conv3, s, o, res_buf=a)
         sums = []
         f = ops.conv(o, pk_conv(self, "ff", self.feat_fusion), chan_sum=sums, **lr)
-        return self.attn.run(f, out=out, res=xt.ch(192, 64), sums=sums)
+        return self.attn.run(f, out=out, res=xt.ch(192, 64), sums=sums, then=then)
 
 
 class FeatureExtract(nn.Module, PackCache):
@@ -488,7 +513,8 @@
         o2 = self.attn.run(o2, sums=sums, **lr)
         o = run_stack(self.recon_layer, o2, res2=x)
         rgb = torch.empty((B, 3, H, W), dtype=torch.float32, device=dev)
-        ops.conv(o, pk_conv(self, "down", self.featdown), act=ops.ACT_CLAMP01, nchw_out=rgb)
+        with ops.rgb_head_kernel(RGB_HEAD and glue_fusions_allowed(self, trace is not None)):
+            ops.conv(o, pk_conv(self, "down", self.featdown), act=ops.ACT_CLAMP01, nchw_out=rgb)
         if trace is not None:
             trace.update(ff_idx=idx, ff_fin=fin, ff_fref=fref)
         return rgb
diff --git a/tdvc_amd/model/pnet.py b/tdvc_amd/model/pnet.py
--- a/tdvc_amd/model/pnet.py
+++ b/tdvc_amd/model/pnet.py
@@ -5,6 +5,7 @@
 
 from .. import ops
 from ..ops import FM
+from . import modules
 from .coder import MVCoder, ResCoder
 from .modules import FeaExtra, FeatureFix, LoopFilter, MCNet, OffsetGen
 
@@ -81,7 +82,7 @@
             npx_ = float(B * H * W)
             f_cur = self.extra_fea.run(cur8, feats.ch(0, 64))
             self.extra_fea.run(ref8, feats.ch(64, 64))
-            estmv = self.motion_est.run(feats, cur32, ref32)
+            estmv = self.motion_est.run(feats, cur32, ref32, traced=trace is not None)
 
             tr_mv = {} if trace is not None else None
             mv_hat, mv_bits = self.mvCoder.run(estmv, training=training, trace=tr_mv, noise=noise.get("mv"), f32=f32)
@@ -93,8 +94,12 @@
             xt = FM.empty(B, H, W, 256, device=dev)
             pred1 = self.mcnet.run(mv_hat, feats, xt.ch(192, 64))
             pred = FM.empty(B, H, W, 64, device=dev)
-            self.mcfilter.run(xt, refs8, pred)
-            resid = ops.scale_act_res(f_cur, FM.empty(B, H, W, 64, device=dev), res=pred, res_sign=-1.0)
+            resid = FM.empty(B, H, W, 64, device=dev)
+            if modules.RESID_FUSED and modules.glue_fusions_allowed(self, trace is not None):
+                self.mcfilter.run(xt, refs8, pred, then=(f_cur, -1.0, resid))
+            else:
+                self.mcfilter.run(xt, refs8, pred)
+                ops.scale_act_res(f_cur, resid, res=pred, res_sign=-1.0)
 
             tr_res = {} if trace is not None else None
             recon_f, res_bits = self.resCoder.run(resid, training=training, res=pred, trace=tr_res, noise=noise.get("res"), f32=f32)
diff --git a/tdvc_amd/ops.py b/tdvc_amd/ops.py
--- a/tdvc_amd/ops.py
+++ b/tdvc_amd/ops.py
@@ -474,7 +474,8 @@
 
 def conv(x: FM, pc: PackedConv, out: FM | None = None, act=ACT_NONE, slope=0.0, res: FM | None = None,
          res2: FM | None = None, gdn=GDN_NONE, aux: FM | None = None, square=False, out_dtype=None,
-         round16=False, nchw_out: torch.Tensor | None = None, bcast_T=0, bcast_slope=0.0, chan_sum: list | None = None) -> FM | torch.Tensor:
+         round16=False, nchw_out: torch.Tensor | None = None, bcast_T=0, bcast_slope=0.0, chan_sum: list | None = None,
+         flow: FM | None = None) -> FM | torch.Tensor:
     d, ret, Ho, Wo, pc, rec_pc = conv_desc(x, pc, out, act, slope, res, res2, gdn, aux, square, out_dtype, round16, nchw_out, bcast_T, bcast_slope)
     if chan_sum is not None and TAPE is None and FUSE_CHAN_SUM:
         rows = L.lib().tdvc_conv_chan_sum_rows(C.byref(d))
@@ -484,6 +485,16 @@
             chan_sum.append((part, rows))
     if bcast_T and TAPE is not None and not _IN_BACKWARD:
         raise L.TdvcHipError("conv: bcast_T is an inference-only fusion (under the tape use conv + bcast_add_act)")
+    if flow is not None:
+        if (TAPE is not None and not _IN_BACKWARD) or chan_sum is not None or nchw_out is not None:
+            raise L.TdvcHipError("conv: flow is an inference-only fusion of an fmap output, not combined with chan_sum (use conv + add_flow)")
+        d.flow = flow.desc()
+        if L.lib().tdvc_conv_flow_supported(C.byref(d)) != 1:
+            d.flow = _NULL_FM
+            L.check(L.lib().tdvc_conv2d(C.byref(d), _stream()), "conv2d")
+            _log_predicated()
+            add_flow(ret, flow)
+            return ret
     if PROFILE is not None:
         e0, e1 = torch.cuda.Event(enable_timing=True), torch.cuda.Event(enable_timing=True)
         e0.record()
@@ -501,6 +512,22 @@
     _log_predicated()
     _rec("conv", x, rec_pc, None if nchw_out is not None else ret, act, slope, res, res2, gdn, aux, square, nchw_out)
     return ret
+
+
+class rgb_head_kernel:
+
+    def __init__(self, enable: bool):
+        self.enable = bool(enable)
+
+    def __enter__(self):
+        if not self.enable:
+            L.lib().tdvc_debug_enable_conv_head3(0)
+        return self
+
+    def __exit__(self, *exc):
+        if not self.enable:
+            L.lib().tdvc_debug_enable_conv_head3(1)
+        return False
 
 
 class PackedConvPair:
@@ -862,6 +889,22 @@
     L.check(L.lib().tdvc_axpy_f32(dst.data_ptr(), src.data_ptr(), scale, dst.numel(), _stream()), "axpy_f32")
 
 
+def scale_act_res3(a: FM, out: FM, b: FM, out3: FM, b_sign=-1.0, gate: torch.Tensor | None = None, act=ACT_NONE, slope=0.0,
+                   res: FM | None = None, res_sign=1.0) -> FM:
+    if TAPE is not None and not _IN_BACKWARD:
+        raise L.TdvcHipError("scale_act_res3 is an inference-only fusion (under the tape: two scale_act_res calls)")
+    if not (a.f32 or out.f32 or b.f32 or out3.f32 or (res is not None and res.f32)):
+        da, dy, db, d3 = a.desc(), out.desc(), b.desc(), out3.desc()
+        dr = res.desc() if res is not None else None
+        L.check(L.lib().tdvc_scale_act_res3(C.byref(da), gate.data_ptr() if gate is not None else None, act, slope,
+                                            C.byref(dr) if dr is not None else None, res_sign, C.byref(dy), C.byref(db), b_sign,
+                                            C.byref(d3), _stream()), "scale_act_res3")
+        return out
+    scale_act_res(a, out, gate=gate, act=act, slope=slope, res=res, res_sign=res_sign)
+    scale_act_res(b, out3, res=out, res_sign=b_sign)
+    return out
+
+
 def scale_act_res(a: FM, out: FM, gate: torch.Tensor | None = None, act=ACT_NONE, slope=0.0, res: FM | None = None,
                   res_sign=1.0, out2: FM | None = None) -> FM:
     da, dy = a.desc(), out.desc()
@@ -938,6 +981,19 @@
     dx, dy = x.desc(), out.desc()
     L.check(L.lib().tdvc_avgpool2(C.byref(dx), C.byref(dy), _stream()), "avgpool2")
     return out
+
+
+def avgpool2_pyramid_supported(a: FM, b: FM) -> bool:
+    return a.f32 and b.f32 and (a.N, a.H, a.W, a.C) == (b.N, b.H, b.W, b.C) and a.C <= 4 and a.H % 32 == 0 and a.W % 32 == 0
+
+
+def avgpool2_pyramid(a: FM, b: FM) -> tuple:
+    lv = lambda x: [FM.empty(x.N, x.H >> k, x.W >> k, x.C, dtype=torch.float32, device=x.t.device) for k in range(1, 6)]
+    la, lb = lv(a), lv(b)
+    da, db = a.desc(), b.desc()
+    ya, yb = (L.FMapDesc * 5)(*[f.desc() for f in la]), (L.FMapDesc * 5)(*[f.desc() for f in lb])
+    L.check(L.lib().tdvc_avgpool2_pyramid(C.byref(da), C.byref(db), ya, yb, _stream()), "avgpool2_pyramid")
+    return la, lb
 
 
 def spynet_level_input(ref: FM, supp: FM, flow_lo: FM | None, flow_up: FM, cat8: FM):
```

After: 52.07 frames/s, median of 6. 1.01x the previous value.
